# akanazawa/human_dynamics

Measured on AMD Instinct MI355X. Metric: frames/sec/GPU (ResNet+temporal+SMPL, 224x224); SMPL verts max-abs-err, higher is better.
Workload: dtype f16x3

## Files before the change

### human_dynamics_amd/_lib.py

```python
from __future__ import annotations

import ctypes as C
import os

from . import devflags

HERE = os.path.dirname(os.path.abspath(__file__))
LIB_PATH = devflags.get("LIB_PATH") or os.path.join(HERE, "libhmmr_hip.so")

HMMR_F32, HMMR_BF16, HMMR_F16X3 = 0, 1, 2
FLAG_SATURATED = 1
FLAG_NAN = 2
ABI_VERSION = 19
RESNET_UNITS = 16
RESNET_PROF_SLOTS = 64
MAX_TEMPORAL_BLOCKS = 8
MAX_REGRESSORS = 8

_vp, _fp, _ip = C.c_void_p, C.c_void_p, C.c_void_p


class ConvDesc(C.Structure):
    _fields_ = [
        ("in_", _vp), ("w", _vp), ("scale", _fp), ("shift", _fp), ("res", _vp), ("out", _vp),
        ("out2", _vp), ("scale2", _fp), ("shift2", _fp),
        ("in_dtype", C.c_int), ("out_dtype", C.c_int),
        ("n_img", C.c_int), ("hin", C.c_int), ("win", C.c_int), ("cin", C.c_int),
        ("in_img_stride", C.c_int64), ("in_row_stride", C.c_int), ("in_px_stride", C.c_int),
        ("kh", C.c_int), ("kw", C.c_int), ("sy", C.c_int), ("sx", C.c_int), ("py", C.c_int), ("px", C.c_int),
        ("ho", C.c_int), ("wo", C.c_int), ("cout", C.c_int), ("ldo", C.c_int),
        ("ldr", C.c_int), ("res_strided", C.c_int), ("res_img_stride", C.c_int64),
        ("res_row_stride", C.c_int), ("res_px_stride", C.c_int),
        ("relu", C.c_int), ("tile", C.c_int),
        ("split_k", C.c_int), ("ws", _vp), ("ws_bytes", C.c_size_t),
        ("pro_scale", _fp), ("pro_shift", _fp),
        ("out_b", _vp), ("ldo_b", C.c_int), ("n_split", C.c_int), ("relu_b", C.c_int),
        ("in2", _vp), ("cin2", C.c_int), ("k_order", C.c_int),
        ("batch", C.c_int), ("batch_in_bytes", C.c_int64), ("batch_w_bytes", C.c_int64), ("batch_out_bytes", C.c_int64),
        ("batch_res_bytes", C.c_int64), ("batch_scale_bytes", C.c_int64), ("batch_shift_bytes", C.c_int64),
    ]


class TailDesc(C.Structure):
    _fields_ = [
        ("dtype", C.c_int), ("h2", _vp), ("m", C.c_int), ("c_mid", C.c_int), ("depth", C.c_int),
        ("w3", _vp), ("scale3", _fp), ("shift3", _fp),
        ("res", _vp), ("ldr", C.c_int), ("res_strided", C.c_int), ("res_img_stride", C.c_int64),
        ("res_row_stride", C.c_int), ("res_px_stride", C.c_int), ("ho", C.c_int), ("wo", C.c_int),
        ("out", _vp), ("pre_scale", _fp), ("pre_shift", _fp),
        ("w1", _vp), ("scale1", _fp), ("shift1", _fp), ("relu1", C.c_int), ("n2", C.c_int),
        ("out_h1", _vp),
        ("h1", _vp), ("hin", C.c_int), ("win", C.c_int), ("w2", _vp), ("scale2", _fp), ("shift2", _fp),
        ("xp", _vp), ("wsc", _vp), ("shift_sc", _fp),
        ("conv2_stride", C.c_int), ("out_pre", _vp),
        ("pair_stream", _vp), ("c_xp", C.c_int), ("unit_stream", _vp),
    ]


class Debug(C.Structure):
    _fields_ = [("stem_route", C.c_int), ("stem_no_conv1", C.c_int), ("gemm_probe", C.c_int), ("smpl_blend_mfma", C.c_int), ("ief_no_group", C.c_int), ("reserved", C.c_int * 3),
                ("pair_min_pixels", C.c_int), ("pair_two_tile_min", C.c_int), ("pair_form", C.c_int)]


class LaunchCounts(C.Structure):
    _fields_ = [("unit_pair", C.c_ulonglong), ("b1_unit", C.c_ulonglong), ("tail_split", C.c_ulonglong), ("conv3x3_stream", C.c_ulonglong),
                ("conv1x1_stream", C.c_ulonglong)]


class StemCounts(C.Structure):
    _fields_ = [(k, C.c_ulonglong) for k in ("fused", "fused_conv1", "repack", "gemm", "pool")]


TILE_GENERIC, TILE_PATCH, TILE_STREAM_3X3, TILE_STREAM_1X1 = range(4)
CONV_TILE_MAX = 63


class ConvTileInfo(C.Structure):
    _fields_ = [(k, C.c_int) for k in ("tile", "family", "fm", "fn", "wgm", "wgn", "pixels", "channels", "row_blocks", "depth", "occupancy", "wmax",
                                       "split_only", "conv3_form", "cols", "tune_cols", "narrow", "rank", "candidate")] + [("text", C.c_char_p)]


class Layer(C.Structure):
    _fields_ = [("w", _vp), ("scale", _fp), ("shift", _fp), ("tile", C.c_int), ("k_order", C.c_int)]


class ResnetUnit(C.Structure):
    _fields_ = [("conv1", Layer), ("conv2", Layer), ("conv3", Layer), ("shortcut", Layer), ("c3sc", Layer), ("sc_c1", Layer),
                ("w3_frag", _vp), ("w1n_frag", _vp), ("pair_stream", _vp), ("conv1_frag", _vp), ("unit_stream", _vp), ("pre_scale", _fp), ("pre_shift", _fp),
                ("c_in", C.c_int), ("base", C.c_int), ("depth", C.c_int), ("stride", C.c_int),
                ("fuse_preact", C.c_int), ("fuse_tail", C.c_int)]


class ResnetWeights(C.Structure):
    _fields_ = [("dtype", C.c_int), ("stem", Layer),
                ("unit", ResnetUnit * RESNET_UNITS), ("post_scale", _fp), ("post_shift", _fp)]


SC_NONE, SC_LAUNCH, SC_LAUNCH_WITH_CONV1, SC_IN_CONV3, SC_IN_TAIL = range(5)
CONV1_LAUNCH, CONV1_READY = range(2)
CONV2_LAUNCH, CONV2_IN_TAIL = range(2)
END_CONV3_LAUNCH, END_TAIL_BF16, END_TAIL_BF16_STRIDE2, END_TAIL_SPLIT, END_B1_UNIT, END_UNIT_PAIR = range(6)


class UnitPlan(C.Structure):
    _fields_ = [(k, C.c_int) for k in ("shortcut", "conv1", "conv2", "end", "reads_fused_preact", "writes_raw", "writes_pre",
                                       "pair_demoted", "swaps_t1_t2", "leaves_h1")]


def resnet_plan(rw, n_total):
    plan = (UnitPlan * RESNET_UNITS)()
    check(load().hmmr_resnet50_plan(C.byref(rw), int(n_total), plan), "hmmr_resnet50_plan")
    return list(plan)


class TemporalBlock(C.Structure):
    _fields_ = [("gn1_gamma", _fp), ("gn1_beta", _fp), ("conv1", Layer),
                ("gn2_gamma", _fp), ("gn2_beta", _fp), ("conv2", Layer)]


class TemporalWeights(C.Structure):
    _fields_ = [("dtype", C.c_int), ("num_blocks", C.c_int), ("block", TemporalBlock * MAX_TEMPORAL_BLOCKS)]


class HallucinatorWeights(C.Structure):
    _fields_ = [("dtype", C.c_int), ("fc1", Layer), ("fc2", Layer), ("fc3", Layer)]


class IefRegressor(C.Structure):
    _fields_ = [("nd", C.c_int), ("fc1_phi", Layer), ("fc1_theta", Layer), ("fc2", Layer), ("fc3", Layer)]


class IefWeights(C.Structure):
    _fields_ = [("dtype", C.c_int), ("num_regressors", C.c_int), ("num_stages", C.c_int),
                ("reg", IefRegressor * MAX_REGRESSORS), ("mean_theta", _fp),
                ("no_optcam", C.c_int), ("delta_from_start", C.c_int)]


class IefRegGrads(C.Structure):
    _fields_ = [(k, _fp) for k in ("d_fc1_phi", "d_fc1_theta", "d_fc2", "d_fc3", "d_b1", "d_b2", "d_b3")]


class IefBwdDesc(C.Structure):
    _fields_ = [("strips", _fp), ("omega_start", _fp), ("keep", _vp), ("keep_scale", C.c_float), ("m", C.c_int), ("d_omegas", _fp),
                ("d_strips", _fp), ("d_omega_start", _fp), ("reg", IefRegGrads * MAX_REGRESSORS)]


TEMPORAL_GRAD_NAMES = ("gn1_gamma", "gn1_beta", "conv1", "b1", "gn2_gamma", "gn2_beta", "conv2", "b2")
HALLUCINATOR_GRAD_NAMES = ("fc1", "fc2", "fc3", "b1", "b2", "b3")


class TemporalBlockGrads(C.Structure):
    _fields_ = [("d_" + k, _fp) for k in TEMPORAL_GRAD_NAMES]


class TemporalBwdDesc(C.Structure):
    _fields_ = [("phi", _fp), ("b", C.c_int), ("t", C.c_int), ("d_strips", _fp), ("d_phi", _fp),
                ("block", TemporalBlockGrads * MAX_TEMPORAL_BLOCKS)]


class HallucinatorBwdDesc(C.Structure):
    _fields_ = [("phi", _fp), ("m", C.c_int), ("d_out", _fp), ("d_phi", _fp)] + [("d_" + k, _fp) for k in HALLUCINATOR_GRAD_NAMES]


class SmplConsts(C.Structure):
    _fields_ = [("num_verts", C.c_int), ("num_kps", C.c_int), ("lbs_nnz", C.c_int), ("vpad", C.c_int),
                ("dirs", _fp), ("j_template", _fp), ("j_shapedirs", _fp), ("parents", _ip),
                ("lbs_idx", _ip), ("lbs_w", _fp), ("kreg_ptr", _ip), ("kreg_idx", _ip), ("kreg_val", _fp),
                ("dirs_split", _vp)]


class SmplGradConsts(C.Structure):
    _fields_ = [("num_verts", C.c_int), ("num_kps", C.c_int), ("vk_ptr", _ip), ("vk_idx", _ip), ("vk_val", _fp)]


LOSS_KP, LOSS_KP_OPTCAM, LOSS_JOINTS, LOSS_SMPL, LOSS_CONST, LOSS_SHAPE_PRIOR = 1, 2, 4, 8, 16, 32
LOSS_NAMES = ("e_kp", "e_joints", "e_smpl_pose", "e_smpl_shape", "e_const", "e_shape", "total")
LOSS_NO_VISIBLE, LOSS_NOT_FINITE = 1, 2


class SeqLossDesc(C.Structure):
    _fields_ = [("B", C.c_int), ("T", C.c_int), ("K", C.c_int), ("delta_t", C.c_int), ("flags", C.c_uint), ("weights", C.c_float * 6),
                ("kps_pred", _fp), ("joints_pred", _fp), ("rs_pred", _fp), ("beta_pred", _fp), ("ld_beta", C.c_int),
                ("kps_gt", _fp), ("joints_gt", _fp), ("rs_gt", _fp), ("shapes_gt", _fp), ("has_gt3d_smpl", _fp), ("has_gt3d_joints", _fp),
                ("losses", _fp), ("d_kps", _fp), ("d_joints", _fp), ("d_rs", _fp), ("d_beta", _fp), ("best_cam", _fp), ("status", _vp),
                ("ws", _vp), ("ws_bytes", C.c_size_t)]


class Var(C.Structure):
    _fields_ = [("name", C.c_char_p), ("data", _fp), ("numel", C.c_int64)]


class SmplSource(C.Structure):
    _fields_ = [("num_verts", C.c_int), ("num_kps", C.c_int), ("v_template", _fp), ("shapedirs", _fp), ("posedirs", _fp),
                ("J_regressor", _fp), ("lbs_weights", _fp), ("kp_regressor", _fp), ("parents", _ip)]


class VideoPlan(C.Structure):
    _fields_ = [(k, C.c_int) for k in ("n", "T", "fov", "margin", "g", "n_windows", "max_frames", "max_windows", "resnet_passes", "tail_passes")]


class TracksPlan(C.Structure):
    _fields_ = [(k, C.c_int) for k in ("n_tracks", "T", "fov", "margin", "g", "n_frames", "n_windows", "max_frames", "max_windows",
                                       "resnet_passes", "tail_passes")]


class Model(C.Structure):
    _fields_ = [("resnet", C.POINTER(ResnetWeights)), ("temporal", C.POINTER(TemporalWeights)), ("hallucinator", C.POINTER(HallucinatorWeights)),
                ("ief", C.POINTER(IefWeights)), ("smpl", C.POINTER(SmplConsts)), ("sequence_length", C.c_int), ("fov", C.c_int)]


RENDER_MAX_FRAMES, RENDER_MIN_SIZE, RENDER_MAX_SIZE, RENDER_MAX_FACES = 4096, 16, 1024, 65536
RENDER_BG_COLOR, RENDER_BG_FLOAT, RENDER_BG_FRAME = 0, 1, 2
TRACK_MAX_KPS, TRACK_MAX_KERNEL, TRACK_MAX_RADIUS, TRACK_MAX_ROWS, TRACK_TILE = 64, 31, 64, 1 << 27, 256
TRACK_EMPTY, TRACK_BEFORE_ORIGIN, TRACK_CLIPPED, TRACK_NOT_FINITE = 1, 2, 4, 8
BBOX_EMPTY, BBOX_NOT_FINITE, BBOX_DEGENERATE, BBOX_BEYOND_START = 1, 2, 4, 8


class RenderDesc(C.Structure):
    _fields_ = [("verts", _fp), ("ld_verts", C.c_int64), ("cams", _fp), ("ld_cam", C.c_int64), ("geom", _fp),
                ("faces", _ip), ("face_colors", _fp), ("ld_face_colors", C.c_int64),
                ("n", C.c_int), ("nv", C.c_int), ("nf", C.c_int), ("size", C.c_int),
                ("rotate", C.c_int), ("rot", C.c_float * 9), ("color", C.c_float * 3), ("bg_color", C.c_float * 3),
                ("light_dir", C.c_float * 3), ("light_int_ambient", C.c_float), ("light_int_directional", C.c_float),
                ("light_color_ambient", C.c_float * 3), ("light_color_directional", C.c_float * 3),
                ("bg_mode", C.c_int), ("bg_image", _vp), ("bg_add", C.c_float), ("bg_mul", C.c_float),
                ("frame_h", C.c_int), ("frame_w", C.c_int), ("out_h", C.c_int), ("out_w", C.c_int),
                ("rgb", _vp), ("alpha", _fp), ("face_index", _ip), ("ws", _vp), ("ws_bytes", C.c_size_t)]


SCENE_MAX_TRACKS = 16


class SceneTrack(C.Structure):
    _fields_ = [("verts", _fp), ("ld_verts", C.c_int64), ("cams", _fp), ("ld_cam", C.c_int64), ("geom", _fp),
                ("priority", _fp), ("start", C.c_int), ("end", C.c_int), ("color", C.c_float * 3)]


class SceneDesc(C.Structure):
    _fields_ = [("tracks", C.POINTER(SceneTrack)), ("n_tracks", C.c_int), ("faces", _ip),
                ("nv", C.c_int), ("nf", C.c_int), ("n_frames", C.c_int), ("size", C.c_int),
                ("out_h", C.c_int), ("out_w", C.c_int), ("bg_color", C.c_float * 3),
                ("light_dir", C.c_float * 3), ("light_int_ambient", C.c_float), ("light_int_directional", C.c_float),
                ("light_color_ambient", C.c_float * 3), ("light_color_directional", C.c_float * 3),
                ("bg_mode", C.c_int), ("bg_image", _vp), ("frame_h", C.c_int), ("frame_w", C.c_int),
                ("rgb", _vp), ("alpha", _fp), ("face_index", _ip), ("owner", _ip), ("ws", _vp), ("ws_bytes", C.c_size_t)]


SKELETON_MAX_RADIUS, COLLAGE_MAX_PANEL_WIDTH = 1024, 4096


class SkeletonDesc(C.Structure):
    _fields_ = [("kps", _fp), ("ld_kps", C.c_int64), ("vis", _vp), ("n", C.c_int), ("nk", C.c_int), ("h", C.c_int), ("w", C.c_int),
                ("kp_add", C.c_float), ("kp_mul", C.c_float), ("draw_edges", C.c_int), ("radius", C.c_int),
                ("bg_float", _fp), ("bg_add", C.c_float), ("bg_mul", C.c_float), ("bg_u8", _vp), ("out", _vp)]


class CollageDesc(C.Structure):
    _fields_ = [("rend_crop", _vp), ("skel_crop", _vp), ("render_og", _vp), ("rot_og", _vp),
                ("n", C.c_int), ("S", C.c_int), ("h", C.c_int), ("w", C.c_int), ("out", _vp)]


SIGNATURES = {
    "hmmr_abi_version": (C.c_int, []),
    "hmmr_pack_resnet_bytes": (C.c_size_t, [C.POINTER(Var), C.c_int, C.c_int]),
    "hmmr_pack_resnet": (C.c_int, [C.POINTER(Var), C.c_int, C.c_int, _vp, C.c_size_t, _vp, C.POINTER(ResnetWeights)]),
    "hmmr_pack_temporal_bytes": (C.c_size_t, [C.POINTER(Var), C.c_int, C.c_int, C.c_int]),
    "hmmr_pack_temporal": (C.c_int, [C.POINTER(Var), C.c_int, C.c_int, C.c_int, _vp, C.c_size_t, _vp, C.POINTER(TemporalWeights)]),
    "hmmr_pack_hallucinator_bytes": (C.c_size_t, [C.POINTER(Var), C.c_int, C.c_int]),
    "hmmr_pack_hallucinator": (C.c_int, [C.POINTER(Var), C.c_int, C.c_int, _vp, C.c_size_t, _vp, C.POINTER(HallucinatorWeights)]),
    "hmmr_pack_ief_bytes": (C.c_size_t, [C.POINTER(Var), C.c_int, C.c_int, C.POINTER(C.c_int), C.c_int]),
    "hmmr_pack_ief": (C.c_int, [C.POINTER(Var), C.c_int, C.c_int, C.POINTER(C.c_int), C.c_int, C.c_int, _vp, C.c_size_t, _vp, C.POINTER(IefWeights)]),
    "hmmr_pack_smpl_bytes": (C.c_size_t, [C.POINTER(SmplSource), C.c_int, C.c_int]),
    "hmmr_pack_smpl": (C.c_int, [C.POINTER(SmplSource), C.c_int, C.c_int, _vp, C.c_size_t, _vp, C.POINTER(SmplConsts)]),
    "hmmr_pack_smpl_grad_bytes": (C.c_size_t, [C.POINTER(SmplSource), C.c_int]),
    "hmmr_pack_smpl_grad": (C.c_int, [C.POINTER(SmplSource), C.c_int, _vp, C.c_size_t, _vp, C.POINTER(SmplGradConsts)]),
    "hmmr_last_error": (C.c_char_p, []),
    "hmmr_run_flags": (C.c_int, [C.POINTER(C.c_uint), C.c_int]),
    "hmmr_set_debug": (None, [C.POINTER(Debug)]),
    "hmmr_get_debug": (None, [C.POINTER(Debug)]),
    "hmmr_launch_counts": (None, [C.POINTER(LaunchCounts), C.c_int]),
    "hmmr_stem_launch_counts": (None, [C.POINTER(StemCounts), C.c_int]),
    "hmmr_conv_gemm": (C.c_int, [C.POINTER(ConvDesc), _vp]),
    "hmmr_conv_tile_info": (C.c_int, [C.c_int, C.POINTER(ConvTileInfo)]),
    "hmmr_conv_tile_for": (C.c_int, [C.c_int] * 6),
    "hmmr_conv_tile_fits": (C.c_int, [C.c_int] * 8),
    "hmmr_conv_tile_f_movie": (C.c_int, []),
    "hmmr_conv_splitk_workspace_bytes": (C.c_size_t, [C.c_int, C.c_int, C.c_int]),
    "hmmr_resnet50_workspace_bytes": (C.c_size_t, [C.c_int, C.c_int]),
    "hmmr_resnet50_fwd": (C.c_int, [C.POINTER(ResnetWeights), _fp, C.c_int, C.c_int, _fp, _vp, C.c_size_t, _vp,
                                    C.POINTER(C.c_float)]),
    "hmmr_resnet50_stem_workspace_bytes": (C.c_size_t, [C.POINTER(ResnetWeights), C.c_int]),
    "hmmr_resnet50_stem": (C.c_int, [C.POINTER(ResnetWeights), _fp, C.c_int, C.c_int, _vp, _vp, C.POINTER(C.c_int), _vp, C.c_size_t, _vp]),
    "hmmr_resnet50_plan": (C.c_int, [C.POINTER(ResnetWeights), C.c_int, C.POINTER(UnitPlan)]),
    "hmmr_temporal_workspace_bytes": (C.c_size_t, [C.c_int, C.c_int, C.c_int]),
    "hmmr_temporal_fwd": (C.c_int, [C.POINTER(TemporalWeights), _fp, C.c_int, C.c_int, _fp, _vp, C.c_size_t, _vp]),
    "hmmr_hallucinator_workspace_bytes": (C.c_size_t, [C.c_int, C.c_int]),
    "hmmr_hallucinator_fwd": (C.c_int, [C.POINTER(HallucinatorWeights), _fp, C.c_int, _fp, _vp, C.c_size_t, _vp]),
    "hmmr_groupnorm_relu": (C.c_int, [_fp, _fp, _fp, C.c_int, C.c_int, C.c_int, C.c_int, _vp, C.c_int, _vp]),
    "hmmr_ief_workspace_bytes": (C.c_size_t, [C.c_int, C.c_int, C.c_int]),
    "hmmr_ief_fwd": (C.c_int, [C.POINTER(IefWeights), _fp, C.c_int, _fp, _vp, C.c_size_t, _vp]),
    "hmmr_ief_fwd_from": (C.c_int, [C.POINTER(IefWeights), _fp, _fp, C.c_int, _fp, _vp, C.c_size_t, _vp]),
    "hmmr_ief_bwd_workspace_bytes": (C.c_size_t, [C.c_int, C.c_int, C.c_int]),
    "hmmr_ief_fwd_train": (C.c_int, [C.POINTER(IefWeights), _fp, _fp, _vp, C.c_float, C.c_int, _fp, _vp, C.c_size_t, _vp]),
    "hmmr_ief_bwd": (C.c_int, [C.POINTER(IefWeights), C.POINTER(IefBwdDesc), _vp, C.c_size_t, _vp]),
    "hmmr_temporal_bwd_workspace_bytes": (C.c_size_t, [C.c_int, C.c_int, C.c_int]),
    "hmmr_temporal_bwd": (C.c_int, [C.POINTER(TemporalWeights), C.POINTER(TemporalBwdDesc), _vp, C.c_size_t, _vp]),
    "hmmr_hallucinator_bwd_workspace_bytes": (C.c_size_t, [C.c_int]),
    "hmmr_hallucinator_bwd": (C.c_int, [C.POINTER(HallucinatorWeights), C.POINTER(HallucinatorBwdDesc), _vp, C.c_size_t, _vp]),
    "hmmr_smpl_workspace_bytes": (C.c_size_t, [C.c_int]),
    "hmmr_smpl_fwd": (C.c_int, [C.POINTER(SmplConsts), _fp, C.c_int, _fp, C.c_int, _fp, C.c_int, C.c_int,
                                _fp, _fp, _fp, _fp, _vp, C.c_size_t, _vp]),
    "hmmr_smpl_bwd_workspace_bytes": (C.c_size_t, [C.POINTER(SmplConsts), C.c_int]),
    "hmmr_smpl_bwd": (C.c_int, [C.POINTER(SmplConsts), C.POINTER(SmplGradConsts), _fp, C.c_int, _fp, C.c_int, _fp, C.c_int, _fp, C.c_int,
                                _fp, _fp, _fp, _fp, _fp, _fp, _fp, _vp, C.c_size_t, _vp]),
    "hmmr_seq_losses_workspace_bytes": (C.c_size_t, [C.c_int, C.c_int]),
    "hmmr_seq_losses": (C.c_int, [C.POINTER(SeqLossDesc), _vp]),
    "hmmr_omega_loss_grad_workspace_bytes": (C.c_size_t, [C.POINTER(SmplConsts), C.c_int, C.c_int]),
    "hmmr_omega_loss_grad": (C.c_int, [C.POINTER(SmplConsts), C.POINTER(SmplGradConsts), C.POINTER(SeqLossDesc), _fp, C.c_int, _fp, _fp,
                                       _vp, C.c_size_t, _vp]),
    "hmmr_crop_frames": (C.c_int, [_vp, _ip, C.c_int, C.c_int, C.c_int, _fp, _vp]),
    "hmmr_tube_augment": (C.c_int, [_vp, C.c_int, C.c_int, C.c_int, C.c_int, _ip, _vp, _fp, C.c_int, _fp, _vp]),
    "hmmr_track_workspace_bytes": (C.c_size_t, [C.c_int, C.c_int]),
    "hmmr_track_bbox": (C.c_int, [_fp, _vp, C.POINTER(C.c_int32), C.c_int, C.c_int, C.c_double, C.c_int, C.POINTER(C.c_double), C.c_int,
                                  _fp, _fp, _ip, _vp, C.c_size_t, _vp]),
    "hmmr_track_smooth": (C.c_int, [_fp, C.POINTER(C.c_int32), C.c_int, C.c_int, C.POINTER(C.c_double), C.c_int, _fp, _vp, C.c_size_t, _vp]),
    "hmmr_track_crop_geom": (C.c_int, [_fp, C.POINTER(C.c_int32), _ip, C.c_int, C.c_int, C.c_int, _ip, _fp, _ip, _vp]),
    "hmmr_bottleneck_tail": (C.c_int, [C.POINTER(TailDesc), _vp]),
    "hmmr_pair_stream_bytes": (C.c_size_t, [C.c_int, C.c_int, C.c_int]),
    "hmmr_b1_unit_stream_bytes": (C.c_size_t, [C.c_int]),
    "hmmr_conv3x3_stream_bytes": (C.c_size_t, [C.c_int, C.c_int]),
    "hmmr_conv1x1_stream_bytes": (C.c_size_t, [C.c_int, C.c_int]),
    "hmmr_mfma_rate_probe": (C.c_int, [C.c_int, C.c_int, _fp, _vp]),
    "hmmr_clock_probe": (C.c_int, [_vp, C.c_int, C.c_int, _vp, _vp]),
    "hmmr_render_handoff": (C.c_int, [_fp, C.c_int64, _fp, C.c_int64, _fp, C.c_int64, _fp, C.c_int, C.c_int, C.c_int,
                                      _fp, _fp, _fp, _vp]),
    "hmmr_render_workspace_bytes": (C.c_size_t, [C.c_int, C.c_int, C.c_int]),
    "hmmr_render_mesh": (C.c_int, [C.POINTER(RenderDesc), _vp]),
    "hmmr_render_scene_workspace_bytes": (C.c_size_t, [C.c_int, C.c_int, C.c_int, C.c_int]),
    "hmmr_render_scene": (C.c_int, [C.POINTER(SceneDesc), _vp]),
    "hmmr_video_bbox": (C.c_int, [_fp, C.c_longlong, _fp, C.c_longlong, C.c_int, _fp, C.c_double, C.POINTER(C.c_int32), C.c_int, C.c_int, C.c_int,
                                  C.c_double, _ip, _fp, _ip, _vp]),
    "hmmr_skeleton_radius": (C.c_int, [C.c_int, C.c_int]),
    "hmmr_draw_skeleton": (C.c_int, [C.POINTER(SkeletonDesc), _vp]),
    "hmmr_collage_width": (C.c_int, [C.c_int, C.c_int, C.c_int]),
    "hmmr_compose_collage": (C.c_int, [C.POINTER(CollageDesc), _vp]),
    "hmmr_eval_joints": (C.c_int, [_fp, _fp, C.c_int, C.c_int, C.c_int, C.c_int, _fp, _fp, _fp, _fp, _vp]),
    "hmmr_eval_verts": (C.c_int, [_fp, C.c_int64, _fp, C.c_int64, C.c_int, C.c_int, _fp, _vp]),
    "hmmr_eval_joints_ld": (C.c_int, [_fp, C.c_int64, _fp, C.c_int64, C.c_int, C.c_int, C.c_int, C.c_int, _fp, _fp, _fp, _fp, _vp]),
    "hmmr_eval_kps": (C.c_int, [_fp, C.c_int64, _fp, C.c_int64, C.c_int, C.c_int, C.c_double, C.c_int, C.c_float,
                                _fp, _fp, _fp, _fp, _vp]),
    "hmmr_rotmat_to_axis_angle": (C.c_int, [_fp, C.c_int64, C.c_int, C.c_int, _fp, C.c_int64, _vp]),
    "hmmr_axis_angle_to_rotmat": (C.c_int, [_fp, C.c_int64, C.c_int, C.c_int, _fp, C.c_int64, _vp]),
    "hmmr_global_rigid_transformation": (C.c_int, [_fp, _fp, _ip, C.c_int, _fp, _fp, C.c_int, _vp]),
    "hmmr_smpl_fwd_records": (C.c_int, [C.POINTER(SmplConsts), _fp, C.c_int, C.c_int, _fp, C.c_int64, C.POINTER(C.c_int32),
                                        _vp, C.c_size_t, _vp]),
    "hmmr_smpl_fwd_strided": (C.c_int, [C.POINTER(SmplConsts), _fp, C.c_int, _fp, C.c_int, _fp, C.c_int, C.c_int,
                                        _fp, _fp, _fp, _fp, C.c_int64, _vp, C.c_size_t, _vp]),
    "hmmr_video_plan": (C.c_int, [C.c_int, C.c_int, C.c_int, C.c_int, C.c_int, C.POINTER(VideoPlan)]),
    "hmmr_record_layout": (C.c_int, [C.c_int, C.c_int, C.c_int, C.POINTER(C.c_int32), C.POINTER(C.c_int64)]),
    "hmmr_gather_windows": (C.c_int, [_fp, C.c_int, _fp, C.c_int, C.c_int, C.c_int, C.c_int, C.c_int, C.c_int, _fp, _vp]),
    "hmmr_keep_rows": (C.c_int, [_fp, C.c_int, C.c_int, C.c_int, C.c_int, C.c_int, C.c_int, C.c_int, _fp, C.c_int64, _vp]),
    "hmmr_predict_video_workspace_bytes": (C.c_size_t, [C.POINTER(Model), C.c_int, C.c_int, C.c_int]),
    "hmmr_predict_video": (C.c_int, [C.POINTER(Model), _fp, C.c_int, _fp, C.c_int64, C.POINTER(C.c_int32), C.c_int, C.c_int,
                                     _vp, C.c_size_t, _vp]),
    "hmmr_tracks_plan": (C.c_int, [C.POINTER(C.c_int32), C.c_int, C.c_int, C.c_int, C.c_int, C.c_int, C.POINTER(TracksPlan)]),
    "hmmr_tracks_window_owner": (C.c_int, [C.POINTER(C.c_int32), C.c_int, C.c_int, C.c_int, C.POINTER(C.c_int), C.POINTER(C.c_int)]),
    "hmmr_tracks_window_rows": (C.c_int, [C.POINTER(C.c_int32), C.c_int, C.c_int, C.c_int, C.c_int, C.POINTER(C.c_int), C.POINTER(C.c_int)]),
    "hmmr_tracks_tail_pass": (C.c_int, [C.POINTER(C.c_int32), C.c_int, C.POINTER(TracksPlan), C.c_int, C.POINTER(C.c_int), C.POINTER(C.c_int),
                                        C.POINTER(C.c_int), C.POINTER(C.c_int)]),
    "hmmr_gather_windows_tracks": (C.c_int, [_fp, _fp, C.POINTER(C.c_int32), C.c_int, C.c_int, C.c_int, C.c_int, C.c_int, C.c_int, C.c_int, _fp, _vp]),
    "hmmr_keep_rows_tracks": (C.c_int, [_fp, C.POINTER(C.c_int32), C.c_int, C.c_int, C.c_int, C.c_int, C.c_int, C.c_int, C.c_int, _fp, C.c_int64,
                                        _vp]),
    "hmmr_predict_tracks_workspace_bytes": (C.c_size_t, [C.POINTER(Model), C.POINTER(C.c_int32), C.c_int, C.c_int, C.c_int]),
    "hmmr_predict_tracks": (C.c_int, [C.POINTER(Model), _fp, C.POINTER(C.c_int32), C.c_int, _fp, C.c_int64, C.POINTER(C.c_int32), C.c_int, C.c_int,
                                      _vp, C.c_size_t, _vp]),
}

_lib = None


class HmmrError(RuntimeError):
    pass


def load():
    global _lib
    if _lib is not None:
        return _lib
    if not os.path.exists(LIB_PATH):
        raise HmmrError("%s not found: build it with `python -m human_dynamics_amd.build` "
                        "(the HIP library is mandatory; there is no CPU fallback)" % LIB_PATH)
    import torch
    if torch.cuda.is_available():
        torch.cuda.init()
    lib = C.CDLL(LIB_PATH)
    for name, (res, args) in SIGNATURES.items():
        fn = getattr(lib, name)
        fn.restype, fn.argtypes = res, args
    if lib.hmmr_abi_version() != ABI_VERSION:
        raise HmmrError("libhmmr_hip.so ABI version mismatch")
    _lib = lib
    return lib


def launch_counts(clear=False):
    c = LaunchCounts()
    load().hmmr_launch_counts(C.byref(c), int(bool(clear)))
    return {k: int(getattr(c, k)) for k, _ in LaunchCounts._fields_}


def conv_tiles(family=None):
    lib, rows = load(), []
    for t in range(1, CONV_TILE_MAX + 1):
        r = ConvTileInfo()
        if lib.hmmr_conv_tile_info(t, C.byref(r)) == 0 and family in (None, r.family):
            rows.append(r)
    return rows


def stem_launch_counts(clear=False):
    c = StemCounts()
    load().hmmr_stem_launch_counts(C.byref(c), int(bool(clear)))
    return {k: int(getattr(c, k)) for k, _ in StemCounts._fields_}


def check(rc, what=""):
    if rc != 0:
        msg = load().hmmr_last_error()
        raise HmmrError("%s failed (%d): %s" % (what or "hmmr call", rc, msg.decode() if msg else "?"))


def ptr(t):
    return None if t is None else t.data_ptr()
```

### human_dynamics_amd/csrc/gemm_conv.hip

```cpp
#include <stdlib.h>
#include <string.h>
#include <type_traits>

#include "conv_tiles.h"
#include "stream_kit.h"

struct ConvArgs {
    const void* in; const void* w; const float* scale; const float* shift;
    const void* res; void* out; void* out2; const float* scale2; const float* shift2;
    const float* pro_scale; const float* pro_shift;
    void* out_b; int ldo_b, n_split, relu_b;
    int M, K, cout, ldo, ldr;
    int Wo, HoWo, Hin, Win;
    long long in_img_stride; int in_row_stride, in_px_stride;
    int cin_log2, KH, KW, SY, SX, PY, PX;
    int res_strided; long long res_img_stride; int res_row_stride, res_px_stride;
    int relu, tiles_n, n_tiles;
    int kt_per_slice;
    long long out_slice_stride;
    int probe;
    const void* in2; int cin2, kt_split;
    int batch; long long bz_in, bz_w, bz_out, bz_res, bz_scale, bz_shift;
};

__device__ __forceinline__ ConvArgs batch_problem(const ConvArgs& a0, int z) {
    ConvArgs a = a0;
    if (a0.batch > 1) {
        const long long zz = z;
        a.in = (const char*)a0.in + zz * a0.bz_in;
        a.w = (const char*)a0.w + zz * a0.bz_w;
        if (a0.out) a.out = (char*)a0.out + zz * a0.bz_out;
        if (a0.out2) a.out2 = (char*)a0.out2 + zz * a0.bz_out;
        if (a0.res) a.res = (const char*)a0.res + zz * a0.bz_res;
        if (a0.scale) a.scale = (const float*)((const char*)a0.scale + zz * a0.bz_scale);
        if (a0.shift) a.shift = (const float*)((const char*)a0.shift + zz * a0.bz_shift);
        if (a0.scale2) a.scale2 = (const float*)((const char*)a0.scale2 + zz * a0.bz_scale);
        if (a0.shift2) a.shift2 = (const float*)((const char*)a0.shift2 + zz * a0.bz_shift);
    }
    return a;
}

#ifdef HMMR_GEMM_PROBE
#define HMMR_PROBE(a, bit) (((a).probe & (bit)) != 0)
#else
#define HMMR_PROBE(a, bit) false
#endif

template <typename TA> struct Frag;
template <> struct Frag<float>  { typedef f32x4 type; };
template <> struct Frag<bf16_t> { typedef bf16x8 type; };
struct split_frag { shalf8 hi, lo; };
template <> struct Frag<bsplit_t> { typedef split_frag type; };

__device__ __forceinline__ f32x16 mma(const f32x4& a, const f32x4& b, f32x16 c) {
#pragma unroll
    for (int j = 0; j < 4; ++j) c = __builtin_amdgcn_mfma_f32_32x32x2f32(a[j], b[j], c, 0, 0, 0);
    return c;
}
__device__ __forceinline__ f32x16 mma(const bf16x8& a, const bf16x8& b, f32x16 c) {
    return __builtin_amdgcn_mfma_f32_32x32x16_bf16(a, b, c, 0, 0, 0);
}
__device__ __forceinline__ f32x16 mma(const split_frag& a, const split_frag& b, f32x16 c) {
    c = mfma_split(a.lo, b.hi, c);
    c = mfma_split(a.hi, b.lo, c);
    return mfma_split(a.hi, b.hi, c);
}
template <typename TA> struct FragIO {
    static constexpr int CHUNKS = 4;
    __device__ static __forceinline__ typename Frag<TA>::type read(const char* row, int c, int lh, int fsw) {
        return *(const typename Frag<TA>::type*)(row + (((2 * c + lh) ^ fsw) << 4));
    }
};
template <> struct FragIO<bsplit_t> {
    static constexpr int CHUNKS = 2;
    __device__ static __forceinline__ split_frag read(const char* row, int c, int lh, int fsw) {
        const int g = 2 * (2 * c + lh);
        split_frag f;
        f.hi = *(const shalf8*)(row + ((g ^ fsw) << 4));
        f.lo = *(const shalf8*)(row + (((g + 1) ^ fsw) << 4));
        return f;
    }
};
template <typename TO> __device__ __forceinline__ void store_tail(TO* p, const float (&v)[8], int cnt) {
    if constexpr (!std::is_same<TO, bsplit_t>::value)
        for (int j = 0; j < cnt; ++j) p[j] = elem_traits<TO>::from_f32(v[j]);
}

__device__ const u32x4 g_zero_page[4] = {};

template <typename TA> __device__ __forceinline__ u32x4 preact_slot(const u32x4& v, const f32x4* sc, const f32x4* sh);
template <> __device__ __forceinline__ u32x4 preact_slot<float>(const u32x4& v, const f32x4* sc, const f32x4* sh) {
    u32x4 o;
#pragma unroll
    for (int i = 0; i < 4; ++i) o[i] = __float_as_uint(fmaxf(fmaf(__uint_as_float(v[i]), sc[0][i], sh[0][i]), 0.f));
    return o;
}
template <> __device__ __forceinline__ u32x4 preact_slot<bf16_t>(const u32x4& v, const f32x4* sc, const f32x4* sh) {
    u32x4 o;
#pragma unroll
    for (int i = 0; i < 4; ++i) {
        const float lo = __uint_as_float(v[i] << 16), hi = __uint_as_float(v[i] & 0xffff0000u);
        const int e = 2 * i;
        const float a = fmaxf(fmaf(lo, sc[e >> 2][e & 3], sh[e >> 2][e & 3]), 0.f);
        const float b = fmaxf(fmaf(hi, sc[(e + 1) >> 2][(e + 1) & 3], sh[(e + 1) >> 2][(e + 1) & 3]), 0.f);
        typedef __attribute__((ext_vector_type(2))) __bf16 bf16x2;
        bf16x2 pk = {(bf16_t)a, (bf16_t)b};
        o[i] = __builtin_bit_cast(unsigned, pk);
    }
    return o;
}


template <typename TA, typename TO, int BM, int BN, int WGM, int WGN, bool PRO, bool UTAP, int NSTAGE>
__global__ __launch_bounds__(WGM * WGN * 64, NSTAGE >= 3 ? (WGM * WGN) / 4 : ((WGM * WGN == 8) ? 4 : 1))
void conv_gemm_kernel(const ConvArgs a0) {
    const ConvArgs a = batch_problem(a0, blockIdx.z);
    static_assert(NSTAGE >= 2 && NSTAGE <= 4, "2 stages (two workgroups per CU) or a 3/4-stage ring (one workgroup per CU)");
    static_assert(NSTAGE == 2 || WGM * WGN == 8, "the deep ring is written for 8-wave workgroups");
    static_assert(!PRO || UTAP, "the fused pre-activation needs one tap per K step");
    constexpr int NT = WGM * WGN * 64;
    constexpr int RPP = NT / 8;
    constexpr int EPS = elem_traits<TA>::EPS;
    constexpr int BKE = 8 * EPS;
    constexpr int TM = BM / WGM, TN = BN / WGN;
    constexpr int FM = TM / 32, FN = TN / 32;
    constexpr int PA = BM / RPP, PB = BN / RPP;
    static_assert(PA >= 1 && PB >= 1, "tile smaller than one staging pass");
    constexpr int A_BYTES = BM * 128, B_BYTES = BN * 128, STAGE = A_BYTES + B_BYTES;
    typedef typename Frag<TA>::type frag_t;

    extern __shared__ __attribute__((aligned(16))) char smem[];

    const int tid = threadIdx.x;
    const int lane = tid & 63;
    const int wave = __builtin_amdgcn_readfirstlane(tid >> 6);
    const int L = xcd_remap(blockIdx.x, a.n_tiles);
    const int m0 = (L / a.tiles_n) * BM;
    const int n0 = (L % a.tiles_n) * BN;

    const int pslot = tid & 7, r0 = tid >> 3;
    const int lslot = pslot ^ ((r0 >> 1) & 7);
    const TA* __restrict__ in = (const TA*)a.in;
    const TA* __restrict__ wt = (const TA*)a.w;

    const TA* aptr[PA]; unsigned amask[PA];
#pragma unroll
    for (int p = 0; p < PA; ++p) {
        const int m = m0 + r0 + RPP * p;
        aptr[p] = in; amask[p] = 0u;
        if (m < a.M) {
            const int img = m / a.HoWo, rem = m - img * a.HoWo;
            const int oy = rem / a.Wo, ox = rem - oy * a.Wo;
            const int iy0 = oy * a.SY - a.PY, ix0 = ox * a.SX - a.PX;
            aptr[p] = in + (long long)img * a.in_img_stride + (long long)iy0 * a.in_row_stride +
                      (long long)ix0 * a.in_px_stride + lslot * EPS;
            unsigned mk = 0u;
            for (int t = 0; t < a.KH * a.KW; ++t) {
                const int ky = t / a.KW, kx = t - ky * a.KW;
                if ((unsigned)(iy0 + ky) < (unsigned)a.Hin && (unsigned)(ix0 + kx) < (unsigned)a.Win) mk |= 1u << t;
            }
            amask[p] = mk;
        }
    }
    const TA* wptr = wt + (long long)(n0 + r0) * a.K + lslot * EPS;
    const int cin_mask = (1 << a.cin_log2) - 1;

    auto tap_of = [&](int k, int& tap) -> int {
        tap = k >> a.cin_log2;
        const int ci = k & cin_mask;
        int ky, kx;
        if (a.KW == 1) { ky = tap; kx = 0; }
        else if (a.KW == 3) { ky = (int)(((unsigned)tap * 43691u) >> 17); kx = tap - 3 * ky; }
        else { ky = tap / a.KW; kx = tap - ky * a.KW; }
        return ky * a.in_row_stride + kx * a.in_px_stride + ci;
    };

    constexpr bool SPLIT = std::is_same<TA, bsplit_t>::value;
    constexpr int PCH = EPS;
    u32x4 ra[PRO ? PA : 1];
    f32x4 psc[PRO ? PCH / 4 : 1], psh[PRO ? PCH / 4 : 1];
    auto glds_a = [&](int kt, int buf) {
        int tap;
        const int koff = UTAP ? tap_of(kt * BKE, tap) : tap_of(kt * BKE + lslot * EPS, tap) - lslot * EPS;
        char* sa = smem + buf * STAGE + wave * 1024;
        if (a.in2 && kt >= a.kt_split) {
            const TA* in2 = (const TA*)a.in2 + (kt - a.kt_split) * BKE + lslot * EPS;
#pragma unroll
            for (int p = 0; p < PA; ++p) {
                const void* src = (amask[p] & 1u) ? (const void*)(in2 + (long long)(m0 + r0 + RPP * p) * a.cin2)
                                                  : (const void*)g_zero_page;
                __builtin_amdgcn_global_load_lds((gptr_t)src, (lptr_t)(sa + p * (RPP * 128)), 16, 0, 0);
            }
            return;
        }
#pragma unroll
        for (int p = 0; p < PA; ++p) {
            const bool ok = (amask[p] >> tap) & 1u;
            const void* src = ok ? (const void*)(aptr[p] + koff) : (const void*)g_zero_page;
            __builtin_amdgcn_global_load_lds((gptr_t)src, (lptr_t)(sa + p * (RPP * 128)), 16, 0, 0);
        }
    };
    auto glds_b = [&](int kt, int buf) {
        char* sb = smem + buf * STAGE + A_BYTES + wave * 1024;
#pragma unroll
        for (int p = 0; p < PB; ++p)
            __builtin_amdgcn_global_load_lds((gptr_t)(wptr + (long long)(RPP * p) * a.K + kt * BKE),
                                             (lptr_t)(sb + p * (RPP * 128)), 16, 0, 0);
    };
    u32x4 rb[PRO ? PB : 1];
    auto load_regs = [&](int kt) {
        if constexpr (PRO) {
            int tap;
            const int koff = tap_of(kt * BKE, tap);
            const int ci = ((kt * BKE) & cin_mask) + lslot * EPS;
#pragma unroll
            for (int q = 0; q < PCH / 4; ++q) {
                psc[q] = *(const f32x4*)(a.pro_scale + ci + 4 * q);
                psh[q] = *(const f32x4*)(a.pro_shift + ci + 4 * q);
            }
#pragma unroll
            for (int p = 0; p < PA; ++p) ra[p] = *(const u32x4*)(aptr[p] + koff);
#pragma unroll
            for (int p = 0; p < PB; ++p) rb[p] = *(const u32x4*)(wptr + (long long)(RPP * p) * a.K + kt * BKE);
        }
    };
    auto store_regs = [&](int buf) {
        if constexpr (PRO) {
            char* sa = smem + buf * STAGE + r0 * 128 + pslot * 16;
#pragma unroll
            for (int p = 0; p < PA; ++p) {
                if constexpr (SPLIT) *(u32x4*)(sa + p * (RPP * 128)) = preact_slot_split(ra[p], psc[0], psh[0], lslot & 1);
                else *(u32x4*)(sa + p * (RPP * 128)) = preact_slot<TA>(ra[p], psc, psh);
            }
#pragma unroll
            for (int p = 0; p < PB; ++p) *(u32x4*)(sa + A_BYTES + p * (RPP * 128)) = rb[p];
        }
    };

    const int wm = wave / WGN, wn = wave % WGN;
    const int lr = lane & 31, lh = lane >> 5;
    const int fsw = (lr >> 1) & 7;
    const int a_row_off = (wm * TM + lr) * 128;
    const int b_row_off = A_BYTES + (wn * TN + lr) * 128;

    f32x16 acc[FM][FN];
#pragma unroll
    for (int i = 0; i < FM; ++i)
#pragma unroll
        for (int j = 0; j < FN; ++j)
#pragma unroll
            for (int r = 0; r < 16; ++r) acc[i][j][r] = 0.f;

    constexpr int VPR = BN / 8;
    constexpr int NIT = (BM * VPR) / NT;
    constexpr int RV = (int)(8 * sizeof(TO) / 16);
    const TO* __restrict__ res = PRO ? nullptr : (const TO*)a.res;
    u32x4 rres[PRO ? 1 : NIT][RV];
    if (!PRO && res) {
#pragma unroll
        for (int it = 0; it < NIT; ++it) {
            const int idx = it * NT + tid;
            const int m = m0 + idx / VPR, n = n0 + (idx % VPR) * 8;
#pragma unroll
            for (int q = 0; q < RV; ++q) rres[it][q] = u32x4{0u, 0u, 0u, 0u};
            if (m < a.M && n < a.cout) {
                long long ro;
                if (a.res_strided) {
                    const int img = m / a.HoWo, rem = m - img * a.HoWo;
                    const int oy = rem / a.Wo, ox = rem - oy * a.Wo;
                    ro = (long long)img * a.res_img_stride + (long long)oy * a.res_row_stride +
                         (long long)ox * a.res_px_stride + n;
                } else {
                    ro = (long long)m * a.ldr + n;
                }
#pragma unroll
                for (int q = 0; q < RV; ++q) rres[it][q] = *((const u32x4*)(res + ro) + q);
            }
        }
    }

    const int nk = a.K / BKE;
    auto compute_stage = [&](const char* sbuf) {
        constexpr int NCHK = FragIO<TA>::CHUNKS;
        constexpr bool DBUF = NSTAGE >= 3 || !(std::is_same<TA, bsplit_t>::value && WGM * WGN == 8 && FM * FN >= 2);
        frag_t fa[DBUF ? 2 : 1][FM], fb[DBUF ? 2 : 1][FN];
        auto read_frags = [&](int c, int slot_) {
#pragma unroll
            for (int i = 0; i < FM; ++i) fa[slot_][i] = FragIO<TA>::read(sbuf + a_row_off + i * 32 * 128, c, lh, fsw);
#pragma unroll
            for (int j = 0; j < FN; ++j) fb[slot_][j] = FragIO<TA>::read(sbuf + b_row_off + j * 32 * 128, c, lh, fsw);
        };
        if constexpr (DBUF) {
            read_frags(0, 0);
#pragma unroll
            for (int c = 0; c < NCHK; ++c) {
                if (c + 1 < NCHK) read_frags(c + 1, (c + 1) & 1);
                __builtin_amdgcn_sched_barrier(0);
#pragma unroll
                for (int i = 0; i < FM; ++i)
#pragma unroll
                    for (int j = 0; j < FN; ++j) acc[i][j] = mma(fa[c & 1][i], fb[c & 1][j], acc[i][j]);
            }
        } else {
#pragma unroll
            for (int c = 0; c < NCHK; ++c) {
                read_frags(c, 0);
#pragma unroll
                for (int i = 0; i < FM; ++i)
#pragma unroll
                    for (int j = 0; j < FN; ++j) acc[i][j] = mma(fa[0][i], fb[0][j], acc[i][j]);
            }
        }
    };
    const int kt0 = blockIdx.y * a.kt_per_slice;
    const int kt1 = min(nk, kt0 + a.kt_per_slice);
    if constexpr (NSTAGE >= 3) {
        constexpr int LPW = PA + PB;
        static_assert(LPW * (NSTAGE - 2) < 64, "vmcnt range");
        [[maybe_unused]] float* s_pro = (float*)(smem + NSTAGE * STAGE);
        if constexpr (PRO) {
            for (int i = tid; i < a.K; i += NT) { s_pro[i] = a.pro_scale[i]; s_pro[a.K + i] = a.pro_shift[i]; }
        }
        auto transform = [&](int kt, int buf) {
            if constexpr (PRO) {
                const int ci = ((kt * BKE) & cin_mask) + lslot * EPS;
                f32x4 sc_[PCH / 4], sh_[PCH / 4];
#pragma unroll
                for (int q = 0; q < PCH / 4; ++q) {
                    sc_[q] = *(const f32x4*)(s_pro + ci + 4 * q);
                    sh_[q] = *(const f32x4*)(s_pro + a.K + ci + 4 * q);
                }
                char* sa = smem + buf * STAGE + r0 * 128 + pslot * 16;
#pragma unroll
                for (int p = 0; p < PA; ++p) {
                    u32x4* q = (u32x4*)(sa + p * (RPP * 128));
                    if constexpr (SPLIT) *q = preact_slot_split(*q, sc_[0], sh_[0], lslot & 1);
                    else *q = preact_slot<TA>(*q, sc_, sh_);
                }
            }
        };
        auto wait_ahead = [&](int ahead) {
            __builtin_amdgcn_sched_barrier(0);
            if (ahead >= 2) { if constexpr (NSTAGE >= 4) wait_vm_lgkm0<2 * LPW>(); }
            else if (ahead == 1) wait_vm_lgkm0<LPW>();
            else wait_vm_lgkm0<0>();
        };
        const int nloc = kt1 - kt0;
#pragma unroll
        for (int s_ = 0; s_ < NSTAGE - 1; ++s_)
            if (s_ < nloc && !HMMR_PROBE(a, 8)) { glds_a(kt0 + s_, s_); glds_b(kt0 + s_, s_); }
        if constexpr (PRO) {
            wait_vm_lgkm0<63>();
            __builtin_amdgcn_s_barrier();
        }
        wait_ahead(min(NSTAGE - 2, nloc - 1));
        transform(kt0, 0);
        wait_vm_lgkm0<63>();
        __builtin_amdgcn_s_barrier();
        constexpr int NCHK = FragIO<TA>::CHUNKS;
        const int grp = wave >> 2;
        int cur = 0, nxt = NSTAGE - 1;
        if (grp == 1) __builtin_amdgcn_s_barrier();
        for (int kt = kt0; kt < kt1; ++kt) {
            const char* sbuf = smem + cur * STAGE;
            const int c1 = (cur + 1 == NSTAGE) ? 0 : cur + 1;
            const bool fill = kt + NSTAGE - 1 < kt1 && !HMMR_PROBE(a, 2);
            frag_t fa[NCHK][FM], fb[NCHK][FN];
#pragma unroll
            for (int c = 0; c < NCHK; ++c) {
                if (c > 0 && HMMR_PROBE(a, 16)) {
#pragma unroll
                    for (int i = 0; i < FM; ++i) fa[c][i] = fa[0][i];
#pragma unroll
                    for (int j = 0; j < FN; ++j) fb[c][j] = fb[0][j];
                    continue;
                }
#pragma unroll
                for (int i = 0; i < FM; ++i) fa[c][i] = FragIO<TA>::read(sbuf + a_row_off + i * 32 * 128, c, lh, fsw);
#pragma unroll
                for (int j = 0; j < FN; ++j) fb[c][j] = FragIO<TA>::read(sbuf + b_row_off + j * 32 * 128, c, lh, fsw);
            }
            if (fill) {
                if (!HMMR_PROBE(a, 64)) glds_a(kt + NSTAGE - 1, nxt);
                if (!HMMR_PROBE(a, 32)) glds_b(kt + NSTAGE - 1, nxt);
            }
            if (grp == 1 && kt + 1 < kt1) {
                wait_ahead(min(NSTAGE - 2, kt1 - 2 - kt));
                transform(kt + 1, c1);
            }
            wait_vm_lgkm0<63>();
            __builtin_amdgcn_sched_barrier(0);
            __builtin_amdgcn_s_barrier();
            __builtin_amdgcn_sched_barrier(0);
            if (!HMMR_PROBE(a, 1)) {
                __builtin_amdgcn_s_setprio(1);
#pragma unroll
                for (int c = 0; c < NCHK; ++c)
#pragma unroll
                    for (int i = 0; i < FM; ++i)
#pragma unroll
                        for (int j = 0; j < FN; ++j) acc[i][j] = mma(fa[c][i], fb[c][j], acc[i][j]);
                __builtin_amdgcn_s_setprio(0);
            }
            if (grp == 0 && kt + 1 < kt1) {
                wait_ahead(min(NSTAGE - 2, kt1 - 2 - kt));
                transform(kt + 1, c1);
                wait_vm_lgkm0<63>();
            }
            __builtin_amdgcn_sched_barrier(0);
            __builtin_amdgcn_s_barrier();
            __builtin_amdgcn_sched_barrier(0);
            nxt = cur; cur = c1;
        }
        if (grp == 0) __builtin_amdgcn_s_barrier();
    } else if constexpr (PRO) {
        load_regs(kt0);
        store_regs(0);
        if (kt0 + 1 < kt1) load_regs(kt0 + 1);
        __syncthreads();
        for (int kt = kt0; kt < kt1; ++kt) {
            const int cur = (kt - kt0) & 1;
            if (kt + 1 < kt1 && !HMMR_PROBE(a, 2)) store_regs(cur ^ 1);
            if (kt + 2 < kt1 && !HMMR_PROBE(a, 2)) load_regs(kt + 2);
            if (!HMMR_PROBE(a, 1)) compute_stage(smem + cur * STAGE);
            if (!HMMR_PROBE(a, 4)) __syncthreads();
        }
    } else {
        glds_a(kt0, 0);
        glds_b(kt0, 0);
        __syncthreads();
        for (int kt = kt0; kt < kt1; ++kt) {
            const int cur = (kt - kt0) & 1;
            if (kt + 1 < kt1 && !HMMR_PROBE(a, 2)) { glds_a(kt + 1, cur ^ 1); glds_b(kt + 1, cur ^ 1); }
            if (!HMMR_PROBE(a, 1)) compute_stage(smem + cur * STAGE);
            if (!HMMR_PROBE(a, 4)) __syncthreads();
        }
    }

    float* sc = (float*)smem;
#pragma unroll
    for (int i = 0; i < FM; ++i)
#pragma unroll
        for (int j = 0; j < FN; ++j)
#pragma unroll
            for (int r = 0; r < 16; ++r) {
                const int row = wm * TM + i * 32 + (r & 3) + 8 * (r >> 2) + 4 * lh;
                const int col = wn * TN + j * 32 + lr;
                sc[row * BN + col] = acc[i][j][r];
            }
    __syncthreads();

    TO* __restrict__ out = a.out ? (TO*)a.out + (long long)blockIdx.y * a.out_slice_stride : nullptr;
    TO* __restrict__ out2 = (TO*)a.out2;
    float satmax = 0.f;
#pragma unroll
    for (int it = 0; it < NIT; ++it) {
        const int idx = it * NT + tid;
        const int row = idx / VPR, col = (idx % VPR) * 8;
        const int m = m0 + row, n = n0 + col;
        if (m >= a.M || n >= a.cout) continue;
        float v[8];
        load8(sc + row * BN + col, v);
        if (a.scale && a.shift) {
            float s[8], b[8]; load8(a.scale + n, s); load8(a.shift + n, b);
#pragma unroll
            for (int j = 0; j < 8; ++j) v[j] = fmaf(v[j], s[j], b[j]);
        } else if (a.scale) {
            float s[8]; load8(a.scale + n, s);
#pragma unroll
            for (int j = 0; j < 8; ++j) v[j] *= s[j];
        } else if (a.shift) {
            float b[8]; load8(a.shift + n, b);
#pragma unroll
            for (int j = 0; j < 8; ++j) v[j] += b[j];
        }
        const bool full = (n + 8 <= a.cout);
        if (!PRO && res) {
            float rr[8];
            unpack8<TO>(rres[PRO ? 0 : it], rr);
#pragma unroll
            for (int j = 0; j < 8; ++j) v[j] += rr[j];
        }
        const bool second = a.out_b && n >= a.n_split;
        if (second ? a.relu_b : a.relu) {
#pragma unroll
            for (int j = 0; j < 8; ++j) v[j] = fmaxf(v[j], 0.f);
        }
        if (second) {
            TO* ob = (TO*)a.out_b + (long long)m * a.ldo_b + (n - a.n_split);
            if (full) store8<TO>(ob, v, satmax);
            else store_tail(ob, v, a.cout - n);
            continue;
        }
        const long long oo = (long long)m * a.ldo + n;
        if (out) {
            if (full) store8<TO>(out + oo, v, satmax);
            else store_tail(out + oo, v, a.cout - n);
        }
        if (out2) {
            float s2[8], b2[8], u[8];
            load8(a.scale2 + n, s2); load8(a.shift2 + n, b2);
#pragma unroll
            for (int j = 0; j < 8; ++j) {
                const float vr = stored_value<TO>(v[j]);
                u[j] = fmaxf(fmaf(vr, s2[j], b2[j]), 0.f);
            }
            if (full) store8<TO>(out2 + oo, u, satmax);
            else store_tail(out2 + oo, u, a.cout - n);
        }
    }
    if constexpr (std::is_same<TO, bsplit_t>::value) split_flag_max(satmax);
}

__device__ __forceinline__ unsigned patch_tap_mask(int m, const ConvArgs& a) {
    if (m >= a.M) return 0u;
    const int rem = m % a.HoWo, y = rem / a.Wo, x = rem - y * a.Wo;
    unsigned mk = 0u;
#pragma unroll
    for (int t = 0; t < 9; ++t) {
        const int yy = y + t / 3 - 1, xx = x + t % 3 - 1;
        if ((unsigned)yy < (unsigned)a.Hin && (unsigned)xx < (unsigned)a.Win) mk |= 1u << t;
    }
    return mk;
}
template <typename TO, int BM, int BN, int WGM, int WGN>
__device__ __forceinline__ void patch_epilogue(const ConvArgs& a, char* smem, const f32x16 (&acc)[2][2], int m0, int n0,
                                               int tid, int wm, int wn, int lr, int lh) {
    constexpr int NT = 512, TM = BM / WGM, TN = BN / WGN;
    static_assert(TM == 64 && TN == 64, "64x64 wave tiles");
    float* sc = (float*)smem;
#pragma unroll
    for (int i = 0; i < 2; ++i)
#pragma unroll
        for (int j = 0; j < 2; ++j)
#pragma unroll
            for (int r = 0; r < 16; ++r) {
                const int row = wm * TM + i * 32 + (r & 3) + 8 * (r >> 2) + 4 * lh;
                const int col = wn * TN + j * 32 + lr;
                sc[row * BN + col] = acc[i][j][r];
            }
    __syncthreads();
    constexpr int VPR = BN / 8, NIT = (BM * VPR) / NT;
    TO* __restrict__ out = (TO*)a.out;
    float satmax = 0.f;
#pragma unroll
    for (int it = 0; it < NIT; ++it) {
        const int idx = it * NT + tid;
        const int row = idx / VPR, col = (idx % VPR) * 8;
        const int m = m0 + row, n = n0 + col;
        if (m >= a.M || n >= a.cout) continue;
        float v[8];
        load8(sc + row * BN + col, v);
        if (a.scale && a.shift) {
            float s[8], b[8]; load8(a.scale + n, s); load8(a.shift + n, b);
#pragma unroll
            for (int j = 0; j < 8; ++j) v[j] = fmaf(v[j], s[j], b[j]);
        } else if (a.scale) {
            float s[8]; load8(a.scale + n, s);
#pragma unroll
            for (int j = 0; j < 8; ++j) v[j] *= s[j];
        } else if (a.shift) {
            float b[8]; load8(a.shift + n, b);
#pragma unroll
            for (int j = 0; j < 8; ++j) v[j] += b[j];
        }
        if (a.relu) {
#pragma unroll
            for (int j = 0; j < 8; ++j) v[j] = fmaxf(v[j], 0.f);
        }
        store8<TO>(out + (long long)m * a.ldo + n, v, satmax);
    }
    if constexpr (std::is_same<TO, bsplit_t>::value) split_flag_max(satmax);
}

template <typename TA, typename TO, int BM, int BN, int WGM, int WGN, int NPP>
__global__ __launch_bounds__(512, 1) void conv3x3_patch_kernel(const ConvArgs a) {
    static_assert(WGM * WGN == 8, "8-wave workgroups");
    constexpr int RPP = 64, NSB = 3;
    constexpr int EPS = elem_traits<TA>::EPS, BKE = 8 * EPS;
    constexpr int TM = BM / WGM, TN = BN / WGN, FM = TM / 32, FN = TN / 32;
    constexpr int PB = BN / RPP;
    constexpr int B_BYTES = BN * 128, P_BYTES = NPP * RPP * 128, OFF_P = NSB * B_BYTES;
    constexpr int NCHK = FragIO<TA>::CHUNKS;
    typedef typename Frag<TA>::type frag_t;

    extern __shared__ __attribute__((aligned(16))) char smem[];
    const int tid = threadIdx.x;
    const int lane = tid & 63;
    const int wave = __builtin_amdgcn_readfirstlane(tid >> 6);
    const int L = xcd_remap(blockIdx.x, a.n_tiles);
    const int m0 = (L / a.tiles_n) * BM;
    const int n0 = (L % a.tiles_n) * BN;
    const int W = a.Win, C = 1 << a.cin_log2;
    const int need = BM + 2 * W + 2;
    constexpr int ZROW = NPP * RPP - 2;
    const int base = m0 - W - 1;

    const int pslot = tid & 7, r0 = tid >> 3;
    const int lslot = pslot ^ ((r0 >> 1) & 7);
    const TA* __restrict__ in = (const TA*)a.in;
    const TA* pptr[NPP];
#pragma unroll
    for (int p = 0; p < NPP; ++p) {
        const int r = RPP * p + r0, px = base + r;
        pptr[p] = (r < need && px >= 0 && px < a.M) ? in + (long long)px * C + lslot * EPS : nullptr;
    }
    const TA* wptr = (const TA*)a.w + (long long)(n0 + r0) * a.K + lslot * EPS;
    auto glds_patch = [&](int c, int buf) {
        char* sp = smem + OFF_P + buf * P_BYTES + wave * 1024;
#pragma unroll
        for (int p = 0; p < NPP; ++p) {
            const void* src = pptr[p] ? (const void*)(pptr[p] + c * BKE) : (const void*)g_zero_page;
            __builtin_amdgcn_global_load_lds((gptr_t)src, (lptr_t)(sp + p * (RPP * 128)), 16, 0, 0);
        }
    };
    auto glds_b = [&](int kt, int buf) {
        char* sb = smem + buf * B_BYTES + wave * 1024;
#pragma unroll
        for (int p = 0; p < PB; ++p)
            __builtin_amdgcn_global_load_lds((gptr_t)(wptr + (long long)(RPP * p) * a.K + kt * BKE),
                                             (lptr_t)(sb + p * (RPP * 128)), 16, 0, 0);
    };

    const int wm = wave / WGN, wn = wave % WGN;
    const int lr = lane & 31, lh = lane >> 5;
    const int fswb = (lr >> 1) & 7;
    const int b_row_off = (wn * TN + lr) * 128;
    int prow[FM];
    unsigned pmask[FM];
#pragma unroll
    for (int i = 0; i < FM; ++i) {
        prow[i] = wm * TM + i * 32 + lr;
        pmask[i] = patch_tap_mask(m0 + prow[i], a);
    }

    f32x16 acc[FM][FN];
#pragma unroll
    for (int i = 0; i < FM; ++i)
#pragma unroll
        for (int j = 0; j < FN; ++j)
#pragma unroll
            for (int r = 0; r < 16; ++r) acc[i][j][r] = 0.f;

    const int nc = C / BKE, nk = 9 * nc;
    auto wait_stage = [&](int kt, int t, int c) {
        __builtin_amdgcn_sched_barrier(0);
        if (kt + 2 < nk) {
            if (t <= 1 && c + 1 < nc) wait_vm_lgkm0<PB + NPP>();
            else wait_vm_lgkm0<PB>();
        } else wait_vm_lgkm0<0>();
    };
    glds_patch(0, 0);
    glds_b(0, 0);
    glds_b(1, 1);
    __builtin_amdgcn_sched_barrier(0);
    wait_vm_lgkm0<PB>();
    __builtin_amdgcn_s_barrier();
    const int grp = wave >> 2;
    int cur = 0, nxt = NSB - 1, t = 0, c = 0;
    if (grp == 1) __builtin_amdgcn_s_barrier();
    for (int kt = 0; kt < nk; ++kt) {
        const char* sb = smem + cur * B_BYTES;
        const char* sp = smem + OFF_P + (c & 1) * P_BYTES;
        const int c1 = (cur + 1 == NSB) ? 0 : cur + 1;
        const int ky = (t * 11) >> 5;
        int ts = ky * W + (t - 3 * ky);
        if (HMMR_PROBE(a, 128)) ts = 0;
        if (HMMR_PROBE(a, 256)) ts &= ~1;
        if (HMMR_PROBE(a, 512)) ts &= ~15;
        frag_t fa[NCHK][FM], fb[NCHK][FN];
#pragma unroll
        for (int i = 0; i < FM; ++i) {
            const int tap_row = prow[i] + ts;
            const int row = ((pmask[i] >> t) & 1u) ? tap_row : ZROW + (tap_row & 1);
            const char* rp = sp + row * 128;
            const int fsw = (tap_row >> 1) & 7;
#pragma unroll
            for (int ch = 0; ch < NCHK; ++ch) {
                if (ch > 0 && HMMR_PROBE(a, 16)) { fa[ch][i] = fa[0][i]; continue; }
                fa[ch][i] = FragIO<TA>::read(rp, ch, lh, fsw);
            }
        }
#pragma unroll
        for (int j = 0; j < FN; ++j)
#pragma unroll
            for (int ch = 0; ch < NCHK; ++ch) {
                if (ch > 0 && HMMR_PROBE(a, 16)) { fb[ch][j] = fb[0][j]; continue; }
                fb[ch][j] = FragIO<TA>::read(sb + b_row_off + j * 32 * 128, ch, lh, fswb);
            }
        if (kt + 2 < nk && !HMMR_PROBE(a, 32)) glds_b(kt + 2, nxt);
        if (t == 0 && c + 1 < nc && !HMMR_PROBE(a, 64)) glds_patch(c + 1, (c + 1) & 1);
        if (grp == 1 && kt + 1 < nk) wait_stage(kt, t, c);
        wait_vm_lgkm0<63>();
        __builtin_amdgcn_sched_barrier(0);
        __builtin_amdgcn_s_barrier();
        __builtin_amdgcn_sched_barrier(0);
        if (!HMMR_PROBE(a, 1)) {
            __builtin_amdgcn_s_setprio(1);
#pragma unroll
            for (int ch = 0; ch < NCHK; ++ch)
#pragma unroll
                for (int i = 0; i < FM; ++i)
#pragma unroll
                    for (int j = 0; j < FN; ++j) acc[i][j] = mma(fa[ch][i], fb[ch][j], acc[i][j]);
            __builtin_amdgcn_s_setprio(0);
        }
        if (grp == 0 && kt + 1 < nk) wait_stage(kt, t, c);
        __builtin_amdgcn_sched_barrier(0);
        __builtin_amdgcn_s_barrier();
        __builtin_amdgcn_sched_barrier(0);
        nxt = cur; cur = c1;
        if (++t == 9) { t = 0; ++c; }
    }
    if (grp == 0) __builtin_amdgcn_s_barrier();

    patch_epilogue<TO, BM, BN, WGM, WGN>(a, smem, acc, m0, n0, tid, wm, wn, lr, lh);
}

template <typename TA, typename TO, int NPP>
__global__ __launch_bounds__(512, 1) void conv3x3_pipe_kernel(const ConvArgs a) {
    constexpr int BM = 256, BN = 128, WGM = 4, WGN = 2;
    constexpr int RPP = 64, NSB = 4;
    constexpr int EPS = elem_traits<TA>::EPS, BKE = 8 * EPS;
    constexpr int TM = BM / WGM, TN = BN / WGN, FM = TM / 32, FN = TN / 32;
    constexpr int PB = BN / RPP;
    constexpr int B_BYTES = BN * 128, P_BYTES = NPP * RPP * 128, OFF_P = NSB * B_BYTES;
    constexpr int NCHK = FragIO<TA>::CHUNKS;
    static_assert(FM == 2 && FN == 2 && NCHK == 2, "written for 64x64 wave tiles of split operands");
    typedef typename Frag<TA>::type frag_t;

    extern __shared__ __attribute__((aligned(16))) char smem[];
    const int tid = threadIdx.x;
    const int lane = tid & 63;
    const int wave = __builtin_amdgcn_readfirstlane(tid >> 6);
    const int L = xcd_remap(blockIdx.x, a.n_tiles);
    const int m0 = (L / a.tiles_n) * BM;
    const int n0 = (L % a.tiles_n) * BN;
    const int W = a.Win, C = 1 << a.cin_log2;
    const int need = BM + 2 * W + 2;
    constexpr int ZROW = NPP * RPP - 2;
    const int base = m0 - W - 1;

    const int pslot = tid & 7, r0 = tid >> 3;
    const int lslot = pslot ^ ((r0 >> 1) & 7);
    const TA* __restrict__ in = (const TA*)a.in;
    const TA* pptr[NPP];
#pragma unroll
    for (int p = 0; p < NPP; ++p) {
        const int r = RPP * p + r0, px = base + r;
        pptr[p] = (r < need && px >= 0 && px < a.M) ? in + (long long)px * C + lslot * EPS : nullptr;
    }
    const TA* wptr = (const TA*)a.w + (long long)(n0 + r0) * a.K + lslot * EPS;
    auto glds_patch = [&](int c, int buf) {
        char* sp = smem + OFF_P + buf * P_BYTES + wave * 1024;
#pragma unroll
        for (int p = 0; p < NPP; ++p) {
            const void* src = pptr[p] ? (const void*)(pptr[p] + c * BKE) : (const void*)g_zero_page;
            __builtin_amdgcn_global_load_lds((gptr_t)src, (lptr_t)(sp + p * (RPP * 128)), 16, 0, 0);
        }
    };
    auto glds_b = [&](int kt, int buf) {
        char* sb = smem + buf * B_BYTES + wave * 1024;
#pragma unroll
        for (int p = 0; p < PB; ++p)
            __builtin_amdgcn_global_load_lds((gptr_t)(wptr + (long long)(RPP * p) * a.K + kt * BKE),
                                             (lptr_t)(sb + p * (RPP * 128)), 16, 0, 0);
    };

    const int wm = wave / WGN, wn = wave % WGN;
    const int lr = lane & 31, lh = lane >> 5;
    const int fswb = (lr >> 1) & 7;
    const int b_row_off = (wn * TN + lr) * 128;
    int prow[FM];
    unsigned pmask[FM];
#pragma unroll
    for (int i = 0; i < FM; ++i) {
        prow[i] = wm * TM + i * 32 + lr;
        pmask[i] = patch_tap_mask(m0 + prow[i], a);
    }

    f32x16 acc[FM][FN];
#pragma unroll
    for (int i = 0; i < FM; ++i)
#pragma unroll
        for (int j = 0; j < FN; ++j)
#pragma unroll
            for (int r = 0; r < 16; ++r) acc[i][j][r] = 0.f;

    const int nc = C / BKE, nk = 9 * nc;
    frag_t fa[2][NCHK][FM], fb[2][NCHK][FN];
    auto read_piece = [&](frag_t (&da)[NCHK][FM], frag_t (&db)[NCHK][FN], int q, int t_, const char* sp_, const char* sb_) {
        const int ch = q >> 2, w_ = q & 3;
        if (w_ == 0 || w_ == 3) {
            const int i = w_ == 0 ? 0 : 1;
            const int ky = (t_ * 11) >> 5;
            const int tap_row = prow[i] + ky * W + (t_ - 3 * ky);
            const int row = ((pmask[i] >> t_) & 1u) ? tap_row : ZROW + (tap_row & 1);
            da[ch][i] = FragIO<TA>::read(sp_ + row * 128, ch, lh, (tap_row >> 1) & 7);
        } else {
            const int j = w_ - 1;
            db[ch][j] = FragIO<TA>::read(sb_ + b_row_off + j * 32 * 128, ch, lh, fswb);
        }
    };
    glds_patch(0, 0);
#pragma unroll
    for (int s_ = 0; s_ < NSB - 1; ++s_) glds_b(s_, s_);
    __builtin_amdgcn_sched_barrier(0);
    wait_vm_lgkm0<PB>();
    __builtin_amdgcn_s_barrier();
#pragma unroll
    for (int q = 0; q < 8; ++q) read_piece(fa[0], fb[0], q, 0, smem + OFF_P, smem);
    int t = 0, c = 0;
    auto step = [&](auto cur_c, int kt) {
        constexpr int CUR = decltype(cur_c)::value, NXT = CUR ^ 1;
        if (kt + 3 < nk) glds_b(kt + 3, (kt + 3) & 3);
        if (t == 0 && c + 1 < nc) glds_patch(c + 1, (c + 1) & 1);
        const int t1 = (t == 8) ? 0 : t + 1, cn = (t == 8) ? c + 1 : c;
        const char* sp1 = smem + OFF_P + (cn & 1) * P_BYTES;
        const char* sb1 = smem + ((kt + 1) & 3) * B_BYTES;
#pragma unroll
        for (int q = 0; q < 8; ++q) {
            read_piece(fa[NXT], fb[NXT], q, t1, sp1, sb1);
            const int ch = q >> 2, i = (q >> 1) & 1, j = q & 1;
            acc[i][j] = mma(fa[CUR][ch][i], fb[CUR][ch][j], acc[i][j]);
        }
        __builtin_amdgcn_sched_barrier(0);
        if (kt + 2 < nk) {
            const bool pend = t <= 1 && c + 1 < nc;
            if (kt + 3 < nk) { if (pend) wait_vm_lgkm0<PB + NPP>(); else wait_vm_lgkm0<PB>(); }
            else wait_vm_lgkm0<0>();
        } else wait_vm_lgkm0<63>();
        __builtin_amdgcn_sched_barrier(0);
        __builtin_amdgcn_s_barrier();
        __builtin_amdgcn_sched_barrier(0);
        t = t1; c = cn;
    };
    for (int kt = 0; kt < nk; kt += 2) {
        step(ic<0>{}, kt);
        if (kt + 1 < nk) step(ic<1>{}, kt + 1);
    }

    patch_epilogue<TO, BM, BN, WGM, WGN>(a, smem, acc, m0, n0, tid, wm, wn, lr, lh);
}

template <typename TA, typename TO, int NPP>
static int launch_pipe(const ConvArgs& base, hipStream_t stream) {
    ConvArgs a = base;
    const int tiles_m = (a.M + 255) / 256;
    a.tiles_n = (a.cout + 127) / 128;
    a.n_tiles = tiles_m * a.tiles_n;
    constexpr int kloop = 4 * 128 * 128 + 2 * NPP * 64 * 128, epi = 256 * 128 * 4;
    constexpr int lds = kloop > epi ? kloop : epi;
    static_assert(lds <= 160 * 1024, "LDS");
    auto kern = conv3x3_pipe_kernel<TA, TO, NPP>;
    static DeviceOnce once;
    return launch_with_lds(kern, once, dim3(a.n_tiles), dim3(512), 160 * 1024, lds, stream, a);
}

static int patch_rows_bound(int bm, int h, int w) { (void)h; return bm + 2 * w + 2 + 2; }

template <typename TA, typename TO, int BM, int BN, int WGM, int WGN, int NPP>
static int launch_patch(const ConvArgs& base, hipStream_t stream) {
    ConvArgs a = base;
    const int tiles_m = (a.M + BM - 1) / BM;
    a.tiles_n = (a.cout + BN - 1) / BN;
    a.n_tiles = tiles_m * a.tiles_n;
    constexpr int kloop = 3 * BN * 128 + 2 * NPP * 64 * 128, epi = BM * BN * 4;
    constexpr int lds = kloop > epi ? kloop : epi;
    static_assert(lds <= 160 * 1024, "LDS");
    auto kern = conv3x3_patch_kernel<TA, TO, BM, BN, WGM, WGN, NPP>;
    static DeviceOnce once;
    return launch_with_lds(kern, once, dim3(a.n_tiles), dim3(512), 160 * 1024, lds, stream, a);
}

template <typename TA, typename TO, int BM, int BN, int WGM, int WGN, bool PIPE>
static int launch_patch_npp(const ConvArgs& a, int tile, hipStream_t stream) {
    const int npp = (patch_rows_bound(BM, a.Hin, a.Win) + 63) / 64;
    if constexpr (PIPE) {
        if constexpr (std::is_same<TA, bsplit_t>::value) {
            if (npp <= 5) return launch_pipe<TA, TO, 5>(a, stream);
            if (npp <= 6) return launch_pipe<TA, TO, 6>(a, stream);
        }
    } else if constexpr (BM == 256) {
        if (npp <= 5) return launch_patch<TA, TO, BM, BN, WGM, WGN, 5>(a, stream);
        if (npp <= 7) return launch_patch<TA, TO, BM, BN, WGM, WGN, 7>(a, stream);
    } else {
        if (npp <= 3) return launch_patch<TA, TO, BM, BN, WGM, WGN, 3>(a, stream);
        if (npp <= 4) return launch_patch<TA, TO, BM, BN, WGM, WGN, 4>(a, stream);
    }
    hmmr_set_error("hmmr_conv_gemm: k_order 1, tile %d: a %d x %d image needs a patch of %d x 64 rows, more than LDS holds",
                   tile, a.Hin, a.Win, npp);
    return -1;
}

template <typename TA, typename TO>
static int launch_patch_tiled(const ConvArgs& a, int tile, hipStream_t stream) {
    switch (tile) {
#define X(ID, BM, BN, WGM, WGN, PIPE, ...) case ID: return launch_patch_npp<TA, TO, BM, BN, WGM, WGN, PIPE>(a, tile, stream);
        HMMR_PATCH_TILES(X)
#undef X
        default: hmmr_set_error("hmmr_conv_gemm: k_order 1: no tile %d", tile); return -1;
    }
}

template <typename TA, typename TO, int BM, int BN, int WGM, int WGN, bool PRO, bool UTAP, int NSTAGE>
static int launch_cfg(const ConvArgs& base, int slices, hipStream_t stream) {
    ConvArgs a = base;
    const int tiles_m = (a.M + BM - 1) / BM;
    a.tiles_n = (a.cout + BN - 1) / BN;
    a.n_tiles = tiles_m * a.tiles_n;
    constexpr int kring = NSTAGE * (BM + BN) * 128, epi = BM * BN * 4;
    const int kloop = kring + ((PRO && NSTAGE >= 3) ? 8 * a.K : 0);
    const int lds = kloop > epi ? kloop : epi;
    if (lds > 160 * 1024) { hmmr_set_error("hmmr_conv_gemm: tile needs %d B of LDS (K = %d)", lds, a.K); return -1; }
    auto kern = conv_gemm_kernel<TA, TO, BM, BN, WGM, WGN, PRO, UTAP, NSTAGE>;
    static DeviceOnce once;
    constexpr int BKE_ = 8 * elem_traits<TA>::EPS;
    const int nk = a.K / BKE_;
    a.kt_per_slice = (nk + slices - 1) / slices;
    return launch_with_lds(kern, once, dim3(a.n_tiles, slices, a.batch), dim3(WGM * WGN * 64), NSTAGE >= 3 ? 160 * 1024 : lds, lds, stream, a);
}

template <typename TA, typename TO, bool PRO, bool UTAP>
static int launch_tiled(const ConvArgs& a, int tile, int slices, hipStream_t stream) {
    switch (tile) {
#define X(ID, BM, BN, WGM, WGN, NSTAGE, ...) case ID: return launch_cfg<TA, TO, BM, BN, WGM, WGN, PRO, UTAP, NSTAGE>(a, slices, stream);
        HMMR_GENERIC_TILES(X)
#undef X
        default: hmmr_set_error("hmmr_conv_gemm: k_order 0: no tile %d", tile); return -1;
    }
}

template <typename TA, typename TO>
static int launch_typed(const ConvArgs& a, int tile, int slices, hipStream_t stream) {
    if (tile == 0) tile = conv_tiles::choose_generic(a.M, a.cout, slices);
    char why[256];
    HMMR_REQUIRE(!conv_tiles::fit(tile, conv_tiles::Problem{0, 0, 0, a.cout, -1, 0, 0}, why, sizeof why), "hmmr_conv_gemm: %s", why);
    const bool utap = ((size_t)1 << a.cin_log2) * sizeof(TA) >= 128;
    if (a.pro_scale) {
        if (!utap) { hmmr_set_error("hmmr_conv_gemm: fused pre-activation needs cin*sizeof >= 128"); return -1; }
        return launch_tiled<TA, TO, true, true>(a, tile, slices, stream);
    }
    return utap ? launch_tiled<TA, TO, false, true>(a, tile, slices, stream)
                : launch_tiled<TA, TO, false, false>(a, tile, slices, stream);
}

template <typename TO>
__global__ __launch_bounds__(256) void splitk_reduce_kernel(const ConvArgs a0, const float* __restrict__ part,
                                                            int slices, int ldw, long long plane) {
    const ConvArgs a = batch_problem(a0, blockIdx.y);
    part += (long long)blockIdx.y * slices * plane;
    const int vpr = (a.cout + 7) / 8;
    const long long i = (long long)blockIdx.x * 256 + threadIdx.x;
    if (i >= (long long)a.M * vpr) return;
    const int m = (int)(i / vpr), n = (int)(i % vpr) * 8;
    float v[8];
    load8(part + (long long)m * ldw + n, v);
    for (int s = 1; s < slices; ++s) {
        float p[8];
        load8(part + s * plane + (long long)m * ldw + n, p);
#pragma unroll
        for (int j = 0; j < 8; ++j) v[j] += p[j];
    }
    if (a.scale && a.shift) {
        float s[8], b[8]; load8(a.scale + n, s); load8(a.shift + n, b);
#pragma unroll
        for (int j = 0; j < 8; ++j) v[j] = fmaf(v[j], s[j], b[j]);
    } else if (a.scale) {
        float s[8]; load8(a.scale + n, s);
#pragma unroll
        for (int j = 0; j < 8; ++j) v[j] *= s[j];
    } else if (a.shift) {
        float b[8]; load8(a.shift + n, b);
#pragma unroll
        for (int j = 0; j < 8; ++j) v[j] += b[j];
    }
    const bool full = (n + 8 <= a.cout);
    const TO* __restrict__ res = (const TO*)a.res;
    if (res) {
        long long ro;
        if (a.res_strided) {
            const int img = m / a.HoWo, rem = m - img * a.HoWo;
            const int oy = rem / a.Wo, ox = rem - oy * a.Wo;
            ro = (long long)img * a.res_img_stride + (long long)oy * a.res_row_stride + (long long)ox * a.res_px_stride + n;
        } else {
            ro = (long long)m * a.ldr + n;
        }
        float rr[8];
        load8(res + ro, rr);
#pragma unroll
        for (int j = 0; j < 8; ++j) v[j] += rr[j];
    }
    if (a.relu) {
#pragma unroll
        for (int j = 0; j < 8; ++j) v[j] = fmaxf(v[j], 0.f);
    }
    TO* __restrict__ out = (TO*)a.out;
    TO* __restrict__ out2 = (TO*)a.out2;
    const long long oo = (long long)m * a.ldo + n;
    if (out) {
        if (full) store8(out + oo, v);
        else store_tail(out + oo, v, a.cout - n);
    }
    if (out2) {
        float s2[8], b2[8], u[8];
        load8(a.scale2 + n, s2); load8(a.shift2 + n, b2);
#pragma unroll
        for (int j = 0; j < 8; ++j) {
            const float vr = stored_value<TO>(v[j]);
            u[j] = fmaxf(fmaf(vr, s2[j], b2[j]), 0.f);
        }
        if (full) store8(out2 + oo, u);
        else store_tail(out2 + oo, u, a.cout - n);
    }
}

extern "C" size_t hmmr_conv_splitk_workspace_bytes(int m, int cout, int split_k) {
    if (split_k <= 1 || m <= 0) return 0;
    return (size_t)split_k * (size_t)m * (size_t)((cout + 127) / 128 * 128) * sizeof(float);
}

static int ilog2_exact(int v) {
    int l = 0;
    while ((1 << l) < v) ++l;
    return ((1 << l) == v) ? l : -1;
}

int hmmr_conv3x3_stream(const hmmr_conv_desc_t* d, hipStream_t stream);
int hmmr_conv1x1_stream(const hmmr_conv_desc_t* d, hipStream_t stream);

extern "C" int hmmr_conv_gemm(const hmmr_conv_desc_t* d, void* stream) {
    HMMR_REQUIRE(d && d->in && d->w && (d->out || d->out2), "hmmr_conv_gemm: null operand");
    const int esz = d->in_dtype == HMMR_BF16 ? 2 : 4;
    const int eps = d->in_dtype == HMMR_F16X3 ? 8 : 16 / esz;
    const int cl2 = ilog2_exact(d->cin);
    HMMR_REQUIRE(cl2 >= 0 && d->cin % eps == 0, "hmmr_conv_gemm: cin=%d must be a power of two >= %d", d->cin, eps);
    const int K = d->kh * d->kw * d->cin + (d->in2 ? d->cin2 : 0);
    HMMR_REQUIRE(d->kh * d->kw <= 32, "hmmr_conv_gemm: at most 32 filter taps");
    const int bke = 128 / esz;
    HMMR_REQUIRE(K % bke == 0, "hmmr_conv_gemm: K=%d must be a multiple of %d", K, bke);
    HMMR_REQUIRE(d->out_dtype != HMMR_F16X3 || d->cout % 8 == 0,
                 "hmmr_conv_gemm: a split (f16x3) output needs cout %% 8 == 0 (rows are whole hi/lo groups)");
    HMMR_REQUIRE(d->ldo % 8 == 0, "hmmr_conv_gemm: ldo=%d must be a multiple of 8", d->ldo);
    const bool px_ok = d->in_px_stride % eps == 0 ||
                       (d->kw == 1 && d->px == 0 && (d->in_px_stride * d->sx) % eps == 0);
    HMMR_REQUIRE(px_ok && d->in_row_stride % eps == 0 && d->in_img_stride % eps == 0,
                 "hmmr_conv_gemm: input strides must keep 16-byte alignment");
    HMMR_REQUIRE(!d->res || d->res_strided || d->ldr % 8 == 0, "hmmr_conv_gemm: ldr must be a multiple of 8");
    HMMR_REQUIRE(!d->res || d->cout % 8 == 0 || (!d->res_strided && d->ldr >= (d->cout + 7) / 8 * 8),
                 "hmmr_conv_gemm: residual rows must be readable up to cout rounded up to 8");
    HMMR_REQUIRE(!d->out2 || (d->scale2 && d->shift2), "hmmr_conv_gemm: out2 needs scale2/shift2");
    HMMR_REQUIRE(!d->pro_scale == !d->pro_shift, "hmmr_conv_gemm: pro_scale and pro_shift go together");
    HMMR_REQUIRE(!d->out_b || (d->out && !d->out2 && !d->res && d->split_k <= 1 && d->n_split > 0 && d->n_split < d->cout &&
                               d->n_split % 8 == 0 && d->ldo_b % 8 == 0 && d->ldo_b >= d->cout - d->n_split),
                 "hmmr_conv_gemm: bad column split (out_b needs out, n_split %% 8 == 0, no out2 / res / split_k)");
    HMMR_REQUIRE(!d->pro_scale || !d->res, "hmmr_conv_gemm: a fused pre-activation (pro_*) cannot be combined with a residual");
    HMMR_REQUIRE(!d->pro_scale || (d->py == 0 && d->px == 0 && d->kh == 1 && d->kw == 1),
                 "hmmr_conv_gemm: the fused pre-activation is for un-padded 1x1 gathers (padding must stay zero)");
    char why[256];
    if (const hmmr_conv_tile_info_t* t = conv_tiles::row(d->tile); t && t->family == HMMR_TILE_GENERIC)
        HMMR_REQUIRE(!conv_tiles::fit(d->tile, conv_tiles::Problem{0, 0, 0, d->cout, -1, 0, 0}, why, sizeof why), "hmmr_conv_gemm: %s", why);
    HMMR_REQUIRE(!d->in2 || (d->kh == 1 && d->kw == 1 && d->py == 0 && d->px == 0 && d->sy == 1 && d->sx == 1 && !d->pro_scale &&
                             d->split_k <= 1 && d->cin2 > 0 && d->cin % bke == 0 && d->cin2 % bke == 0 &&
                             d->in_px_stride == d->cin && d->in_row_stride == d->win * d->cin &&
                             d->in_img_stride == (int64_t)d->hin * d->win * d->cin && d->ho == d->hin && d->wo == d->win),
                 "hmmr_conv_gemm: a second operand source (in2) needs a dense 1x1 stride-1 un-padded GEMM, cin and cin2 "
                 "multiples of the 128-byte K step, no pro_scale, no split_k");
    ConvArgs a;
    a.in = d->in; a.w = d->w; a.scale = d->scale; a.shift = d->shift; a.res = d->res;
    a.out = d->out; a.out2 = d->out2; a.scale2 = d->scale2; a.shift2 = d->shift2;
    a.pro_scale = d->pro_scale; a.pro_shift = d->pro_shift;
    a.out_b = d->out_b; a.ldo_b = d->ldo_b; a.n_split = d->n_split; a.relu_b = d->relu_b;
    a.M = d->n_img * d->ho * d->wo; a.K = K; a.cout = d->cout; a.ldo = d->ldo; a.ldr = d->ldr;
    a.Wo = d->wo; a.HoWo = d->ho * d->wo; a.Hin = d->hin; a.Win = d->win;
    a.in_img_stride = d->in_img_stride; a.in_row_stride = d->in_row_stride; a.in_px_stride = d->in_px_stride;
    a.cin_log2 = cl2; a.KH = d->kh; a.KW = d->kw; a.SY = d->sy; a.SX = d->sx; a.PY = d->py; a.PX = d->px;
    a.res_strided = d->res_strided; a.res_img_stride = d->res_img_stride;
    a.res_row_stride = d->res_row_stride; a.res_px_stride = d->res_px_stride;
    a.relu = d->relu; a.tiles_n = 0; a.n_tiles = 0;
    a.kt_per_slice = 0; a.out_slice_stride = 0; a.probe = 0;
    a.in2 = d->in2; a.cin2 = d->in2 ? d->cin2 : 0; a.kt_split = d->cin / bke;
    a.batch = d->batch > 1 ? d->batch : 1;
    a.bz_in = d->batch_in_bytes; a.bz_w = d->batch_w_bytes; a.bz_out = d->batch_out_bytes;
    a.bz_res = d->batch_res_bytes; a.bz_scale = d->batch_scale_bytes; a.bz_shift = d->batch_shift_bytes;
    HMMR_REQUIRE(a.batch == 1 || (a.batch <= 64 && !d->k_order && !d->out_b && !d->in2 && !d->pro_scale &&
                                  ((d->batch_in_bytes | d->batch_w_bytes | d->batch_out_bytes | d->batch_res_bytes | d->batch_scale_bytes | d->batch_shift_bytes) & 15) == 0),
                 "hmmr_conv_gemm: a grouped launch (batch > 1) takes up to 64 problems, strides that are multiples of 16 bytes, "
                 "and no k_order / out_b / in2 / pro_scale");
#ifdef HMMR_GEMM_PROBE
    a.probe = hmmr_debug_state()->gemm_probe;
#endif
    if (a.M <= 0) return 0;
    hipStream_t s = (hipStream_t)stream;
    if (d->k_order == 2 && d->kh == 1 && d->kw == 1) return hmmr_conv1x1_stream(d, s);
    if (d->k_order) {
        HMMR_REQUIRE((d->k_order == 1 || d->k_order == 2) && d->kh == 3 && d->kw == 3 && d->sy == 1 && d->sx == 1 && d->py == 1 && d->px == 1 &&
                     d->ho == d->hin && d->wo == d->win && d->in_px_stride == d->cin && d->in_row_stride == d->win * d->cin &&
                     d->in_img_stride == (int64_t)d->hin * d->win * d->cin && (d->cin * esz) % 128 == 0 &&
                     !d->res && !d->out2 && !d->out_b && !d->pro_scale && !d->in2 && d->split_k <= 1 && d->out && d->cout % 8 == 0,
                     "hmmr_conv_gemm: k_order 1 is for 3x3 / stride 1 / pad 1 convolutions over a dense NHWC tensor with "
                     "cin a multiple of the 128-byte K step and a scale/shift/relu epilogue (no res, out2, out_b, pro_scale, in2, split_k)");
        if (d->k_order == 2) return hmmr_conv3x3_stream(d, s);
        const bool px3 = d->in_dtype == HMMR_F16X3 && d->out_dtype == HMMR_F16X3, pbf = d->in_dtype == HMMR_BF16 && d->out_dtype == HMMR_BF16;
        HMMR_REQUIRE(px3 || pbf, "hmmr_conv_gemm: k_order 1 is built for split (f16x3) and bf16 tensors");
        const int ptile = d->tile ? d->tile : conv_tiles::choose_patch();
        HMMR_REQUIRE(!conv_tiles::fit(ptile, conv_tiles::Problem{1, 0, 0, d->cout, d->in_dtype, 0, 0}, why, sizeof why), "hmmr_conv_gemm: %s", why);
        if (pbf) return launch_patch_tiled<bf16_t, bf16_t>(a, ptile, s);
        return launch_patch_tiled<bsplit_t, bsplit_t>(a, ptile, s);
    }
    const bool in16 = d->in_dtype == HMMR_BF16, in32 = d->in_dtype == HMMR_F32, inx3 = d->in_dtype == HMMR_F16X3;
    const bool out16 = d->out_dtype == HMMR_BF16, out32 = d->out_dtype == HMMR_F32, outx3 = d->out_dtype == HMMR_F16X3;
    HMMR_REQUIRE((in16 || in32 || inx3) && (out16 || out32 || outx3), "hmmr_conv_gemm: unsupported dtypes %d -> %d", d->in_dtype, d->out_dtype);
    const int nk = K / bke;
    int slices = d->split_k > 1 ? d->split_k : 1;
    if (slices > nk) slices = nk;
    slices = (nk + ((nk + slices - 1) / slices) - 1) / ((nk + slices - 1) / slices);
    if (slices > 1) {
        const int ldw = (d->cout + 127) / 128 * 128;
        const long long plane = (long long)a.M * ldw;
        HMMR_REQUIRE(d->ws && d->ws_bytes >= a.batch * hmmr_conv_splitk_workspace_bytes(a.M, d->cout, slices),
                     "hmmr_conv_gemm: split-K workspace missing or too small (a grouped launch needs batch x the planes)");
        ConvArgs p = a;
        p.bz_out = (long long)slices * plane * (long long)sizeof(float);
        p.scale = p.shift = nullptr; p.res = nullptr; p.out2 = nullptr; p.scale2 = p.shift2 = nullptr;
        p.relu = 0; p.out = d->ws; p.ldo = ldw; p.out_slice_stride = plane;
        const int rc = in16 ? launch_typed<bf16_t, float>(p, d->tile, slices, s)
                     : inx3 ? launch_typed<bsplit_t, float>(p, d->tile, slices, s)
                            : launch_typed<float, float>(p, d->tile, slices, s);
        if (rc) return rc;
        const long long nvec = (long long)a.M * ((a.cout + 7) / 8);
        const unsigned grid = (unsigned)((nvec + 255) / 256);
        const dim3 rgrid(grid, a.batch);
        if (out16) hipLaunchKernelGGL(splitk_reduce_kernel<bf16_t>, rgrid, dim3(256), 0, s, a, (const float*)d->ws, slices, ldw, plane);
        else if (outx3) hipLaunchKernelGGL(splitk_reduce_kernel<bsplit_t>, rgrid, dim3(256), 0, s, a, (const float*)d->ws, slices, ldw, plane);
        else hipLaunchKernelGGL(splitk_reduce_kernel<float>, rgrid, dim3(256), 0, s, a, (const float*)d->ws, slices, ldw, plane);
        HMMR_CHECK_HIP(hipGetLastError());
        return 0;
    }
    if (in16 && out16) return launch_typed<bf16_t, bf16_t>(a, d->tile, 1, s);
    if (in16 && out32) return launch_typed<bf16_t, float>(a, d->tile, 1, s);
    if (in32 && out32) return launch_typed<float, float>(a, d->tile, 1, s);
    if (in32 && out16) return launch_typed<float, bf16_t>(a, d->tile, 1, s);
    if (inx3 && outx3) return launch_typed<bsplit_t, bsplit_t>(a, d->tile, 1, s);
    if (inx3 && out32) return launch_typed<bsplit_t, float>(a, d->tile, 1, s);
    if (in32 && outx3) return launch_typed<float, bsplit_t>(a, d->tile, 1, s);
    hmmr_set_error("hmmr_conv_gemm: unsupported dtypes %d -> %d", d->in_dtype, d->out_dtype);
    return -1;
}
```

### human_dynamics_amd/csrc/tail_sched.h

```cpp
#pragma once
#include "common.h"
#include "hmmr_hip.h"

static constexpr int TAIL_C = 2048;
static constexpr float GN_EPS = 1e-6f;
static constexpr int GN_GROUPS = 32;
static constexpr int TEMPORAL_SPLIT_K_MAX = 5;
static inline int temporal_split_k(int dtype) { return dtype == HMMR_F16X3 ? 5 : 4; }
static constexpr int HAL_SPLIT_K = 4;

__device__ __forceinline__ float block_sum_256(float v, float* red) {
#pragma unroll
    for (int o = 32; o > 0; o >>= 1) v += __shfl_xor(v, o);
    __syncthreads();
    if ((threadIdx.x & 63) == 0) red[threadIdx.x >> 6] = v;
    __syncthreads();
    return red[0] + red[1] + red[2] + red[3];
}

static inline hmmr_conv_desc_t temporal_conv_desc(const void* in, int in_dtype, const hmmr_layer_t& l, const float* res, float* out, int b, int t,
                                                  void* sk, size_t skbytes) {
    constexpr int C = TAIL_C;
    hmmr_conv_desc_t d = {};
    d.in = in; d.w = l.w; d.scale = l.scale; d.shift = l.shift; d.tile = l.tile;
    d.out = out; d.in_dtype = in_dtype; d.out_dtype = HMMR_F32;
    d.n_img = b; d.hin = t; d.win = 1; d.cin = C;
    d.in_img_stride = (int64_t)t * C; d.in_row_stride = C; d.in_px_stride = C;
    d.kh = 3; d.kw = 1; d.sy = d.sx = 1; d.py = 1; d.px = 0; d.ho = t; d.wo = 1; d.cout = C; d.ldo = C;
    d.split_k = temporal_split_k(in_dtype); d.ws = sk; d.ws_bytes = skbytes;
    if (res) { d.res = res; d.ldr = C; }
    return d;
}

static inline hmmr_conv_desc_t fc_desc(const void* in, int in_dtype, int m, int k, const hmmr_layer_t& l, void* out, int out_dtype, int cout,
                                       int ldo, int split_k = 0, void* sk = nullptr, size_t skbytes = 0) {
    hmmr_conv_desc_t d = {};
    d.in = in; d.w = l.w; d.scale = l.scale; d.shift = l.shift; d.out = out;
    d.in_dtype = in_dtype; d.out_dtype = out_dtype;
    d.n_img = m; d.hin = d.win = 1; d.cin = k;
    d.in_img_stride = k; d.in_row_stride = k; d.in_px_stride = k;
    d.kh = d.kw = 1; d.sy = d.sx = 1; d.ho = d.wo = 1; d.cout = cout; d.ldo = ldo;
    if (split_k) { d.split_k = split_k; d.ws = sk; d.ws_bytes = skbytes; }
    return d;
}
static inline hmmr_conv_desc_t hal_fc_desc(const void* in, int in_dtype, const hmmr_layer_t& l, void* out, int out_dtype, int m, int relu,
                                           const float* res, void* sk, size_t skbytes) {
    hmmr_conv_desc_t d = fc_desc(in, in_dtype, m, TAIL_C, l, out, out_dtype, TAIL_C, TAIL_C, HAL_SPLIT_K, sk, skbytes);
    d.relu = relu; d.res = res; d.ldr = TAIL_C;
    return d;
}

static constexpr int LDT = 128;
static constexpr int IEF_SPLIT_K = 4;

__global__ void ief_finalize_kernel(const float* __restrict__ theta, const float* __restrict__ bsrc, int ld_b, int mode,
                                    float* __restrict__ out, int m, long long th_stride);
```

### human_dynamics_amd/csrc/temporal.hip

```cpp
#include "common.h"
#include "hmmr_hip.h"
#include "tail_sched.h"
#include "workspace.h"

template <typename TO>
__global__ __launch_bounds__(256) void groupnorm_relu_kernel(const float* __restrict__ x,
                                                             const float* __restrict__ gamma,
                                                             const float* __restrict__ beta,
                                                             TO* __restrict__ out, int t, int c, int groups) {
    __shared__ float red[4];
    const int cpg = c / groups;
    const int b = blockIdx.x / groups, g = blockIdx.x % groups;
    const int cnt = t * cpg;
    const float* xb = x + (long long)b * t * c + g * cpg;
    float s = 0.f;
    for (int i = threadIdx.x; i < cnt; i += 256) s += xb[(i / cpg) * c + (i % cpg)];
    const float mean = block_sum_256(s, red) / (float)cnt;
    float q = 0.f;
    for (int i = threadIdx.x; i < cnt; i += 256) {
        const float d = xb[(i / cpg) * c + (i % cpg)] - mean;
        q += d * d;
    }
    const float var = block_sum_256(q, red) / (float)cnt;
    const float rstd = rsqrtf(var + GN_EPS);
    TO* ob = out + (long long)b * t * c + g * cpg;
    const int v8 = cpg / 8;
    for (int i = threadIdx.x; i < t * v8; i += 256) {
        const int tt = i / v8, j = (i % v8) * 8;
        float xv[8], gm[8], bt[8], o[8];
        load8(xb + tt * c + j, xv); load8(gamma + g * cpg + j, gm); load8(beta + g * cpg + j, bt);
#pragma unroll
        for (int e = 0; e < 8; ++e) {
            const float gain = rstd * gm[e];
            o[e] = fmaxf((xv[e] - mean) * gain + bt[e], 0.f);
        }
        store8(ob + tt * c + j, o);
    }
}

extern "C" int hmmr_groupnorm_relu(const float* x, const float* gamma, const float* beta, int b, int t,
                                   int c, int groups, void* out, int out_dtype, void* stream) {
    HMMR_REQUIRE(x && gamma && beta && out, "hmmr_groupnorm_relu: null argument");
    HMMR_REQUIRE(b > 0 && t > 0 && groups > 0 && c % groups == 0 && (c / groups) % 8 == 0,
                 "hmmr_groupnorm_relu: bad shape (channels per group must be a multiple of 8)");
    hipStream_t s = (hipStream_t)stream;
    if (out_dtype == HMMR_BF16)
        hipLaunchKernelGGL(groupnorm_relu_kernel<bf16_t>, dim3(b * groups), dim3(256), 0, s, x, gamma, beta,
                           (bf16_t*)out, t, c, groups);
    else if (out_dtype == HMMR_F32)
        hipLaunchKernelGGL(groupnorm_relu_kernel<float>, dim3(b * groups), dim3(256), 0, s, x, gamma, beta,
                           (float*)out, t, c, groups);
    else if (out_dtype == HMMR_F16X3)
        hipLaunchKernelGGL(groupnorm_relu_kernel<bsplit_t>, dim3(b * groups), dim3(256), 0, s, x, gamma, beta,
                           (bsplit_t*)out, t, c, groups);
    else { hmmr_set_error("hmmr_groupnorm_relu: bad dtype %d", out_dtype); return -1; }
    HMMR_CHECK_HIP(hipGetLastError());
    return 0;
}

struct MovieBufs { size_t buf[4], sk, skbytes, total; };
static MovieBufs movie_layout(size_t m, int dtype, int nop, int nf32) {
    MovieBufs l = {}; WsCarver c;
    for (int i = 0; i < nop + nf32; ++i) l.buf[i] = c.take(m * 2048 * (i < nop && dtype == HMMR_BF16 ? 2 : 4));
    l.skbytes = hmmr_conv_splitk_workspace_bytes((int)m, 2048, TEMPORAL_SPLIT_K_MAX);
    l.sk = c.take(l.skbytes);
    l.total = c.total();
    return l;
}
static MovieBufs temporal_layout(int b, int t, int dtype) { return movie_layout((size_t)b * t, dtype, 1, 3); }
static MovieBufs hallucinator_layout(int m, int dtype) { return movie_layout((size_t)m, dtype, 3, 0); }

extern "C" size_t hmmr_temporal_workspace_bytes(int b, int t, int dtype) {
    return b > 0 && t > 0 ? temporal_layout(b, t, dtype).total : 0;
}

extern "C" int hmmr_temporal_fwd(const hmmr_temporal_weights_t* w, const float* phi, int b, int t,
                                 float* strips, void* ws, size_t ws_bytes, void* stream) {
    HMMR_REQUIRE(w && phi && strips && ws, "hmmr_temporal_fwd: null argument");
    HMMR_REQUIRE(b > 0 && t > 0, "hmmr_temporal_fwd: bad shape");
    HMMR_REQUIRE(w->num_blocks >= 1 && w->num_blocks <= HMMR_MAX_TEMPORAL_BLOCKS, "hmmr_temporal_fwd: bad num_blocks");
    const MovieBufs L = temporal_layout(b, t, w->dtype);
    HMMR_REQUIRE(ws_bytes >= L.total, "hmmr_temporal_fwd: workspace too small");
    constexpr int C = TAIL_C;
    char* base = (char*)ws;
    void* h = base + L.buf[0];
    float *h1 = (float*)(base + L.buf[1]), *net[2] = {(float*)(base + L.buf[2]), (float*)(base + L.buf[3])};
    const float* cur = phi;
    for (int i = 0; i < w->num_blocks; ++i) {
        const hmmr_temporal_block_t& B = w->block[i];
        float* dst = (i == w->num_blocks - 1) ? strips : net[i & 1];
        if (hmmr_groupnorm_relu(cur, B.gn1_gamma, B.gn1_beta, b, t, C, GN_GROUPS, h, w->dtype, stream)) return -2;
        hmmr_conv_desc_t d = temporal_conv_desc(h, w->dtype, B.conv1, nullptr, h1, b, t, base + L.sk, L.skbytes);
        if (hmmr_conv_gemm(&d, stream)) return -2;
        if (hmmr_groupnorm_relu(h1, B.gn2_gamma, B.gn2_beta, b, t, C, GN_GROUPS, h, w->dtype, stream)) return -2;
        d = temporal_conv_desc(h, w->dtype, B.conv2, cur, dst, b, t, base + L.sk, L.skbytes);
        if (hmmr_conv_gemm(&d, stream)) return -2;
        cur = dst;
    }
    return 0;
}

extern "C" size_t hmmr_hallucinator_workspace_bytes(int m, int dtype) {
    return m > 0 ? hallucinator_layout(m, dtype).total : 0;
}

template <typename TO>
__global__ void hal_cast_kernel(const float* __restrict__ in, TO* __restrict__ out, long long n8) {
    const long long i = (long long)blockIdx.x * blockDim.x + threadIdx.x;
    if (i >= n8) return;
    float v[8];
    load8(in + i * 8, v);
    store8(out + i * 8, v);
}

extern "C" int hmmr_hallucinator_fwd(const hmmr_hallucinator_weights_t* w, const float* phi, int m,
                                     float* out, void* ws, size_t ws_bytes, void* stream) {
    HMMR_REQUIRE(w && phi && out && ws, "hmmr_hallucinator_fwd: null argument");
    HMMR_REQUIRE(m > 0, "hmmr_hallucinator_fwd: m must be positive");
    const MovieBufs L = hallucinator_layout(m, w->dtype);
    HMMR_REQUIRE(ws_bytes >= L.total, "hmmr_hallucinator_fwd: workspace too small");
    constexpr int C = TAIL_C;
    char* base = (char*)ws;
    void *x = base + L.buf[0], *h1 = base + L.buf[1], *h2 = base + L.buf[2];
    hipStream_t s = (hipStream_t)stream;
    const void* xin = phi;
    if (w->dtype != HMMR_F32) {
        const long long n8 = (long long)m * C / 8;
        if (w->dtype == HMMR_BF16)
            hipLaunchKernelGGL(hal_cast_kernel<bf16_t>, dim3((unsigned)((n8 + 255) / 256)), dim3(256), 0, s, phi, (bf16_t*)x, n8);
        else
            hipLaunchKernelGGL(hal_cast_kernel<bsplit_t>, dim3((unsigned)((n8 + 255) / 256)), dim3(256), 0, s, phi, (bsplit_t*)x, n8);
        HMMR_CHECK_HIP(hipGetLastError());
        xin = x;
    }
    auto fc = [&](const void* in, const hmmr_layer_t& l, void* o, int odt, int relu, const float* res) {
        hmmr_conv_desc_t d = hal_fc_desc(in, w->dtype, l, o, odt, m, relu, res, base + L.sk, L.skbytes);
        return hmmr_conv_gemm(&d, s);
    };
    if (fc(xin, w->fc1, h1, w->dtype, 1, nullptr)) return -2;
    if (fc(h1, w->fc2, h2, w->dtype, 1, nullptr)) return -2;
    if (fc(h2, w->fc3, out, HMMR_F32, 0, phi)) return -2;
    return 0;
}
```

### human_dynamics_amd/engine.py

```python
from __future__ import annotations

import ctypes as C
import os
import threading
import time

import numpy as np
import torch

from . import _lib as L
from . import assets, devflags, packing

DTYPES = {"f32": L.HMMR_F32, "fp32": L.HMMR_F32, "float32": L.HMMR_F32,
          "bf16": L.HMMR_BF16, "bfloat16": L.HMMR_BF16,
          "f16x3": L.HMMR_F16X3, "split": L.HMMR_F16X3}
DTYPE_NAMES = {L.HMMR_F32: "f32", L.HMMR_BF16: "bf16", L.HMMR_F16X3: "f16x3"}
DEFAULT_DTYPE = "f16x3"
TILE_TABLES = os.path.join(os.path.dirname(os.path.abspath(__file__)), "tile_tables.json")


def set_debug(stem_route=0, stem_no_conv1=0, gemm_probe=0, smpl_blend_mfma=0, ief_no_group=0, pair_min_pixels=0, pair_two_tile_min=0, pair_form=0):
    d = L.Debug()
    d.stem_route, d.stem_no_conv1, d.gemm_probe = int(stem_route), int(stem_no_conv1), int(gemm_probe)
    d.smpl_blend_mfma, d.ief_no_group, d.pair_min_pixels = int(smpl_blend_mfma), int(ief_no_group), int(pair_min_pixels)
    d.pair_two_tile_min, d.pair_form = int(pair_two_tile_min), int(pair_form)
    L.load().hmmr_set_debug(C.byref(d))


def _debug_from_env():
    e = devflags.get("STEM")
    c1 = devflags.get("STEM_C1")
    probe = int(devflags.get("GEMM_PROBE") or 0)
    if e or c1 == "0" or probe or _debug_from_env.was_set:
        set_debug(stem_route={"u": 1, "f": 2}.get(e[:1], 0), stem_no_conv1=int(c1 == "0"), gemm_probe=probe)
        _debug_from_env.was_set = bool(e or c1 == "0" or probe)


_debug_from_env.was_set = False


def _dt(d):
    if isinstance(d, str):
        if d == "bf16x3":
            import warnings
            warnings.warn("dtype 'bf16x3' is now 'f16x3' (split operands with fp16 halves since round 3)", DeprecationWarning, stacklevel=3)
            d = "f16x3"
        if d not in DTYPES:
            raise ValueError("unknown operand mode %r: use one of %s" % (d, ", ".join(sorted(set(DTYPES)))))
        return DTYPES[d]
    return int(d)


def _packer_choices(fold_sc=None, fuse_tail=None, patch_3x3=None, unit_pair=None, b1_stream=None, b1_unit=None, stem_conv1=True,
                    stream_1x1=None):
    def _flag_choice(name):
        v = devflags.get(name)
        return {"0": False, "1": True}.get(v, v)

    def pick(arg, flag):
        return flag if arg is None else arg
    fsc, fold = _flag_choice("FUSE_SC"), _flag_choice("FOLD_SC")
    return dict(fuse_preact_blocks=tuple(b for b in devflags.get("FUSE_PREACT").split(",") if b),
                fuse_tail=pick(fuse_tail, _flag_choice("FUSE_TAIL")),
                fuse_sc=fsc if isinstance(fsc, bool) else "all",
                fuse_preact_first=_flag_choice("PREACT_FIRST") is not False,
                fold_sc=pick(fold_sc, fold if isinstance(fold, bool) else None),
                patch_3x3=pick(patch_3x3, int(devflags.get("PATCH_3X3"))),
                unit_pair=pick(unit_pair, _flag_choice("UNIT_PAIR")),
                b1_stream=pick(b1_stream, _flag_choice("B1_STREAM") is True),
                b1_unit=pick(b1_unit, _flag_choice("B1_UNIT") is True),
                stem_conv1=stem_conv1,
                stream_1x1=pick(stream_1x1, _flag_choice("STREAM_1X1") is True))


class _Workspace(object):

    def __init__(self, device):
        self.device, self.buf = device, None

    def get(self, nbytes):
        if self.buf is None or self.buf.numel() < nbytes:
            self.buf = torch.empty(int(nbytes), dtype=torch.uint8, device=self.device)
        return self.buf


class HmmrEngine(object):

    def __init__(self, weights, smpl, dtype=DEFAULT_DTYPE, device="cuda:0", num_conv_layers=3,
                 delta_t_values=(-5, 5), joint_type="cocoplus", resnet_chunk=0,
                 temporal_dtype=None, ief_dtype=None, autotune=True, fold_sc=None, fuse_tail=None, patch_3x3=None,
                 unit_pair=None, b1_stream=None, b1_unit=None, stem_conv1=True, stream_1x1=None):
        self.lib = L.load()
        _debug_from_env()
        if not torch.cuda.is_available():
            raise L.HmmrError("HmmrEngine needs a HIP device (torch.cuda.is_available() is False)")
        self.device = torch.device(device)
        torch.cuda.set_device(self.device)
        self.dtype = _dt(dtype)
        self.temporal_dtype = self.dtype if temporal_dtype is None else _dt(temporal_dtype)
        self.ief_dtype = self.dtype if ief_dtype is None else _dt(ief_dtype)
        self.resnet_chunk = int(devflags.get("RESNET_CHUNK") or resnet_chunk)
        self.store = packing.DeviceStore(self.device)
        self.num_conv_layers = num_conv_layers
        self.delta_keys = sorted(int(d) for d in delta_t_values)
        w = weights if weights is not None else {}
        for name, v in w.items():
            a_ = np.asarray(v)
            if a_.dtype.kind == "f" and not np.isfinite(a_).all():
                raise ValueError("variable %r holds %d non-finite value(s)" % (name, int((~np.isfinite(a_)).sum())))
        choices = _packer_choices(fold_sc=fold_sc, fuse_tail=fuse_tail, patch_3x3=patch_3x3, unit_pair=unit_pair, b1_stream=b1_stream,
                                  b1_unit=b1_unit, stem_conv1=stem_conv1, stream_1x1=stream_1x1)
        self.rw = packing.pack_resnet(w, self.dtype, self.store, **choices) if "resnet_v2_50/conv1/weights" in w else None
        self.tw = (packing.pack_temporal(w, self.temporal_dtype, self.store, num_conv_layers)
                   if assets.temporal_scopes(0)[1] + "/weights" in w else None)
        self.hw = packing.pack_hallucinator(w, self.temporal_dtype, self.store)
        if "single_view_ief/3D_module/fc1/weights" in w and "mean_param" in w:
            self.iw, self.reg_keys = packing.pack_ief(w, self.ief_dtype, self.store, self.delta_keys)
        else:
            self.iw, self.reg_keys = None, [0]
        self._ief_source = {k: v for k, v in w.items() if k.startswith("single_view_ief") or k == "mean_param"} if self.iw is not None else None
        self._ief_bank = None
        self._movie_source = {k: v for k, v in w.items() if k.startswith(("AZ_FC_block", "fc2_res/"))} if self.tw is not None else None
        self._movie_bank = None
        all_f32 = (self.dtype, self.temporal_dtype, self.ief_dtype) == (L.HMMR_F32,) * 3
        self.sc = packing.pack_smpl(smpl, self.store, joint_type, split=not all_f32) if smpl is not None else None
        self._smpl_source, self.joint_type, self._gc = smpl, joint_type, None
        self.num_kps = self.sc.num_kps if self.sc is not None else assets.NUM_KPS
        self.num_verts = self.sc.num_verts if self.sc is not None else assets.NUM_VERTS
        self._ws = {k: _Workspace(self.device) for k in ("resnet", "temporal", "ief", "smpl", "hal")}
        at = devflags.get("AUTOTUNE")
        self.autotune = False if (not autotune or at == "0") else ("force" if (autotune == "force" or at == "force") else True)
        self._tiles, self._shipped = {}, set()
        self.tune_log = []
        self._tile_cache = devflags.get("TILE_CACHE")
        sources = []
        if self.autotune != "force" and devflags.get("TILE_TABLE") != "0" and os.path.exists(TILE_TABLES):
            sources.append((TILE_TABLES, True))
        if self._tile_cache and os.path.exists(self._tile_cache):
            sources.append((self._tile_cache, False))
        for path, shipped in sources:
            import json
            for key, tab in json.load(open(path)).items():
                if key.startswith("_"):
                    continue
                dt, nt = key.split(":")
                if int(dt) == self.dtype:
                    self._tiles[int(nt)] = {(int(k.split(":")[0]), k.split(":")[1]): int(v) for k, v in tab.items()}
                    if shipped:
                        self._shipped.add(int(nt))
        self.resnet_streams = int(devflags.get("RESNET_STREAMS"))
        self._side_streams = []

    @staticmethod
    def _need(packed, names):
        if packed is None:
            raise L.HmmrError("the loaded weights have no %s variables: this stage was not packed" % names)

    def _stream(self):
        return torch.cuda.current_stream(self.device).cuda_stream

    _carried_flags = {}

    def run_flags(self, clear=False):
        key = (self.device.type, self.device.index)
        v = self._device_flags(clear) | HmmrEngine._carried_flags.get(key, 0)
        if clear:
            HmmrEngine._carried_flags.pop(key, None)
        return v

    def _device_flags(self, clear):
        torch.cuda.synchronize(self.device)
        with torch.cuda.device(self.device):
            v = C.c_uint(0)
            L.check(self.lib.hmmr_run_flags(C.byref(v), int(bool(clear))), "hmmr_run_flags")
        return int(v.value)

    def flag_scope(self):
        return _FlagScope(self)

    def to_device(self, a, dtype=torch.float32):
        if isinstance(a, torch.Tensor):
            return a.to(self.device, dtype).contiguous()
        return torch.from_numpy(np.ascontiguousarray(a)).to(self.device).to(dtype).contiguous()

    _TUNE_TILES = tuple(int(t) for t in devflags.get("TUNE_TILES").split(","))
    _TUNE_MIN_FRAMES = 32
    _SPLIT_MIN_FRAMES = 176

    def _resnet_layers(self):
        out, slot = [], 3
        for u in range(L.RESNET_UNITS):
            names = (["shortcut"] if self.rw.unit[u].shortcut.w else []) + ["conv1", "conv2", "conv3"]
            for nm in names:
                out.append((slot, u, nm))
                slot += 1
        return out

    def _layer_of(self, u, nm):
        U = self.rw.unit[u]
        if nm == "conv3" and U.c3sc.w:
            return U.c3sc
        return getattr(U, nm)

    @staticmethod
    def _tile_for(lay, cand, cout, dtype=None, nm="conv2"):
        return L.load().hmmr_conv_tile_for(lay.k_order, int(nm != "conv2"), int(nm == "conv3"), cout, -1 if dtype is None else dtype, cand)

    def _layer_cout(self, u, nm):
        U = self.rw.unit[u]
        if nm == "shortcut" and U.sc_c1.w:
            return U.depth + U.base
        return U.base if nm in ("conv1", "conv2") else U.depth

    def _set_tiles(self, table):
        for (u, nm), t in table.items():
            self._layer_of(u, nm).tile = self._tile_for(self._layer_of(u, nm), int(t), self._layer_cout(u, nm), self.dtype, nm)

    def _needs_tuning(self, nt):
        if not self.autotune or nt < self._TUNE_MIN_FRAMES or nt in self._tiles or torch.cuda.is_current_stream_capturing():
            return False
        if len(self.tune_log) >= 8:
            return False
        if self.autotune == "force":
            return True
        return not any(max(k, nt) <= 1.3 * min(k, nt) for k in self._tiles)

    def _tune_resnet(self, images, n, n_zero, ws_key="resnet", reps=3):
        layers = self._resnet_layers()
        t_start = time.perf_counter()
        nt = n + n_zero
        nbytes = self.lib.hmmr_resnet50_workspace_bytes(nt, self.dtype)
        ws = self._ws.setdefault(ws_key, _Workspace(self.device)).get(nbytes)
        phi = torch.empty((nt, 2048), dtype=torch.float32, device=self.device)
        src = images.data_ptr() if n else None
        best = {}
        for cand in (0,) + self._TUNE_TILES:
            for slot, u, nm in layers:
                lay = self._layer_of(u, nm)
                lay.tile = self._tile_for(lay, cand, self._layer_cout(u, nm), self.dtype, nm)
            t = None
            for rep in range(reps):
                pm = (C.c_float * L.RESNET_PROF_SLOTS)()
                L.check(self.lib.hmmr_resnet50_fwd(C.byref(self.rw), src, n, n_zero, phi.data_ptr(), ws.data_ptr(),
                                                   nbytes, self._stream(), pm), "hmmr_resnet50_fwd")
                cur = np.frombuffer(pm, dtype=np.float32).copy()
                t = cur if (t is None or rep == 0) else np.minimum(t, cur)
            for slot, u, nm in layers:
                tile = self._layer_of(u, nm).tile
                if (u, nm) not in best or t[slot] < best[(u, nm)][0] * 0.98:
                    best[(u, nm)] = (float(t[slot]), tile)
        table = {k: v[1] for k, v in best.items()}
        self.tune_log.append((nt, round((time.perf_counter() - t_start) * 1e3, 1)))
        if self._tile_cache:
            import json
            old = json.load(open(self._tile_cache)) if os.path.exists(self._tile_cache) else {}
            old["%d:%d" % (self.dtype, nt)] = {"%d:%s" % k: v for k, v in table.items()}
            json.dump(old, open(self._tile_cache, "w"))
        return table

    def _resnet_pass(self, images, n, n_zero, phi, ws_key, prof=False, tune=True):
        nt = n + n_zero
        table = None
        if tune and nt >= self._TUNE_MIN_FRAMES:
            if self._needs_tuning(nt):
                self._tiles[nt] = self._tune_resnet(images, n, n_zero, ws_key)
            if self._tiles:
                table = self._tiles[min(self._tiles, key=lambda k: abs(k - nt))]
        if table is not None:
            self._set_tiles(table)
        elif self._tiles:
            self._set_tiles({k: 0 for k in next(iter(self._tiles.values()))})
        nbytes = self.lib.hmmr_resnet50_workspace_bytes(nt, self.dtype)
        ws = self._ws.setdefault(ws_key, _Workspace(self.device)).get(nbytes)
        pm = (C.c_float * L.RESNET_PROF_SLOTS)() if prof else None
        L.check(self.lib.hmmr_resnet50_fwd(C.byref(self.rw), images.data_ptr() if n else None, n, n_zero,
                                           phi.data_ptr(), ws.data_ptr(), nbytes, self._stream(), pm),
                "hmmr_resnet50_fwd")
        return np.frombuffer(pm, dtype=np.float32).astype(np.float64) if prof else None

    def resnet_cuts(self, n, parts=None):
        parts = self.resnet_streams if parts is None else int(parts)
        if parts < 2 or n < self._SPLIT_MIN_FRAMES or self.resnet_chunk > 0:
            return [0, n]
        return [(i * n) // parts for i in range(parts + 1)]

    def resnet(self, images, prof=False, n_zero=0, out=None, ws_key="resnet", parts=None):
        self._need(self.rw, "resnet_v2_50/*")
        images = self.to_device(images)
        n = images.shape[0]
        assert n == 0 or tuple(images.shape[1:]) == (224, 224, 3), images.shape
        nt = n + n_zero
        if out is not None:
            assert out.is_cuda and out.dtype == torch.float32 and out.shape == (nt, 2048) and out.is_contiguous()
        phi = out if out is not None else torch.empty((nt, 2048), dtype=torch.float32, device=self.device)
        if self.resnet_chunk > 0:
            chunk, i = self.resnet_chunk, 0
            prof_tot = np.zeros(L.RESNET_PROF_SLOTS, np.float64) if prof else None
            while i < nt:
                c_real = max(0, min(chunk, n - i))
                c_zero = min(chunk - c_real, nt - i - c_real) if i + c_real >= n else 0
                pm = self._resnet_pass(images[i:i + c_real], c_real, c_zero, phi[i:i + c_real + c_zero], "resnet",
                                       prof, tune=False)
                if prof:
                    prof_tot += pm
                i += c_real + c_zero
            return (phi, prof_tot) if prof else phi
        parts = self.resnet_streams if parts is None else int(parts)
        if prof or parts < 2 or n < self._SPLIT_MIN_FRAMES or torch.cuda.is_current_stream_capturing():
            pm = self._resnet_pass(images, n, n_zero, phi, ws_key, prof)
            return (phi, pm) if prof else phi
        cur = torch.cuda.current_stream(self.device)
        self.side_stream(parts - 1)
        cuts = [(i * n) // parts for i in range(parts + 1)]
        if self.autotune:
            for i in range(parts):
                ni, nz = cuts[i + 1] - cuts[i], (n_zero if i == parts - 1 else 0)
                if self._needs_tuning(ni + nz):
                    self._tiles[ni + nz] = self._tune_resnet(images[cuts[i]:cuts[i + 1]], ni, nz, "resnet%d" % i)
        for i in range(parts):
            side = self._side_streams[i]
            side.wait_stream(cur)
            with torch.cuda.stream(side):
                nz = n_zero if i == parts - 1 else 0
                self._resnet_pass(images[cuts[i]:cuts[i + 1]], cuts[i + 1] - cuts[i], nz,
                                  phi[cuts[i]:cuts[i + 1] + nz], "resnet%d" % i)
        for i in range(parts):
            cur.wait_stream(self._side_streams[i])
        return phi

    def side_stream(self, i):
        while len(self._side_streams) <= i:
            self._side_streams.append(torch.cuda.Stream(device=self.device, priority=int(devflags.get("RESNET_PRIORITY"))))
        return self._side_streams[i]

    def _out(self, out, shape, dtype=torch.float32):
        if out is None:
            return torch.empty(shape, dtype=dtype, device=self.device)
        assert out.is_cuda and out.device == self.device and out.dtype == dtype and out.is_contiguous(), "out: a contiguous device tensor"
        assert out.dim() == len(shape) and out.shape[0] >= shape[0] and tuple(out.shape[1:]) == tuple(shape[1:]), (tuple(out.shape), shape)
        return out[:shape[0]]

    def temporal(self, phi, out=None):
        self._need(self.tw, "AZ_FC_block*")
        phi = self.to_device(phi)
        b, t, c = phi.shape
        assert c == 2048
        out = self._out(out, (b, t, c))
        nbytes = self.lib.hmmr_temporal_workspace_bytes(b, t, self.temporal_dtype)
        ws = self._ws["temporal"].get(nbytes)
        L.check(self.lib.hmmr_temporal_fwd(C.byref(self.tw), phi.data_ptr(), b, t, out.data_ptr(),
                                           ws.data_ptr(), nbytes, self._stream()), "hmmr_temporal_fwd")
        return out

    def hallucinate(self, phi, out=None):
        if self.hw is None:
            raise L.HmmrError("the loaded weights have no fc2_res/* variables (pred_mode 'hal')")
        phi = self.to_device(phi)
        flat = phi.reshape(-1, 2048)
        m = flat.shape[0]
        out = self._out(out, (m, 2048))
        nbytes = self.lib.hmmr_hallucinator_workspace_bytes(m, self.temporal_dtype)
        ws = self._ws["hal"].get(nbytes)
        L.check(self.lib.hmmr_hallucinator_fwd(C.byref(self.hw), flat.data_ptr(), m, out.data_ptr(),
                                               ws.data_ptr(), nbytes, self._stream()), "hmmr_hallucinator_fwd")
        return out.reshape(phi.shape)

    def ief(self, strips, omega_start=None, use_delta_from_pred=True, out=None):
        self._need(self.iw, "single_view_ief*/3D_module/* and mean_param")
        strips = self.to_device(strips)
        m = strips.shape[0]
        R = self.iw.num_regressors
        out = self._out(out, (R * m * 85,)).view(R, m, 85)
        nbytes = self.lib.hmmr_ief_workspace_bytes(m, R, self.ief_dtype)
        ws = self._ws["ief"].get(nbytes)
        start = None
        if omega_start is not None:
            start = self.to_device(omega_start).reshape(-1, 85)
            if start.shape[0] == 1:
                start = start.expand(m, 85).contiguous()
            assert start.shape == (m, 85), start.shape
        iw = L.IefWeights.from_buffer_copy(self.iw)
        iw.delta_from_start = int(not use_delta_from_pred)
        L.check(self.lib.hmmr_ief_fwd_from(C.byref(iw), strips.data_ptr(), L.ptr(start), m, out.data_ptr(),
                                           ws.data_ptr(), nbytes, self._stream()), "hmmr_ief_fwd_from")
        return out

    @property
    def use_optcam(self):
        return self.iw is None or not self.iw.no_optcam

    def ief_bank(self):
        self._need(self.iw, "single_view_ief*/3D_module/* and mean_param")
        if self._ief_bank is None:
            from .ief_bank import IefBank
            self._ief_bank = IefBank(self._ief_source, [k for k in self.reg_keys if k != 0], self.device, num_stages=self.iw.num_stages)
        return self._ief_bank

    def _ief_train_args(self, strips, omega_start, keep, keep_prob, use_delta_from_pred):
        bank = self.ief_bank()
        strips = self.to_device(strips).reshape(-1, 2048)
        m, R, S = strips.shape[0], bank.iw.num_regressors, bank.iw.num_stages
        start = None
        if omega_start is not None:
            start = self.to_device(omega_start).reshape(-1, 85)
            if start.shape[0] == 1:
                start = start.expand(m, 85).contiguous()
            if start.shape != (m, 85):
                raise ValueError("omega_start: expected [%d, 85], got %s" % (m, tuple(start.shape)))
        scale = 1.0
        if keep is not None:
            keep = (keep if isinstance(keep, torch.Tensor) else torch.tensor(np.asarray(keep))).to(self.device, torch.uint8).contiguous()
            if tuple(keep.shape) != (R, S, 2, m, 1024):
                raise ValueError("keep: expected a uint8 mask of shape %s, got %s" % ((R, S, 2, m, 1024), tuple(keep.shape)))
            if keep_prob is None or not (0.0 < float(keep_prob) <= 1.0):
                raise ValueError("keep is given: keep_prob must lie in (0, 1], got %r" % (keep_prob,))
            scale = 1.0 / float(keep_prob)
        iw = L.IefWeights.from_buffer_copy(bank.iw)
        iw.delta_from_start = int(not use_delta_from_pred)
        nbytes = self.lib.hmmr_ief_bwd_workspace_bytes(m, R, S)
        ws = self._ws.setdefault("ief_grad", _Workspace(self.device)).get(nbytes)
        return bank, iw, strips, start, keep, scale, m, R, ws, nbytes

    def ief_train(self, strips, omega_start=None, keep=None, keep_prob=None, use_delta_from_pred=True):
        bank, iw, strips, start, keep, scale, m, R, ws, nbytes = self._ief_train_args(strips, omega_start, keep, keep_prob, use_delta_from_pred)
        out = torch.empty((R, m, 85), dtype=torch.float32, device=self.device)
        L.check(self.lib.hmmr_ief_fwd_train(C.byref(iw), strips.data_ptr(), L.ptr(start), L.ptr(keep), scale, m, out.data_ptr(),
                                            ws.data_ptr(), nbytes, self._stream()), "hmmr_ief_fwd_train")
        return out

    def ief_backward(self, strips, d_omegas, omega_start=None, keep=None, keep_prob=None, use_delta_from_pred=True,
                     want_strips=True, want_start=None, want_weights=True):
        from .ief_bank import NAMES
        bank, iw, strips, start, keep, scale, m, R, ws, nbytes = self._ief_train_args(strips, omega_start, keep, keep_prob, use_delta_from_pred)
        d_omegas = self.to_device(d_omegas).reshape(R, m, 85).contiguous()
        want_start = (start is not None) if want_start is None else bool(want_start)
        d = L.IefBwdDesc()
        d.strips, d.omega_start, d.keep, d.keep_scale, d.m, d.d_omegas = strips.data_ptr(), L.ptr(start), L.ptr(keep), scale, m, d_omegas.data_ptr()
        d_strips = torch.empty((m, 2048), dtype=torch.float32, device=self.device) if want_strips else None
        d_start = torch.empty((m, 85), dtype=torch.float32, device=self.device) if want_start else None
        d.d_strips, d.d_omega_start = L.ptr(d_strips), L.ptr(d_start)
        grads = []
        for r in range(R):
            names = NAMES if want_weights is True else (() if not want_weights else tuple(want_weights[r] or ()))
            g = {n: (torch.empty(bank.params[r][n].shape, dtype=torch.float32, device=self.device) if n in names else None) for n in NAMES}
            for n in NAMES:
                setattr(d.reg[r], "d_" + n, L.ptr(g[n]))
            grads.append(g)
        L.check(self.lib.hmmr_ief_bwd(C.byref(iw), C.byref(d), ws.data_ptr(), nbytes, self._stream()), "hmmr_ief_bwd")
        return d_strips, d_start, grads

    def movie_bank(self):
        self._need(self.tw, "AZ_FC_block*")
        if self._movie_bank is None:
            from .movie_bank import MovieBank
            self._movie_bank = MovieBank(self._movie_source, self.device, num_conv_layers=self.num_conv_layers)
        return self._movie_bank

    def _hal_bank(self):
        bank = self.movie_bank()
        if bank.hw is None:
            raise L.HmmrError("the loaded weights have no fc2_res/* variables (pred_mode 'hal')")
        return bank

    def _movie_ws(self, nbytes):
        return self._ws.setdefault("movie_grad", _Workspace(self.device)).get(nbytes)

    def temporal_train(self, phi):
        bank = self.movie_bank()
        phi = self.to_device(phi)
        b, t, c = phi.shape
        assert c == 2048
        out = torch.empty((b, t, c), dtype=torch.float32, device=self.device)
        nbytes = self.lib.hmmr_temporal_workspace_bytes(b, t, L.HMMR_F32)
        ws = self._movie_ws(nbytes)
        L.check(self.lib.hmmr_temporal_fwd(C.byref(bank.tw), phi.data_ptr(), b, t, out.data_ptr(), ws.data_ptr(), nbytes, self._stream()),
                "hmmr_temporal_fwd")
        return out

    def hallucinate_train(self, phi):
        bank = self._hal_bank()
        phi = self.to_device(phi)
        flat = phi.reshape(-1, 2048)
        m = flat.shape[0]
        out = torch.empty((m, 2048), dtype=torch.float32, device=self.device)
        nbytes = self.lib.hmmr_hallucinator_workspace_bytes(m, L.HMMR_F32)
        ws = self._movie_ws(nbytes)
        L.check(self.lib.hmmr_hallucinator_fwd(C.byref(bank.hw), flat.data_ptr(), m, out.data_ptr(), ws.data_ptr(), nbytes, self._stream()),
                "hmmr_hallucinator_fwd")
        return out.reshape(phi.shape)

    def temporal_backward(self, phi, d_strips, want_phi=True, want_weights=True):
        from .movie_bank import BLOCK_NAMES
        bank = self.movie_bank()
        phi = self.to_device(phi)
        b, t, c = phi.shape
        assert c == 2048
        d_strips = self.to_device(d_strips).reshape(b, t, c)
        d = L.TemporalBwdDesc()
        d.phi, d.b, d.t, d.d_strips = phi.data_ptr(), b, t, d_strips.data_ptr()
        d_phi = torch.empty((b, t, c), dtype=torch.float32, device=self.device) if want_phi else None
        d.d_phi = L.ptr(d_phi)
        grads = []
        for i in range(bank.num_blocks):
            names = BLOCK_NAMES if want_weights is True else (() if not want_weights else tuple(want_weights[i] or ()))
            g = {n: (torch.empty(bank.blocks[i][n].shape, dtype=torch.float32, device=self.device) if n in names else None) for n in BLOCK_NAMES}
            for n in BLOCK_NAMES:
                setattr(d.block[i], "d_" + n, L.ptr(g[n]))
            grads.append(g)
        nbytes = self.lib.hmmr_temporal_bwd_workspace_bytes(b, t, bank.num_blocks)
        ws = self._movie_ws(nbytes)
        L.check(self.lib.hmmr_temporal_bwd(C.byref(bank.tw), C.byref(d), ws.data_ptr(), nbytes, self._stream()), "hmmr_temporal_bwd")
        return d_phi, grads

    def hallucinate_backward(self, phi, d_out, want_phi=True, want_weights=True):
        from .movie_bank import HAL_NAMES
        bank = self._hal_bank()
        phi = self.to_device(phi)
        flat = phi.reshape(-1, 2048)
        m = flat.shape[0]
        d_out = self.to_device(d_out).reshape(m, 2048)
        names = HAL_NAMES if want_weights is True else (() if not want_weights else tuple(want_weights))
        d = L.HallucinatorBwdDesc()
        d.phi, d.m, d.d_out = flat.data_ptr(), m, d_out.data_ptr()
        d_phi = torch.empty((m, 2048), dtype=torch.float32, device=self.device) if want_phi else None
        d.d_phi = L.ptr(d_phi)
        g = {n: (torch.empty(bank.hal[n].shape, dtype=torch.float32, device=self.device) if n in names else None) for n in HAL_NAMES}
        for n in HAL_NAMES:
            setattr(d, "d_" + n, L.ptr(g[n]))
        nbytes = self.lib.hmmr_hallucinator_bwd_workspace_bytes(m)
        ws = self._movie_ws(nbytes)
        L.check(self.lib.hmmr_hallucinator_bwd(C.byref(bank.hw), C.byref(d), ws.data_ptr(), nbytes, self._stream()), "hmmr_hallucinator_bwd")
        return (d_phi.reshape(phi.shape) if d_phi is not None else None), g

    def smpl(self, theta, beta, cams=None, want_rs=True):
        def prep(x, width):
            if not (isinstance(x, torch.Tensor) and x.is_cuda and x.dtype == torch.float32
                    and x.dim() == 2 and x.stride(1) == 1 and x.shape[1] == width):
                x = self.to_device(x).reshape(-1, width)
            return x
        theta, beta = prep(theta, 72), prep(beta, 10)
        m = theta.shape[0]
        cams = prep(cams, 3) if cams is not None else None
        V, K = self.num_verts, self.num_kps
        verts = torch.empty((m, V, 3), dtype=torch.float32, device=self.device)
        joints = torch.empty((m, K, 3), dtype=torch.float32, device=self.device)
        kps = torch.empty((m, K, 2), dtype=torch.float32, device=self.device) if cams is not None else None
        rs = torch.empty((m, 24, 3, 3), dtype=torch.float32, device=self.device) if want_rs else None
        nbytes = self.lib.hmmr_smpl_workspace_bytes(m)
        ws = self._ws["smpl"].get(nbytes)
        L.check(self.lib.hmmr_smpl_fwd(C.byref(self.sc), theta.data_ptr(), theta.stride(0),
                                       beta.data_ptr(), beta.stride(0),
                                       L.ptr(cams), cams.stride(0) if cams is not None else 0, m,
                                       verts.data_ptr(), joints.data_ptr(), L.ptr(kps), L.ptr(rs),
                                       ws.data_ptr(), nbytes, self._stream()), "hmmr_smpl_fwd")
        return verts, joints, kps, rs

    def smpl_backward(self, theta, beta, cams=None, joints=None, d_verts=None, d_joints=None, d_kps=None, d_rs=None, want_cams=None):
        def prep(x, width):
            if not (isinstance(x, torch.Tensor) and x.is_cuda and x.dtype == torch.float32
                    and x.dim() == 2 and x.stride(1) == 1 and x.shape[1] == width):
                x = self.to_device(x).reshape(-1, width)
            return x
        theta, beta = prep(theta, 72), prep(beta, 10)
        m = theta.shape[0]
        cams = prep(cams, 3) if cams is not None else None
        V, K = self.num_verts, self.num_kps

        def dense(x, shape):
            if x is None:
                return None
            x = self.to_device(x)
            if tuple(x.shape) != (m,) + shape:
                raise ValueError("expected a gradient of shape %s, got %s" % ((m,) + shape, tuple(x.shape)))
            return x
        joints, d_verts, d_joints = dense(joints, (K, 3)), dense(d_verts, (V, 3)), dense(d_joints, (K, 3))
        d_kps, d_rs = dense(d_kps, (K, 2)), dense(d_rs, (24, 3, 3))
        if self._gc is None:
            self._gc = packing.pack_smpl_grad(self._smpl_source, self.store, self.joint_type)
        want_cams = (cams is not None) if want_cams is None else (bool(want_cams) and cams is not None)
        d_theta = torch.empty((m, 72), dtype=torch.float32, device=self.device)
        d_beta = torch.empty((m, 10), dtype=torch.float32, device=self.device)
        d_cams = torch.empty((m, 3), dtype=torch.float32, device=self.device) if want_cams else None
        nbytes = self.lib.hmmr_smpl_bwd_workspace_bytes(C.byref(self.sc), m)
        ws = self._ws.setdefault("smpl_bwd", _Workspace(self.device)).get(nbytes)
        L.check(self.lib.hmmr_smpl_bwd(C.byref(self.sc), C.byref(self._gc), theta.data_ptr(), theta.stride(0), beta.data_ptr(), beta.stride(0),
                                       L.ptr(cams), cams.stride(0) if cams is not None else 0, L.ptr(joints), m,
                                       L.ptr(d_verts), L.ptr(d_joints), L.ptr(d_kps), L.ptr(d_rs),
                                       d_theta.data_ptr(), d_beta.data_ptr(), L.ptr(d_cams),
                                       ws.data_ptr(), nbytes, self._stream()), "hmmr_smpl_bwd")
        return d_theta, d_beta, d_cams

    def _loss_desc(self, B, T, K, flags, weights, delta_t, gt):
        d = L.SeqLossDesc()
        d.B, d.T, d.K, d.delta_t, d.flags = int(B), int(T), int(K), int(delta_t), int(flags)
        w = list(weights) if weights is not None else [1.0] * 5
        if len(w) not in (5, 6):
            raise ValueError("weights: (e_kp, e_joints, e_smpl, e_const, e_shape), got %d values" % len(w))
        d.weights = (C.c_float * 6)(*([float(v) for v in w] + [0.0] * (6 - len(w))))
        N = d.B * d.T
        shapes = {"kps": (N, d.K, 3), "joints": (N, 14, 3), "rs": (N, 24, 3, 3), "shapes": (d.B, 10), "has_gt3d_smpl": (d.B,),
                  "has_gt3d_joints": (d.B,)}
        keep = {}
        for k, shp in shapes.items():
            x = (gt or {}).get(k)
            if x is None:
                continue
            x = self.to_device(x).reshape(shp)
            keep[k] = x
            setattr(d, {"kps": "kps_gt", "joints": "joints_gt", "rs": "rs_gt", "shapes": "shapes_gt"}.get(k, k), x.data_ptr())
        return d, keep

    def seq_losses(self, B, T, flags, gt, kps_pred=None, joints_pred=None, rs_pred=None, beta_pred=None, weights=None, delta_t=0,
                   want_grads=True, want_best_cam=False, check=False, K=None):
        N, K = int(B) * int(T), int(self.num_kps if K is None else K)
        d, keep = self._loss_desc(B, T, K, flags, weights, delta_t, gt)

        def dense(x, shape):
            if x is None:
                return None
            x = self.to_device(x)
            if tuple(x.shape) != shape:
                raise ValueError("expected a prediction of shape %s, got %s" % (shape, tuple(x.shape)))
            return x
        kps_pred, joints_pred, rs_pred = dense(kps_pred, (N, K, 2)), dense(joints_pred, (N, K, 3)), dense(rs_pred, (N, 24, 3, 3))
        if beta_pred is not None:
            if not (isinstance(beta_pred, torch.Tensor) and beta_pred.is_cuda and beta_pred.dtype == torch.float32 and beta_pred.dim() == 2
                    and beta_pred.stride(1) == 1 and beta_pred.shape[1] == 10):
                beta_pred = self.to_device(beta_pred).reshape(-1, 10)
            if beta_pred.shape[0] != N:
                raise ValueError("expected %d rows of beta, got %d" % (N, beta_pred.shape[0]))
            d.beta_pred, d.ld_beta = beta_pred.data_ptr(), beta_pred.stride(0)
        d.kps_pred, d.joints_pred, d.rs_pred = L.ptr(kps_pred), L.ptr(joints_pred), L.ptr(rs_pred)
        names = ("d_kps", "d_joints", "d_rs", "d_beta")
        wanted = set(names if want_grads is True else (() if not want_grads else want_grads))
        out = {"losses": torch.empty(8, dtype=torch.float32, device=self.device),
               "status": torch.zeros(1, dtype=torch.int32, device=self.device)}
        for k, shp in zip(names, ((N, K, 2), (N, K, 3), (N, 24, 3, 3), (N, 10))):
            out[k] = torch.empty(shp, dtype=torch.float32, device=self.device) if k in wanted else None
            setattr(d, k, L.ptr(out[k]))
        out["best_cam"] = torch.full((N, 3), float("nan"), dtype=torch.float32, device=self.device) if want_best_cam else None
        d.losses, d.status, d.best_cam = out["losses"].data_ptr(), out["status"].data_ptr(), L.ptr(out["best_cam"])
        nbytes = self.lib.hmmr_seq_losses_workspace_bytes(d.B, d.T)
        ws = self._ws.setdefault("losses", _Workspace(self.device)).get(nbytes)
        d.ws, d.ws_bytes = ws.data_ptr(), nbytes
        L.check(self.lib.hmmr_seq_losses(C.byref(d), self._stream()), "hmmr_seq_losses")
        if check and int(out["status"].item()) & L.LOSS_NO_VISIBLE:
            raise L.HmmrError("hmmr_seq_losses: a frame of the slice has no visible keypoint under KP_OPTCAM (the loss is not finite)")
        return out

    def omega_loss_grad(self, omega, B, T, flags, gt, weights=None, delta_t=0, use_optcam=False, want_best_cam=False):
        shape = tuple(omega.shape) if isinstance(omega, torch.Tensor) else None
        om = self.to_device(omega).reshape(-1, 85)
        N = int(B) * int(T)
        if om.shape[0] != N:
# ... 546 lines not shown
```

### human_dynamics_amd/evaluation/tester.py

```python
from __future__ import annotations

import os

import numpy as np
import torch

from .. import _lib as L
from .. import assets
from ..engine import DEFAULT_DTYPE, HmmrEngine
from ..models import (batch_pred_omega, get_hallucinator_model, get_image_encoder,
                      get_temporal_encoder)
from ..omega import OmegasPred
from ..tf_smpl.batch_smpl import SMPL, load_smpl_constants

OUTPUT_KEYS = ("cams", "joints", "kps", "poses", "shapes", "verts", "omegas")


def mean_theta_from_file(path):
    if not os.path.exists(path):
        raise FileNotFoundError("{} doesnt exist..".format(path))
    if str(path).endswith((".h5", ".hdf5")):
        from .. import hdf5_lite
        v = hdf5_lite.load(path)
        if "pose" not in v or "shape" not in v:
            raise ValueError("%s has no 'pose' / 'shape' datasets (found %s)" % (path, sorted(v)))
    else:
        v = np.load(path)
    if isinstance(v, np.ndarray):
        if v.size != 85:
            raise ValueError("%s holds %d values, the mean theta has 85" % (path, v.size))
        return np.asarray(v, np.float32).reshape(1, 85)
    pose = np.array(v["pose"], np.float64).reshape(72)
    pose[:3] = 0.0
    pose[0] = np.pi
    shape = np.asarray(v["shape"], np.float64).reshape(10)
    return np.hstack(([0.9, 0.0, 0.0], pose, shape))[None].astype(np.float32)


def load_weights(load_path, resnet_path="", mean_param_path=""):
    from .. import tf_checkpoint

    def one(path):
        if str(path).startswith("synthetic"):
            seed = int(str(path).split(":")[1]) if ":" in str(path) else 0
            return assets.make_synthetic_weights(seed)
        if os.path.exists(path) and str(path).endswith(".npz"):
            return {k: v for k, v in np.load(path).items()}
        if tf_checkpoint.is_checkpoint(path):
            return tf_checkpoint.read_checkpoint(path)
        raise FileNotFoundError("{} doesnt exist..".format(path))
    w = dict(one(load_path))
    if resnet_path:
        for k, v in one(resnet_path).items():
            if "resnet" in k:
                w[k] = v
    if mean_param_path:
        mean = mean_theta_from_file(mean_param_path)
        w.setdefault("mean_param", mean)
    return w


def window_plan(n_frames, batch_size, sequence_length, fov):
    margin = (fov - 1) // 2
    g = sequence_length - 2 * margin
    count = int(np.ceil(n_frames / float(g * batch_size)))
    num_fill = count * batch_size * g + sequence_length - n_frames
    return margin, g, count, num_fill


class Tester(object):
    MAX_DEVICE_FRAMES = 1024
    MAX_TAIL_WINDOWS = 128

    def __init__(self, config, pretrained_resnet_path="", sequence_length=None,
                 weights=None, smpl=None, dtype=None, device=None, dedup=True, use_containers=False):
        self.config = config
        self.load_path = config.load_path
        if not config.load_path and weights is None:
            raise Exception("[!] You need to specify `load_path` to load a pretrained model")
        self.batch_size = config.batch_size
        self.sequence_length = sequence_length if sequence_length else config.sequence_length
        self.pred_mode = config.pred_mode
        self.num_conv_layers = config.num_conv_layers
        self.fov = self.num_conv_layers * 4 + 1
        self.delta_t_values = [int(dt) for dt in config.delta_t_values]
        self.img_size = 224
        self.num_output = 85
        self.smpl_model_path = config.smpl_model_path
        self.dedup = dedup
        self.use_containers = use_containers
        if self.pred_mode not in ("pred", "hal"):
            raise Exception("Pred mode {} not recognized".format(self.pred_mode))

        if weights is None:
            weights = load_weights(config.load_path, pretrained_resnet_path,
                                   getattr(config, "mean_param_path", "") or self._default_mean_path(config))
        if smpl is None:
            smpl = load_smpl_constants(self.smpl_model_path, checkpoint_vars=weights)
        dtype = dtype or getattr(config, "dtype", None) or "auto"
        device = device or getattr(config, "device", "cuda:0")
        kw = dict(num_conv_layers=self.num_conv_layers, delta_t_values=self.delta_t_values,
                  resnet_chunk=getattr(config, "resnet_chunk", 0))
        self.precision = None
        if dtype == "auto":
            from .. import precision
            self.engine, self.precision = precision.choose_engine(weights, smpl, device, pred_mode=self.pred_mode, **kw)
        else:
            self.engine = HmmrEngine(weights, smpl, dtype=dtype, device=device, **kw)
        if self.precision is None:
            from .. import precision
            self.precision = {"operands": precision.describe(self.engine), "rungs": []}
        self.precision["saturated"] = False
        self._rebuild = (weights, smpl, device, kw)
        self.smpl = SMPL(smpl, engine=self.engine)
        if self.engine.num_kps != config.num_kps:
            raise ValueError("config.num_kps=%d but the SMPL regressor has %d keypoints"
                             % (config.num_kps, self.engine.num_kps))
        self.f_hal = get_hallucinator_model()
        self.f_image_enc = get_image_encoder()
        self.f_temporal_enc = get_temporal_encoder()
        if "mean_param" not in weights:
            raise KeyError("the loaded weights have no 'mean_param' variable (the 1 x 85 mean theta both published "
                           "checkpoints carry) and no neutral_smpl_meanwjoints.h5 sits next to the SMPL model; add the variable to "
                           "the .npz, load a checkpoint that was saved by the reference, or set config.mean_param_path to the .h5 "
                           "(or an .npy / .npz of its pose / shape fields)")
        self.theta_mean = np.asarray(weights["mean_param"], np.float32).reshape(1, 85)
        self._streamer = None

    @staticmethod
    def _default_mean_path(config):
        d = os.path.dirname(str(getattr(config, "smpl_model_path", "") or ""))
        for ext in (".h5", ".npz", ".npy"):
            p = os.path.join(d, "neutral_smpl_meanwjoints" + ext)
            if d and os.path.exists(p):
                return p
        return ""

    def make_omega_pred(self, registry, use_optcam=False, batch_size=None):
        return OmegasPred(config=self.config, smpl_engine=self.engine, use_optcam=use_optcam,
                          vis_max_batch=batch_size or self.batch_size, batch_size=batch_size,
                          is_training=False, registry=registry)

    def _regress(self, movie_strips, B, T):
        registry = []
        omegas_pred = {0: self.make_omega_pred(registry, use_optcam=False, batch_size=B)}
        for dt in self.delta_t_values:
            omegas_pred[dt] = self.make_omega_pred(registry, use_optcam=True, batch_size=B)
        omegas_raw, deltas_pred = batch_pred_omega(
            input_features=movie_strips, batch_size=B, sequence_length=T,
            num_output=self.num_output, is_training=False, omega_mean=None,
            scope="single_view_ief", engine=self.engine,
            predict_delta_keys=omegas_pred.keys(), use_optcam=True, use_delta_from_pred=True)
        omegas_pred[0].append_batched(omegas_raw)
        for k in deltas_pred.keys():
            omegas_pred[k].append_batched(deltas_pred[k])
            omegas_pred[k].set_cams(omegas_pred[0].get_cams())
        OmegasPred.compute_all_smpl(registry)
        return omegas_pred

    @staticmethod
    def make_fetch_dict(omegas, suffix=""):
        return {
            "cams" + suffix: omegas.get_cams(),
            "joints" + suffix: omegas.get_joints(),
            "kps" + suffix: omegas.get_kps(),
            "poses" + suffix: omegas.get_poses_rot(),
            "shapes" + suffix: omegas.get_shapes(),
            "verts" + suffix: omegas.get_verts(),
            "omegas" + suffix: omegas.get_raw(),
        }

    def _fetch(self, omegas_pred, to_numpy=True):
        fetch = self.make_fetch_dict(omegas_pred[0])
        deltas = {}
        for delta_t, omega_delta in sorted(omegas_pred.items()):
            if delta_t == 0:
                continue
            for k, v in self.make_fetch_dict(omega_delta, suffix="_delta").items():
                deltas.setdefault(k, []).append(v)
        for k, v in deltas.items():
            fetch[k] = torch.stack(v, dim=2)
        if not to_numpy:
            return fetch
        torch.cuda.synchronize(self.engine.device)
        return {k: v.float().cpu().numpy() for k, v in fetch.items()}

    def record_layout(self):
        from ..dist import record_layout
        K = self.engine.num_kps
        V = self.engine.num_verts
        fields = (("cams", (3,)), ("joints", (K, 3)), ("kps", (K, 2)), ("poses", (24, 3, 3)),
                  ("shapes", (10,)), ("verts", (V, 3)), ("omegas", (85,)))
        return record_layout(len(self.delta_t_values), fields)

    def predict_records(self, strips, out=None):
        return self.records_from_omegas(self.engine.ief(strips), out)

    def records_from_omegas(self, om, out=None):
        eng = self.engine
        n = om.shape[1]
        layout, rec_len = self.record_layout()
        off = {k: (o, sz) for k, shp, o, sz in layout}
        if out is None:
            out = torch.empty((n, rec_len), dtype=torch.float32, device=eng.device)
        if n == 0:
            return out
        rows = []
        for r, key in enumerate(eng.reg_keys):
            if key == 0:
                rows.append([off[k][0] for k in OUTPUT_KEYS])
            else:
                d = r - 1
                rows.append([off[k + "_delta"][0] + d * (off[k + "_delta"][1] // len(self.delta_t_values)) for k in OUTPUT_KEYS])
        eng.smpl_records(om.contiguous(), out, rows)
        return out

    def _movie_strips(self, img_feat_full):
        if self.pred_mode == "pred":
            return self.f_temporal_enc(is_training=False, net=img_feat_full,
                                       num_conv_layers=self.num_conv_layers, engine=self.engine)
        return self.f_hal(img_feat_full, engine=self.engine)

    def predict_device(self, images):
        from ..dist import unpack_outputs
        B, T = images.shape[0], images.shape[1]
        I_t = self.engine.to_device(images).reshape(B * T, self.img_size, self.img_size, 3)
        img_feat, _ = self.f_image_enc(I_t, engine=self.engine, is_training=False, reuse=False)
        img_feat_full = img_feat.reshape(B, T, -1)
        movie_strips = self._movie_strips(img_feat_full)
        if self.use_containers:
            return self._fetch(self._regress(movie_strips, B, T), to_numpy=False)
        rec = self.predict_records(movie_strips.reshape(B * T, -1))
        layout, _ = self.record_layout()
        return {k: v.reshape((B, T) + v.shape[1:]) for k, v in unpack_outputs(rec, layout).items()}

    def predict(self, images):
        def run():
            out = self.predict_device(images)
            torch.cuda.synchronize(self.engine.device)
            return {k: v.float().cpu().numpy() for k, v in out.items()}
        return self._guard_saturation(run)

    def _uses_split_operands(self):
        e = self.engine
        return L.HMMR_F16X3 in (e.dtype, e.temporal_dtype, e.ief_dtype) or bool(e.sc is not None and e.sc.dirs_split)

    def _guard_saturation(self, run):
        if not self._uses_split_operands():
            return run()
        with self.engine.flag_scope() as scope:
            out = run()
        if not (scope.flags & L.FLAG_SATURATED):
            return out
        import warnings
        e = self.engine
        stages = [n for n, d in (("ResNet", e.dtype), ("f_movie", e.temporal_dtype), ("IEF", e.ief_dtype)) if d == L.HMMR_F16X3]
        if e.sc is not None and e.sc.dirs_split:
            stages.append("SMPL blend product")
        what = "a NaN reached" if scope.flags & L.FLAG_NAN else "a value left the fp16 range (clamped to +-65504) in"
        warnings.warn("human_dynamics_amd: %s a split-fp16 store (stages with split operands: %s) -- repeating the call with "
                      "fp32 operands and keeping them for this Tester" % (what, ", ".join(stages)), RuntimeWarning, stacklevel=3)
        weights, smpl, device, kw = self._rebuild
        self.engine = HmmrEngine(weights, smpl, dtype="f32", device=device, **kw)
        self.smpl = SMPL(smpl, engine=self.engine)
        self._streamer = None
        self.precision.update(saturated=True, operands="f32", nan=bool(scope.flags & L.FLAG_NAN))
        return run()

    def features(self, frames, chunk=256, n_zero=0):
        if isinstance(frames, torch.Tensor) and frames.is_cuda:
            N, big = len(frames), self.MAX_DEVICE_FRAMES
            if N <= big:
                return self.engine.resnet(frames, n_zero=n_zero)
            phi = torch.empty((N + n_zero, 2048), dtype=torch.float32, device=self.engine.device)
            for i in range(0, N, big):
                last = i + big >= N
                self.engine.resnet(frames[i:i + big], n_zero=n_zero if last else 0,
                                   out=phi[i:min(i + big, N) + (n_zero if last else 0)])
            return phi
        outs = []
        for i in range(0, len(frames), chunk):
            last = i + chunk >= len(frames)
            outs.append(self.engine.resnet(np.asarray(frames[i:i + chunk], np.float32),
                                           n_zero=n_zero if last else 0))
        return torch.cat(outs, dim=0)

    def predict_strips_records(self, windows, n_keep, out=None):
        T = self.sequence_length
        margin = (self.fov - 1) // 2
        strips = self._movie_strips(windows)
        kept = strips[:, margin:T - margin].reshape(-1, strips.shape[-1])[:n_keep]
        return self.predict_records(kept, out)

    def predict_strips_omegas(self, windows, n_keep):
        T = self.sequence_length
        margin = (self.fov - 1) // 2
        strips = self._movie_strips(windows)
        kept = strips[:, margin:T - margin].reshape(-1, strips.shape[-1])[:n_keep]
        return self.engine.ief(kept)

    def predict_strips_device(self, windows, n_keep):
        from ..dist import unpack_outputs
        if n_keep == 0:
            return {}
        layout, _ = self.record_layout()
        return unpack_outputs(self.predict_strips_records(windows, n_keep), layout)

    def predict_windows_device(self, phi, phi_zero):
        B, T = self.batch_size, self.sequence_length
        N = phi.shape[0]
        margin, g, count, num_fill = window_plan(N, B, T, self.fov)
        padded = torch.cat([phi_zero.expand(margin, -1), phi, phi_zero.expand(num_fill, -1)], dim=0)
        idx = (torch.arange(count * B, device=phi.device)[:, None] * g +
               torch.arange(T, device=phi.device)[None, :])
        wmax = self.MAX_TAIL_WINDOWS
        if idx.shape[0] <= wmax or N == 0:
            return self.predict_strips_device(padded[idx], N)
        from ..dist import unpack_outputs
        layout, rec_len = self.record_layout()
        rec = torch.empty((N, rec_len), dtype=torch.float32, device=phi.device)
        for w0 in range(0, idx.shape[0], wmax):
            o0, o1 = w0 * g, min(N, (w0 + wmax) * g)
            if o0 >= N:
                break
            self.predict_strips_records(padded[idx[w0:w0 + wmax]], o1 - o0, out=rec[o0:o1])
        return unpack_outputs(rec, layout)

    def predict_all_images(self, all_images, want=None, stream=True):
        if self._uses_split_operands() and not getattr(self, "_in_guard", False):
            self._in_guard = True
            try:
                return self._guard_saturation(lambda: self.predict_all_images(all_images, want, stream))
            finally:
                self._in_guard = False
        N = len(all_images)
        if not self.dedup:
            return self._predict_all_images_literal(all_images)
        host_input = not (isinstance(all_images, torch.Tensor) and all_images.is_cuda)
        if host_input and stream:
            if self._streamer is None:
                from .streaming import HostStreamer
                self._streamer = HostStreamer(self)
            return self._streamer.run(all_images, want)
        if host_input and getattr(all_images, "dtype", None) == np.uint8:
            raise ValueError("uint8 input goes through the streamed path (stream=True)")
        phi = self.features(all_images, n_zero=1)
        out = self.predict_windows_device(phi[:N], phi[N:])
        torch.cuda.synchronize(self.engine.device)
        return {k: v.float().cpu().numpy() for k, v in out.items() if want is None or k in want}

    def native_model(self):
        import ctypes as C
        eng = self.engine
        eng._need(eng.rw, "resnet_v2_50/*")
        eng._need(eng.iw, "single_view_ief*/3D_module/* and mean_param")
        eng._need(eng.sc, "SMPL")
        model = L.Model()
        model.resnet, model.ief, model.smpl = C.pointer(eng.rw), C.pointer(eng.iw), C.pointer(eng.sc)
        if self.pred_mode == "pred":
            eng._need(eng.tw, "AZ_FC_block*")
            model.temporal = C.pointer(eng.tw)
        else:
            eng._need(eng.hw, "fc2_res/*")
            model.hallucinator = C.pointer(eng.hw)
        model.sequence_length, model.fov = self.sequence_length, self.fov
        return model

    def _native_records(self, frames, who, max_frames, max_windows):
        import ctypes as C
        from ..engine import _Workspace
        eng = self.engine
        model = self.native_model()
        if isinstance(who, np.ndarray):
            name, n, args = "hmmr_predict_tracks", int(who[-1]), (who.ctypes.data_as(C.POINTER(C.c_int32)), len(who) - 1)
        else:
            name, n, args = "hmmr_predict_video", int(who), (int(who),)
        R = eng.iw.num_regressors
        offs, ld_rec = (C.c_int32 * (R * 7))(), C.c_int64(0)
        L.check(eng.lib.hmmr_record_layout(eng.num_kps, eng.num_verts, R, offs, C.byref(ld_rec)), "hmmr_record_layout")
        layout, rec_len = self.record_layout()
        assert rec_len == ld_rec.value, (rec_len, ld_rec.value)
        rec = torch.empty((n, rec_len), dtype=torch.float32, device=eng.device)
        nbytes = getattr(eng.lib, name + "_workspace_bytes")(C.byref(model), *args, max_frames, max_windows)
        if not nbytes:
            L.check(-1, name + "_workspace_bytes")
        ws = eng._ws.setdefault("video", _Workspace(eng.device)).get(nbytes)
        L.check(getattr(eng.lib, name)(C.byref(model), frames.data_ptr() if n else None, *args, rec.data_ptr() if n else None, rec_len, offs,
                                       max_frames, max_windows, ws.data_ptr(), nbytes, eng._stream()), name)
        torch.cuda.synchronize(eng.device)
        return rec, layout

    def predict_all_images_native(self, all_images, want=None, max_frames=MAX_DEVICE_FRAMES, max_windows=MAX_TAIL_WINDOWS):
        from ..dist import unpack_outputs

        def run():
            frames = self.engine.to_device(all_images)
            n = frames.shape[0]
            assert n == 0 or tuple(frames.shape[1:]) == (224, 224, 3), frames.shape
            rec, layout = self._native_records(frames, n, int(max_frames), int(max_windows))
            return {k: v.float().cpu().numpy() for k, v in unpack_outputs(rec, layout).items() if want is None or k in want}
        return self._guard_saturation(run)

    def predict_tracks(self, tracks, want=None, records=False, max_frames=MAX_DEVICE_FRAMES, max_windows=MAX_TAIL_WINDOWS):
        from ..dist import unpack_outputs
        tracks = list(tracks)
        for k, trk in enumerate(tracks):
            if (trk.dtype == torch.uint8) if isinstance(trk, torch.Tensor) else (np.asarray(trk).dtype == np.uint8):
                raise ValueError("track %d: uint8 input goes through the streamed path (predict_videos / predict_all_images, stream=True)" % k)
            if len(trk) and tuple(trk.shape[1:]) != (224, 224, 3):
                raise ValueError("track %d: frames of shape %s, need [N,224,224,3]" % (k, tuple(trk.shape)))

        def run():
            parts = [self.engine.to_device(trk).reshape(-1, 224, 224, 3) for trk in tracks if len(trk)]
            offsets = np.zeros(len(tracks) + 1, np.int32)
            np.cumsum([len(trk) for trk in tracks], out=offsets[1:])
            frames = parts[0] if len(parts) == 1 else torch.cat(parts, dim=0) if parts else None
            rec, layout = self._native_records(frames, offsets, int(max_frames), int(max_windows))
            views = [rec[int(offsets[k]):int(offsets[k + 1])] for k in range(len(tracks))]
            if records:
                return views, layout
            return [{k: v.float().cpu().numpy() for k, v in unpack_outputs(view, layout).items() if want is None or k in want} for view in views]
        return self._guard_saturation(run)

    def predict_videos(self, videos, want=None, batched=False):
        videos = list(videos)
        if batched:
            return self.predict_tracks(videos, want)
        if self._uses_split_operands() and not getattr(self, "_in_guard", False):
            self._in_guard = True
            try:
                return self._guard_saturation(lambda: self.predict_videos(videos, want))
            finally:
                self._in_guard = False
        if not self.dedup or any(isinstance(v, torch.Tensor) and v.is_cuda for v in videos):
            return [self.predict_all_images(v, want) for v in videos]
        if self._streamer is None:
            from .streaming import HostStreamer
            self._streamer = HostStreamer(self)
        return self._streamer.run_many(videos, want)

    def _predict_all_images_literal(self, all_images):
        B, T = self.batch_size, self.sequence_length
        N = len(all_images)
        H = W = self.img_size
        margin, g, count, num_fill = window_plan(N, B, T, self.fov)
        images_padded = np.concatenate((np.zeros((margin, H, W, 3), np.float32),
                                        np.asarray(all_images, np.float32),
                                        np.zeros((num_fill, H, W, 3), np.float32)), axis=0)
        results = {}
        for c in range(count):
            batch = np.stack([images_padded[i * g:i * g + T] for i in range(c * B, (c + 1) * B)])
            for k, v in self.predict(batch).items():
                results.setdefault(k, []).append(v)
        new_results = {}
        for k, v in results.items():
            v = np.array(v)[:, :, margin:-margin]
            new_results[k] = v.reshape((-1,) + v.shape[3:])[:N]
        return new_results
```

### include/hmmr_hip.h

```cpp
#ifndef HMMR_HIP_H
#define HMMR_HIP_H

#include <stddef.h>
#include <stdint.h>

#ifdef __cplusplus
extern "C" {
#endif

#define HMMR_ABI_VERSION 19

enum { HMMR_F32 = 0, HMMR_BF16 = 1, HMMR_F16X3 = 2 };

int hmmr_abi_version(void);
const char* hmmr_last_error(void);

#define HMMR_FLAG_SATURATED 1u
#define HMMR_FLAG_NAN 2u
int hmmr_run_flags(unsigned* flags, int clear);

typedef struct hmmr_debug_s {
    int stem_route;
    int stem_no_conv1;
    int gemm_probe;
    int smpl_blend_mfma;
    int ief_no_group;
    int reserved[3];
    int pair_min_pixels;
    int pair_two_tile_min;
    int pair_form;
} hmmr_debug_t;
void hmmr_set_debug(const hmmr_debug_t* d);
void hmmr_get_debug(hmmr_debug_t* d);

typedef struct {
    unsigned long long unit_pair;
    unsigned long long b1_unit;
    unsigned long long tail_split;
    unsigned long long conv3x3_stream;
    unsigned long long conv1x1_stream;
} hmmr_launch_counts_t;
void hmmr_launch_counts(hmmr_launch_counts_t* out, int clear);
typedef struct {
    unsigned long long fused;
    unsigned long long fused_conv1;
    unsigned long long repack;
    unsigned long long gemm;
    unsigned long long pool;
} hmmr_stem_counts_t;
void hmmr_stem_launch_counts(hmmr_stem_counts_t* out, int clear);

typedef struct {
    const void* in;
    const void* w;
    const float* scale;
    const float* shift;
    const void* res;
    void* out;
    void* out2;
    const float* scale2;
    const float* shift2;
    int in_dtype;
    int out_dtype;
    int n_img, hin, win, cin;
    int64_t in_img_stride;
    int in_row_stride, in_px_stride;
    int kh, kw, sy, sx, py, px;
    int ho, wo;
    int cout;
    int ldo;
    int ldr;
    int res_strided;
    int64_t res_img_stride;
    int res_row_stride, res_px_stride;
    int relu;
    int tile;
    int split_k;
    void* ws;
    size_t ws_bytes;
    const float* pro_scale;
    const float* pro_shift;
    void* out_b;
    int ldo_b, n_split, relu_b;
    const void* in2;
    int cin2;
    int k_order;
    int batch;
    int64_t batch_in_bytes, batch_w_bytes, batch_out_bytes, batch_res_bytes, batch_scale_bytes, batch_shift_bytes;
} hmmr_conv_desc_t;

#define HMMR_CONV_TILE_MAX 63
enum { HMMR_TILE_GENERIC = 0, HMMR_TILE_PATCH = 1, HMMR_TILE_STREAM_3X3 = 2, HMMR_TILE_STREAM_1X1 = 3 };
typedef struct {
    int tile, family;
    int fm, fn, wgm, wgn;
    int pixels, channels;
    int row_blocks;
    int depth;
    int occupancy;
    int wmax;
    int split_only;
    int conv3_form;
    int cols;
    int tune_cols;
    int narrow;
    int rank;
    int candidate;
    const char* text;
} hmmr_conv_tile_info_t;
int hmmr_conv_tile_info(int tile, hmmr_conv_tile_info_t* out);
int hmmr_conv_tile_for(int k_order, int filter_1x1, int conv3_form, int cout, int dtype, int candidate);
int hmmr_conv_tile_fits(int tile, int k_order, int filter_1x1, int conv3_form, int cout, int dtype, int win, int ksteps);
int hmmr_conv_tile_f_movie(void);

int hmmr_conv_gemm(const hmmr_conv_desc_t* d, void* stream);
size_t hmmr_conv_splitk_workspace_bytes(int m, int cout, int split_k);

typedef struct {
    const void* w;
    const float* scale;
    const float* shift;
    int tile;
    int k_order;
} hmmr_layer_t;

typedef struct {
    hmmr_layer_t conv1, conv2, conv3, shortcut;
    hmmr_layer_t c3sc;
    hmmr_layer_t sc_c1;
    const void* w3_frag;
    const void* w1n_frag;
    const void* pair_stream;
    const void* conv1_frag;
    const void* unit_stream;
    const float* pre_scale;
    const float* pre_shift;
    int c_in, base, depth, stride;
    int fuse_preact;
    int fuse_tail;
} hmmr_resnet_unit_t;

#define HMMR_RESNET_UNITS 16

typedef struct {
    int dtype;
    hmmr_layer_t stem;
    hmmr_resnet_unit_t unit[HMMR_RESNET_UNITS];
    const float* post_scale;
    const float* post_shift;
} hmmr_resnet_weights_t;

typedef struct {
    int dtype;
    const void* h2; int m; int c_mid; int depth;
    const void* w3; const float* scale3; const float* shift3;
    const void* res; int ldr; int res_strided; int64_t res_img_stride; int res_row_stride, res_px_stride; int ho, wo;
    void* out;
    const float* pre_scale; const float* pre_shift;
    const void* w1; const float* scale1; const float* shift1; int relu1; int n2;
    void* out_h1;
    const void* h1; int hin, win;
    const void* w2; const float* scale2; const float* shift2;
    const void* xp;
    const void* wsc; const float* shift_sc;
    int conv2_stride;
    void* out_pre;
    const void* pair_stream;
    int c_xp;
    const void* unit_stream;
} hmmr_tail_desc_t;
size_t hmmr_pair_stream_bytes(int kc3, int depth, int n2);
size_t hmmr_b1_unit_stream_bytes(int c_xp);
int hmmr_mfma_rate_probe(int workgroups, int n8, float* out, void* stream);
int hmmr_clock_probe(unsigned long long* samples, int n, int sleep, const int* stop, void* stream);
size_t hmmr_conv3x3_stream_bytes(int cin, int cout);
size_t hmmr_conv1x1_stream_bytes(int cin, int cout);
int hmmr_bottleneck_tail(const hmmr_tail_desc_t* d, void* stream);

size_t hmmr_resnet50_workspace_bytes(int n, int dtype);
#define HMMR_RESNET_PROF_SLOTS 64
int hmmr_resnet50_fwd(const hmmr_resnet_weights_t* w, const float* images, int n, int n_zero,
                      float* phi, void* ws, size_t ws_bytes, void* stream, float* prof_ms);

size_t hmmr_resnet50_stem_workspace_bytes(const hmmr_resnet_weights_t* w, int n_total);
int hmmr_resnet50_stem(const hmmr_resnet_weights_t* w, const float* images, int n, int n_zero, void* pooled, void* h1,
                       int* h1_written, void* ws, size_t ws_bytes, void* stream);

enum { HMMR_SC_NONE = 0,
       HMMR_SC_LAUNCH,
       HMMR_SC_LAUNCH_WITH_CONV1,
       HMMR_SC_IN_CONV3,
       HMMR_SC_IN_TAIL };
enum { HMMR_CONV1_LAUNCH = 0,
       HMMR_CONV1_READY };
enum { HMMR_CONV2_LAUNCH = 0, HMMR_CONV2_IN_TAIL };
enum { HMMR_END_CONV3_LAUNCH = 0,
       HMMR_END_TAIL_BF16,
       HMMR_END_TAIL_BF16_STRIDE2,
       HMMR_END_TAIL_SPLIT,
       HMMR_END_B1_UNIT,
       HMMR_END_UNIT_PAIR };
typedef struct {
    int shortcut, conv1, conv2, end;
    int reads_fused_preact;
    int writes_raw, writes_pre;
    int pair_demoted;
    int swaps_t1_t2;
    int leaves_h1;
} hmmr_unit_plan_t;
int hmmr_resnet50_plan(const hmmr_resnet_weights_t* w, int n_total, hmmr_unit_plan_t out[HMMR_RESNET_UNITS]);

typedef struct {
    const float* gn1_gamma; const float* gn1_beta;
    hmmr_layer_t conv1;
    const float* gn2_gamma; const float* gn2_beta;
    hmmr_layer_t conv2;
} hmmr_temporal_block_t;

#define HMMR_MAX_TEMPORAL_BLOCKS 8

typedef struct {
    int dtype;
    int num_blocks;
    hmmr_temporal_block_t block[HMMR_MAX_TEMPORAL_BLOCKS];
} hmmr_temporal_weights_t;

size_t hmmr_temporal_workspace_bytes(int b, int t, int dtype);
int hmmr_temporal_fwd(const hmmr_temporal_weights_t* w, const float* phi, int b, int t,
                      float* strips, void* ws, size_t ws_bytes, void* stream);

typedef struct {
    int dtype;
    hmmr_layer_t fc1, fc2, fc3;
} hmmr_hallucinator_weights_t;

size_t hmmr_hallucinator_workspace_bytes(int m, int dtype);
int hmmr_hallucinator_fwd(const hmmr_hallucinator_weights_t* w, const float* phi, int m,
                          float* out, void* ws, size_t ws_bytes, void* stream);

int hmmr_groupnorm_relu(const float* x, const float* gamma, const float* beta, int b, int t,
                        int c, int groups, void* out, int out_dtype, void* stream);

typedef struct {
    int nd;
    hmmr_layer_t fc1_phi;
    hmmr_layer_t fc1_theta;
    hmmr_layer_t fc2;
    hmmr_layer_t fc3;
} hmmr_ief_regressor_t;

#define HMMR_MAX_REGRESSORS 8

typedef struct {
    int dtype;
    int num_regressors;
    int num_stages;
    hmmr_ief_regressor_t reg[HMMR_MAX_REGRESSORS];
    const float* mean_theta;
    int no_optcam;
    int delta_from_start;
} hmmr_ief_weights_t;

size_t hmmr_ief_workspace_bytes(int m, int num_regressors, int dtype);
int hmmr_ief_fwd(const hmmr_ief_weights_t* w, const float* strips, int m, float* omegas,
                 void* ws, size_t ws_bytes, void* stream);
int hmmr_ief_fwd_from(const hmmr_ief_weights_t* w, const float* strips, const float* omega_start, int m, float* omegas,
                      void* ws, size_t ws_bytes, void* stream);

typedef struct {
    float* d_fc1_phi;
    float* d_fc1_theta;
    float* d_fc2;
    float* d_fc3;
    float* d_b1;
    float* d_b2;
    float* d_b3;
} hmmr_ief_reg_grads_t;

typedef struct {
    const float* strips;
    const float* omega_start;
    const unsigned char* keep;
    float keep_scale;
    int m;
    const float* d_omegas;
    float* d_strips;
    float* d_omega_start;
    hmmr_ief_reg_grads_t reg[HMMR_MAX_REGRESSORS];
} hmmr_ief_bwd_desc_t;

size_t hmmr_ief_bwd_workspace_bytes(int m, int num_regressors, int num_stages);
int hmmr_ief_fwd_train(const hmmr_ief_weights_t* w, const float* strips, const float* omega_start, const unsigned char* keep,
                       float keep_scale, int m, float* omegas, void* ws, size_t ws_bytes, void* stream);
int hmmr_ief_bwd(const hmmr_ief_weights_t* w, const hmmr_ief_bwd_desc_t* desc, void* ws, size_t ws_bytes, void* stream);

typedef struct {
    float* d_gn1_gamma; float* d_gn1_beta;
    float* d_conv1; float* d_b1;
    float* d_gn2_gamma; float* d_gn2_beta;
    float* d_conv2; float* d_b2;
} hmmr_temporal_block_grads_t;

typedef struct {
    const float* phi;
    int b, t;
    const float* d_strips;
    float* d_phi;
    hmmr_temporal_block_grads_t block[HMMR_MAX_TEMPORAL_BLOCKS];
} hmmr_temporal_bwd_desc_t;

size_t hmmr_temporal_bwd_workspace_bytes(int b, int t, int num_blocks);
int hmmr_temporal_bwd(const hmmr_temporal_weights_t* w, const hmmr_temporal_bwd_desc_t* desc, void* ws, size_t ws_bytes, void* stream);

typedef struct {
    const float* phi;
    int m;
    const float* d_out;
    float* d_phi;
    float* d_fc1; float* d_fc2; float* d_fc3;
    float* d_b1; float* d_b2; float* d_b3;
} hmmr_hallucinator_bwd_desc_t;

size_t hmmr_hallucinator_bwd_workspace_bytes(int m);
int hmmr_hallucinator_bwd(const hmmr_hallucinator_weights_t* w, const hmmr_hallucinator_bwd_desc_t* desc, void* ws, size_t ws_bytes,
                          void* stream);

typedef struct {
    int num_verts;
    int num_kps;
    int lbs_nnz;
    int vpad;
    const float* dirs;
    const float* j_template;
    const float* j_shapedirs;
    const int32_t* parents;
    const int32_t* lbs_idx;
    const float* lbs_w;
    const int32_t* kreg_ptr;
    const int32_t* kreg_idx;
    const float* kreg_val;
    const void* dirs_split;
} hmmr_smpl_consts_t;

size_t hmmr_smpl_workspace_bytes(int m);
int hmmr_smpl_fwd(const hmmr_smpl_consts_t* c, const float* theta, int ld_theta,
                  const float* beta, int ld_beta, const float* cams, int ld_cam, int m,
                  float* verts, float* joints, float* kps, float* rs,
                  void* ws, size_t ws_bytes, void* stream);
int hmmr_smpl_fwd_strided(const hmmr_smpl_consts_t* c, const float* theta, int ld_theta,
                          const float* beta, int ld_beta, const float* cams, int ld_cam, int m,
                          float* verts, float* joints, float* kps, float* rs, int64_t ld_out,
                          void* ws, size_t ws_bytes, void* stream);
int hmmr_smpl_fwd_records(const hmmr_smpl_consts_t* c, const float* omegas, int num_containers, int n,
                          float* rec, int64_t ld_rec, const int32_t* field_offsets, void* ws, size_t ws_bytes,
                          void* stream);
int hmmr_global_rigid_transformation(const float* Rs, const float* Js, const int32_t* parents, int m,
                                     float* new_j, float* A, int rotate_base, void* stream);

typedef struct {
    int num_verts;
    int num_kps;
    const int32_t* vk_ptr;
    const int32_t* vk_idx;
    const float* vk_val;
} hmmr_smpl_grad_consts_t;

size_t hmmr_smpl_bwd_workspace_bytes(const hmmr_smpl_consts_t* c, int m);
int hmmr_smpl_bwd(const hmmr_smpl_consts_t* c, const hmmr_smpl_grad_consts_t* g,
                  const float* theta, int ld_theta, const float* beta, int ld_beta,
                  const float* cams, int ld_cam, const float* joints, int m,
                  const float* d_verts, const float* d_joints, const float* d_kps, const float* d_rs,
                  float* d_theta, float* d_beta, float* d_cams,
                  void* ws, size_t ws_bytes, void* stream);

enum { HMMR_LOSS_KP = 1, HMMR_LOSS_KP_OPTCAM = 2, HMMR_LOSS_JOINTS = 4, HMMR_LOSS_SMPL = 8, HMMR_LOSS_CONST = 16,
       HMMR_LOSS_SHAPE_PRIOR = 32 };
enum { HMMR_L_KP = 0, HMMR_L_JOINTS = 1, HMMR_L_SMPL_POSE = 2, HMMR_L_SMPL_SHAPE = 3, HMMR_L_CONST = 4, HMMR_L_SHAPE = 5,
       HMMR_L_TOTAL = 6 };
enum { HMMR_W_KP = 0, HMMR_W_JOINTS = 1, HMMR_W_SMPL = 2, HMMR_W_CONST = 3, HMMR_W_SHAPE = 4 };
#define HMMR_LOSS_NO_VISIBLE 1u
#define HMMR_LOSS_NOT_FINITE 2u
typedef struct {
    int B, T, K;
    int delta_t;
    unsigned flags;
    float weights[6];
    const float* kps_pred;
    const float* joints_pred;
    const float* rs_pred;
    const float* beta_pred;
    int ld_beta;
    const float* kps_gt;
    const float* joints_gt;
    const float* rs_gt;
    const float* shapes_gt;
    const float* has_gt3d_smpl;
    const float* has_gt3d_joints;
    float* losses;
    float* d_kps;
    float* d_joints;
    float* d_rs;
    float* d_beta;
    float* best_cam;
    unsigned* status;
    void* ws;
    size_t ws_bytes;
} hmmr_seq_loss_desc_t;

size_t hmmr_seq_losses_workspace_bytes(int B, int T);
int hmmr_seq_losses(const hmmr_seq_loss_desc_t* d, void* stream);

size_t hmmr_omega_loss_grad_workspace_bytes(const hmmr_smpl_consts_t* c, int B, int T);
int hmmr_omega_loss_grad(const hmmr_smpl_consts_t* c, const hmmr_smpl_grad_consts_t* g, const hmmr_seq_loss_desc_t* gt_and_flags,
                         const float* omega, int use_optcam, float* losses, float* d_omega,
                         void* ws, size_t ws_bytes, void* stream);

int hmmr_crop_frames(const unsigned char* frames, const int32_t* geom, int n, int h, int w,
                     float* out, void* stream);

int hmmr_tube_augment(const void* images, int images_are_u8, int n, int h, int w, const int32_t* geom,
                      const unsigned char* flip, const float* rot, int S, float* out, void* stream);

#define HMMR_TRACK_MAX_KPS 64
#define HMMR_TRACK_MAX_KERNEL 31
#define HMMR_TRACK_MAX_RADIUS 64
#define HMMR_TRACK_MAX_ROWS (1 << 27)
#define HMMR_TRACK_TILE 256
enum { HMMR_TRACK_EMPTY = 1,
       HMMR_TRACK_BEFORE_ORIGIN = 2,
       HMMR_TRACK_CLIPPED = 4,
       HMMR_TRACK_NOT_FINITE = 8 };
size_t hmmr_track_workspace_bytes(int n_total, int n_tracks);
int hmmr_track_bbox(const double* kps, const unsigned char* present, const int32_t* offsets, int n_tracks, int k,
                    double vis_thresh, int kernel_size, const double* gauss_w, int gauss_radius, double* bbox_raw,
                    double* bbox_smooth, int32_t* range, void* ws, size_t ws_bytes, void* stream);
int hmmr_track_smooth(const double* params, const int32_t* offsets, int n_tracks, int kernel_size, const double* gauss_w,
                      int gauss_radius, double* out, void* ws, size_t ws_bytes, void* stream);
int hmmr_track_crop_geom(const double* bbox_smooth, const int32_t* offsets, const int32_t* range, int n_tracks, int h, int w,
                         int32_t* geom, double* info, int32_t* status, void* stream);

int hmmr_render_handoff(const float* cams, int64_t ld_cam, const float* verts, int64_t ld_verts,
                        const float* kps, int64_t ld_kps, const float* geom, int n, int nv, int nk,
                        float* new_cam, float* proj_verts, float* kp_orig, void* stream);

#define HMMR_RENDER_MAX_FRAMES 4096
#define HMMR_RENDER_MIN_SIZE 16
#define HMMR_RENDER_MAX_SIZE 1024
#define HMMR_RENDER_MAX_FACES 65536
enum { HMMR_RENDER_BG_COLOR = 0,
       HMMR_RENDER_BG_FLOAT = 1,
       HMMR_RENDER_BG_FRAME = 2 };
typedef struct {
    const float* verts; int64_t ld_verts;
    const float* cams; int64_t ld_cam;
    const float* geom;
    const int32_t* faces;
    const float* face_colors;
    int64_t ld_face_colors;
    int n, nv, nf, size;
    int rotate;
    float rot[9];
    float color[3];
    float bg_color[3];
    float light_dir[3];
    float light_int_ambient, light_int_directional;
    float light_color_ambient[3], light_color_directional[3];
    int bg_mode;
    const void* bg_image;
    float bg_add, bg_mul;
    int frame_h, frame_w;
    int out_h, out_w;
    unsigned char* rgb;
    float* alpha;
    int32_t* face_index;
    void* ws; size_t ws_bytes;
} hmmr_render_desc_t;
size_t hmmr_render_workspace_bytes(int n, int nv, int nf);
int hmmr_render_mesh(const hmmr_render_desc_t* d, void* stream);

#define HMMR_SCENE_MAX_TRACKS 16
typedef struct {
    const float* verts; int64_t ld_verts;
    const float* cams; int64_t ld_cam;
    const float* geom;
    const float* priority;
    int start, end;
    float color[3];
} hmmr_scene_track_t;
typedef struct {
    const hmmr_scene_track_t* tracks;
    int n_tracks;
    const int32_t* faces;
    int nv, nf, n_frames, size;
    int out_h, out_w;
    float bg_color[3];
    float light_dir[3];
    float light_int_ambient, light_int_directional;
    float light_color_ambient[3], light_color_directional[3];
    int bg_mode;
    const void* bg_image;
    int frame_h, frame_w;
    unsigned char* rgb;
    float* alpha;
    int32_t* face_index;
    int32_t* owner;
    void* ws; size_t ws_bytes;
} hmmr_scene_desc_t;
size_t hmmr_render_scene_workspace_bytes(int n_frames, int n_tracks, int nv, int nf);
int hmmr_render_scene(const hmmr_scene_desc_t* d, void* stream);

enum { HMMR_BBOX_EMPTY = 1, HMMR_BBOX_NOT_FINITE = 2, HMMR_BBOX_DEGENERATE = 4, HMMR_BBOX_BEYOND_START = 8 };
int hmmr_video_bbox(const float* cams, long long ld_cam, const float* kps, long long ld_kps, int k, const double* proc,
                    double proc_size, const int32_t* offsets, int n_tracks, int img_h, int img_w, double margin,
                    int32_t* bbox, float* cams_crop, int32_t* status, void* stream);

#define HMMR_SKELETON_MAX_RADIUS 1024
typedef struct {
    const float* kps; int64_t ld_kps;
    const unsigned char* vis;
    int n, nk, h, w;
    float kp_add, kp_mul;
    int draw_edges;
    int radius;
    const float* bg_float; float bg_add, bg_mul;
    const unsigned char* bg_u8;
    unsigned char* out;
} hmmr_skeleton_desc_t;
int hmmr_skeleton_radius(int h, int w);
int hmmr_draw_skeleton(const hmmr_skeleton_desc_t* d, void* stream);

#define HMMR_COLLAGE_MAX_PANEL_WIDTH 4096
typedef struct {
// ... 123 lines not shown
```

Measured before the change: 39270.

## Compute only kept temporal rows in last conv and pick XCD-aware GEMM tile order

```diff
diff --git a/human_dynamics_amd/_lib.py b/human_dynamics_amd/_lib.py
--- a/human_dynamics_amd/_lib.py
+++ b/human_dynamics_amd/_lib.py
@@ -58,7 +58,7 @@
 
 
 class Debug(C.Structure):
-    _fields_ = [("stem_route", C.c_int), ("stem_no_conv1", C.c_int), ("gemm_probe", C.c_int), ("smpl_blend_mfma", C.c_int), ("ief_no_group", C.c_int), ("reserved", C.c_int * 3),
+    _fields_ = [("stem_route", C.c_int), ("stem_no_conv1", C.c_int), ("gemm_probe", C.c_int), ("smpl_blend_mfma", C.c_int), ("ief_no_group", C.c_int), ("reserved", C.c_int * 2), ("gemm_tile_order", C.c_int),
                 ("pair_min_pixels", C.c_int), ("pair_two_tile_min", C.c_int), ("pair_form", C.c_int)]
 
 
@@ -281,6 +281,7 @@
     "hmmr_launch_counts": (None, [C.POINTER(LaunchCounts), C.c_int]),
     "hmmr_stem_launch_counts": (None, [C.POINTER(StemCounts), C.c_int]),
     "hmmr_conv_gemm": (C.c_int, [C.POINTER(ConvDesc), _vp]),
+    "hmmr_conv_gemm_tile_order": (C.c_int, [C.POINTER(ConvDesc)]),
     "hmmr_conv_tile_info": (C.c_int, [C.c_int, C.POINTER(ConvTileInfo)]),
     "hmmr_conv_tile_for": (C.c_int, [C.c_int] * 6),
     "hmmr_conv_tile_fits": (C.c_int, [C.c_int] * 8),
@@ -294,6 +295,7 @@
     "hmmr_resnet50_plan": (C.c_int, [C.POINTER(ResnetWeights), C.c_int, C.POINTER(UnitPlan)]),
     "hmmr_temporal_workspace_bytes": (C.c_size_t, [C.c_int, C.c_int, C.c_int]),
     "hmmr_temporal_fwd": (C.c_int, [C.POINTER(TemporalWeights), _fp, C.c_int, C.c_int, _fp, _vp, C.c_size_t, _vp]),
+    "hmmr_temporal_fwd_kept": (C.c_int, [C.POINTER(TemporalWeights), _fp, C.c_int, C.c_int, C.c_int, C.c_int, _fp, _vp, C.c_size_t, _vp]),
     "hmmr_hallucinator_workspace_bytes": (C.c_size_t, [C.c_int, C.c_int]),
     "hmmr_hallucinator_fwd": (C.c_int, [C.POINTER(HallucinatorWeights), _fp, C.c_int, _fp, _vp, C.c_size_t, _vp]),
     "hmmr_groupnorm_relu": (C.c_int, [_fp, _fp, _fp, C.c_int, C.c_int, C.c_int, C.c_int, _vp, C.c_int, _vp]),
diff --git a/human_dynamics_amd/csrc/gemm_conv.hip b/human_dynamics_amd/csrc/gemm_conv.hip
--- a/human_dynamics_amd/csrc/gemm_conv.hip
+++ b/human_dynamics_amd/csrc/gemm_conv.hip
@@ -16,6 +16,7 @@
     int cin_log2, KH, KW, SY, SX, PY, PX;
     int res_strided; long long res_img_stride; int res_row_stride, res_px_stride;
     int relu, tiles_n, n_tiles;
+    int tile_order, tiles_m;
     int kt_per_slice;
     long long out_slice_stride;
     int probe;
@@ -84,6 +85,14 @@
 template <typename TO> __device__ __forceinline__ void store_tail(TO* p, const float (&v)[8], int cnt) {
     if constexpr (!std::is_same<TO, bsplit_t>::value)
         for (int j = 0; j < cnt; ++j) p[j] = elem_traits<TO>::from_f32(v[j]);
+}
+
+template <int BM, int BN> __device__ __forceinline__ void tile_origin(const ConvArgs& a, int L, int& m0, int& n0) {
+    const bool m_fast = a.tile_order == 2;
+    const unsigned inner = m_fast ? a.tiles_m : a.tiles_n;
+    const unsigned slow = (unsigned)L / inner, fast = (unsigned)L - slow * inner;
+    m0 = __builtin_amdgcn_readfirstlane((int)(m_fast ? fast : slow) * BM);
+    n0 = __builtin_amdgcn_readfirstlane((int)(m_fast ? slow : fast) * BN);
 }
 
 __device__ const u32x4 g_zero_page[4] = {};
@@ -134,9 +143,8 @@
     const int tid = threadIdx.x;
     const int lane = tid & 63;
     const int wave = __builtin_amdgcn_readfirstlane(tid >> 6);
-    const int L = xcd_remap(blockIdx.x, a.n_tiles);
-    const int m0 = (L / a.tiles_n) * BM;
-    const int n0 = (L % a.tiles_n) * BN;
+    int m0, n0;
+    tile_origin<BM, BN>(a, xcd_remap(blockIdx.x, a.n_tiles), m0, n0);
 
     const int pslot = tid & 7, r0 = tid >> 3;
     const int lslot = pslot ^ ((r0 >> 1) & 7);
@@ -588,9 +596,8 @@
     const int tid = threadIdx.x;
     const int lane = tid & 63;
     const int wave = __builtin_amdgcn_readfirstlane(tid >> 6);
-    const int L = xcd_remap(blockIdx.x, a.n_tiles);
-    const int m0 = (L / a.tiles_n) * BM;
-    const int n0 = (L % a.tiles_n) * BN;
+    int m0, n0;
+    tile_origin<BM, BN>(a, xcd_remap(blockIdx.x, a.n_tiles), m0, n0);
     const int W = a.Win, C = 1 << a.cin_log2;
     const int need = BM + 2 * W + 2;
     constexpr int ZROW = NPP * RPP - 2;
@@ -733,9 +740,8 @@
     const int tid = threadIdx.x;
     const int lane = tid & 63;
     const int wave = __builtin_amdgcn_readfirstlane(tid >> 6);
-    const int L = xcd_remap(blockIdx.x, a.n_tiles);
-    const int m0 = (L / a.tiles_n) * BM;
-    const int n0 = (L % a.tiles_n) * BN;
+    int m0, n0;
+    tile_origin<BM, BN>(a, xcd_remap(blockIdx.x, a.n_tiles), m0, n0);
     const int W = a.Win, C = 1 << a.cin_log2;
     const int need = BM + 2 * W + 2;
     constexpr int ZROW = NPP * RPP - 2;
@@ -843,12 +849,36 @@
     patch_epilogue<TO, BM, BN, WGM, WGN>(a, smem, acc, m0, n0, tid, wm, wn, lr, lh);
 }
 
+static constexpr int TILE_ORDER_MAX_TILES = 256;
+static int conv_tile_order(long long M, int cout, int bm, int bn) {
+    if (const int forced = hmmr_debug_state()->gemm_tile_order; forced == 1 || forced == 2) return forced;
+    const long long tiles_m = (M + bm - 1) / bm, tiles_n = (cout + bn - 1) / bn, n_tiles = tiles_m * tiles_n;
+    if (n_tiles > TILE_ORDER_MAX_TILES) return 1;
+    const long long q = n_tiles >> 3, r = n_tiles & 7;
+    long long rows[2] = {0, 0};
+    for (long long xcd = 0, lo = 0; xcd < 8; ++xcd) {
+        const long long len = q + (xcd < r ? 1 : 0), hi = lo + len;
+        if (!len) break;
+        for (int o = 0; o < 2; ++o) {
+            const long long inner = o ? tiles_m : tiles_n;
+            const long long n_slow = (hi - 1) / inner - lo / inner + 1, n_fast = len < inner ? len : inner;
+            rows[o] += o ? n_fast * bm + n_slow * bn : n_slow * bm + n_fast * bn;
+        }
+        lo = hi;
+    }
+    return rows[1] < rows[0] ? 2 : 1;
+}
+static void plan_tiles(ConvArgs& a, int bm, int bn) {
+    a.tiles_m = (a.M + bm - 1) / bm;
+    a.tiles_n = (a.cout + bn - 1) / bn;
+    a.n_tiles = a.tiles_m * a.tiles_n;
+    a.tile_order = conv_tile_order(a.M, a.cout, bm, bn);
+}
+
 template <typename TA, typename TO, int NPP>
 static int launch_pipe(const ConvArgs& base, hipStream_t stream) {
     ConvArgs a = base;
-    const int tiles_m = (a.M + 255) / 256;
-    a.tiles_n = (a.cout + 127) / 128;
-    a.n_tiles = tiles_m * a.tiles_n;
+    plan_tiles(a, 256, 128);
     constexpr int kloop = 4 * 128 * 128 + 2 * NPP * 64 * 128, epi = 256 * 128 * 4;
     constexpr int lds = kloop > epi ? kloop : epi;
     static_assert(lds <= 160 * 1024, "LDS");
@@ -862,9 +892,7 @@
 template <typename TA, typename TO, int BM, int BN, int WGM, int WGN, int NPP>
 static int launch_patch(const ConvArgs& base, hipStream_t stream) {
     ConvArgs a = base;
-    const int tiles_m = (a.M + BM - 1) / BM;
-    a.tiles_n = (a.cout + BN - 1) / BN;
-    a.n_tiles = tiles_m * a.tiles_n;
+    plan_tiles(a, BM, BN);
     constexpr int kloop = 3 * BN * 128 + 2 * NPP * 64 * 128, epi = BM * BN * 4;
     constexpr int lds = kloop > epi ? kloop : epi;
     static_assert(lds <= 160 * 1024, "LDS");
@@ -906,9 +934,7 @@
 template <typename TA, typename TO, int BM, int BN, int WGM, int WGN, bool PRO, bool UTAP, int NSTAGE>
 static int launch_cfg(const ConvArgs& base, int slices, hipStream_t stream) {
     ConvArgs a = base;
-    const int tiles_m = (a.M + BM - 1) / BM;
-    a.tiles_n = (a.cout + BN - 1) / BN;
-    a.n_tiles = tiles_m * a.tiles_n;
+    plan_tiles(a, BM, BN);
     constexpr int kring = NSTAGE * (BM + BN) * 128, epi = BM * BN * 4;
     const int kloop = kring + ((PRO && NSTAGE >= 3) ? 8 * a.K : 0);
     const int lds = kloop > epi ? kloop : epi;
@@ -1028,6 +1054,27 @@
 
 int hmmr_conv3x3_stream(const hmmr_conv_desc_t* d, hipStream_t stream);
 int hmmr_conv1x1_stream(const hmmr_conv_desc_t* d, hipStream_t stream);
+
+static int splitk_slices(int split_k, int nk) {
+    int slices = split_k > 1 ? split_k : 1;
+    if (slices > nk) slices = nk;
+    return (nk + ((nk + slices - 1) / slices) - 1) / ((nk + slices - 1) / slices);
+}
+
+extern "C" int hmmr_conv_gemm_tile_order(const hmmr_conv_desc_t* d) {
+    HMMR_REQUIRE(d, "hmmr_conv_gemm_tile_order: null descriptor");
+    HMMR_REQUIRE(d->k_order == 0 || d->k_order == 1, "hmmr_conv_gemm_tile_order: the stream kernels (k_order 2) walk their tiles in an order of their own");
+    HMMR_REQUIRE(d->in_dtype == HMMR_F32 || d->in_dtype == HMMR_BF16 || d->in_dtype == HMMR_F16X3, "hmmr_conv_gemm_tile_order: bad dtype %d", d->in_dtype);
+    const long long esz = d->in_dtype == HMMR_BF16 ? 2 : 4;
+    const long long M = (long long)d->n_img * d->ho * d->wo;
+    const int K = d->kh * d->kw * d->cin + (d->in2 ? d->cin2 : 0);
+    HMMR_REQUIRE(M > 0 && K > 0 && d->cout > 0 && K % (int)(128 / esz) == 0, "hmmr_conv_gemm_tile_order: empty or ragged problem");
+    int tile = d->tile;
+    if (!tile) tile = d->k_order ? conv_tiles::choose_patch() : conv_tiles::choose_generic(M, d->cout, splitk_slices(d->split_k, K / (int)(128 / esz)));
+    const hmmr_conv_tile_info_t* t = conv_tiles::row(tile);
+    HMMR_REQUIRE(t && t->family == conv_tiles::family_of(d->k_order, 0), "hmmr_conv_gemm_tile_order: %s has no tile %d", conv_tiles::family_name(conv_tiles::family_of(d->k_order, 0)), tile);
+    return conv_tile_order(M, d->cout, t->pixels, t->channels);
+}
 
 extern "C" int hmmr_conv_gemm(const hmmr_conv_desc_t* d, void* stream) {
     HMMR_REQUIRE(d && d->in && d->w && (d->out || d->out2), "hmmr_conv_gemm: null operand");
@@ -1077,7 +1124,7 @@
     a.cin_log2 = cl2; a.KH = d->kh; a.KW = d->kw; a.SY = d->sy; a.SX = d->sx; a.PY = d->py; a.PX = d->px;
     a.res_strided = d->res_strided; a.res_img_stride = d->res_img_stride;
     a.res_row_stride = d->res_row_stride; a.res_px_stride = d->res_px_stride;
-    a.relu = d->relu; a.tiles_n = 0; a.n_tiles = 0;
+    a.relu = d->relu; a.tiles_n = 0; a.n_tiles = 0; a.tile_order = 1; a.tiles_m = 0;
     a.kt_per_slice = 0; a.out_slice_stride = 0; a.probe = 0;
     a.in2 = d->in2; a.cin2 = d->in2 ? d->cin2 : 0; a.kt_split = d->cin / bke;
     a.batch = d->batch > 1 ? d->batch : 1;
@@ -1112,9 +1159,7 @@
     const bool out16 = d->out_dtype == HMMR_BF16, out32 = d->out_dtype == HMMR_F32, outx3 = d->out_dtype == HMMR_F16X3;
     HMMR_REQUIRE((in16 || in32 || inx3) && (out16 || out32 || outx3), "hmmr_conv_gemm: unsupported dtypes %d -> %d", d->in_dtype, d->out_dtype);
     const int nk = K / bke;
-    int slices = d->split_k > 1 ? d->split_k : 1;
-    if (slices > nk) slices = nk;
-    slices = (nk + ((nk + slices - 1) / slices) - 1) / ((nk + slices - 1) / slices);
+    const int slices = splitk_slices(d->split_k, nk);
     if (slices > 1) {
         const int ldw = (d->cout + 127) / 128 * 128;
         const long long plane = (long long)a.M * ldw;
diff --git a/human_dynamics_amd/csrc/tail_sched.h b/human_dynamics_amd/csrc/tail_sched.h
--- a/human_dynamics_amd/csrc/tail_sched.h
+++ b/human_dynamics_amd/csrc/tail_sched.h
@@ -32,6 +32,17 @@
     return d;
 }
 
+static inline hmmr_conv_desc_t temporal_conv_kept_desc(const void* in, int in_dtype, const hmmr_layer_t& l, const float* res, float* out, int b, int t,
+                                                       int first, int keep, void* sk, size_t skbytes) {
+    constexpr int C = TAIL_C;
+    hmmr_conv_desc_t d = temporal_conv_desc(in, in_dtype, l, nullptr, out, b, t, sk, skbytes);
+    const int above = first > 0 ? 1 : 0, below = first + keep < t ? 1 : 0;
+    d.in = (const char*)in + (size_t)(first - above) * C * (in_dtype == HMMR_BF16 ? 2 : 4);
+    d.hin = keep + above + below; d.py = 1 - above; d.ho = keep;
+    if (res) { d.res = res + (size_t)first * C; d.res_strided = 1; d.res_img_stride = (int64_t)t * C; d.res_row_stride = C; d.res_px_stride = C; }
+    return d;
+}
+
 static inline hmmr_conv_desc_t fc_desc(const void* in, int in_dtype, int m, int k, const hmmr_layer_t& l, void* out, int out_dtype, int cout,
                                        int ldo, int split_k = 0, void* sk = nullptr, size_t skbytes = 0) {
     hmmr_conv_desc_t d = {};
diff --git a/human_dynamics_amd/csrc/temporal.hip b/human_dynamics_amd/csrc/temporal.hip
--- a/human_dynamics_amd/csrc/temporal.hip
+++ b/human_dynamics_amd/csrc/temporal.hip
@@ -74,13 +74,14 @@
     return b > 0 && t > 0 ? temporal_layout(b, t, dtype).total : 0;
 }
 
-extern "C" int hmmr_temporal_fwd(const hmmr_temporal_weights_t* w, const float* phi, int b, int t,
-                                 float* strips, void* ws, size_t ws_bytes, void* stream) {
-    HMMR_REQUIRE(w && phi && strips && ws, "hmmr_temporal_fwd: null argument");
-    HMMR_REQUIRE(b > 0 && t > 0, "hmmr_temporal_fwd: bad shape");
-    HMMR_REQUIRE(w->num_blocks >= 1 && w->num_blocks <= HMMR_MAX_TEMPORAL_BLOCKS, "hmmr_temporal_fwd: bad num_blocks");
+static int temporal_run(const char* who, const hmmr_temporal_weights_t* w, const float* phi, int b, int t, int first, int keep,
+                        float* strips, void* ws, size_t ws_bytes, void* stream) {
+    HMMR_REQUIRE(w && phi && strips && ws, "%s: null argument", who);
+    HMMR_REQUIRE(b > 0 && t > 0, "%s: bad shape", who);
+    HMMR_REQUIRE(keep < 0 || (first >= 0 && keep > 0 && first + keep <= t), "%s: kept rows %d .. %d outside a window of %d", who, first, first + keep, t);
+    HMMR_REQUIRE(w->num_blocks >= 1 && w->num_blocks <= HMMR_MAX_TEMPORAL_BLOCKS, "%s: bad num_blocks", who);
     const MovieBufs L = temporal_layout(b, t, w->dtype);
-    HMMR_REQUIRE(ws_bytes >= L.total, "hmmr_temporal_fwd: workspace too small");
+    HMMR_REQUIRE(ws_bytes >= L.total, "%s: workspace too small", who);
     constexpr int C = TAIL_C;
     char* base = (char*)ws;
     void* h = base + L.buf[0];
@@ -93,11 +94,23 @@
         hmmr_conv_desc_t d = temporal_conv_desc(h, w->dtype, B.conv1, nullptr, h1, b, t, base + L.sk, L.skbytes);
         if (hmmr_conv_gemm(&d, stream)) return -2;
         if (hmmr_groupnorm_relu(h1, B.gn2_gamma, B.gn2_beta, b, t, C, GN_GROUPS, h, w->dtype, stream)) return -2;
-        d = temporal_conv_desc(h, w->dtype, B.conv2, cur, dst, b, t, base + L.sk, L.skbytes);
+        d = (keep >= 0 && dst == strips) ? temporal_conv_kept_desc(h, w->dtype, B.conv2, cur, dst, b, t, first, keep, base + L.sk, L.skbytes)
+                                         : temporal_conv_desc(h, w->dtype, B.conv2, cur, dst, b, t, base + L.sk, L.skbytes);
         if (hmmr_conv_gemm(&d, stream)) return -2;
         cur = dst;
     }
     return 0;
+}
+
+extern "C" int hmmr_temporal_fwd(const hmmr_temporal_weights_t* w, const float* phi, int b, int t,
+                                 float* strips, void* ws, size_t ws_bytes, void* stream) {
+    return temporal_run("hmmr_temporal_fwd", w, phi, b, t, 0, -1, strips, ws, ws_bytes, stream);
+}
+
+extern "C" int hmmr_temporal_fwd_kept(const hmmr_temporal_weights_t* w, const float* phi, int b, int t, int first, int keep,
+                                      float* out_kept, void* ws, size_t ws_bytes, void* stream) {
+    HMMR_REQUIRE(keep >= 0, "hmmr_temporal_fwd_kept: kept rows %d .. %d outside a window of %d", first, first + keep, t);
+    return temporal_run("hmmr_temporal_fwd_kept", w, phi, b, t, first, keep, out_kept, ws, ws_bytes, stream);
 }
 
 extern "C" size_t hmmr_hallucinator_workspace_bytes(int m, int dtype) {
diff --git a/human_dynamics_amd/engine.py b/human_dynamics_amd/engine.py
--- a/human_dynamics_amd/engine.py
+++ b/human_dynamics_amd/engine.py
@@ -19,11 +19,12 @@
 TILE_TABLES = os.path.join(os.path.dirname(os.path.abspath(__file__)), "tile_tables.json")
 
 
-def set_debug(stem_route=0, stem_no_conv1=0, gemm_probe=0, smpl_blend_mfma=0, ief_no_group=0, pair_min_pixels=0, pair_two_tile_min=0, pair_form=0):
+def set_debug(stem_route=0, stem_no_conv1=0, gemm_probe=0, smpl_blend_mfma=0, ief_no_group=0, pair_min_pixels=0, pair_two_tile_min=0, pair_form=0,
+              gemm_tile_order=0):
     d = L.Debug()
     d.stem_route, d.stem_no_conv1, d.gemm_probe = int(stem_route), int(stem_no_conv1), int(gemm_probe)
     d.smpl_blend_mfma, d.ief_no_group, d.pair_min_pixels = int(smpl_blend_mfma), int(ief_no_group), int(pair_min_pixels)
-    d.pair_two_tile_min, d.pair_form = int(pair_two_tile_min), int(pair_form)
+    d.pair_two_tile_min, d.pair_form, d.gemm_tile_order = int(pair_two_tile_min), int(pair_form), int(gemm_tile_order)
     L.load().hmmr_set_debug(C.byref(d))
 
 
@@ -102,6 +103,7 @@
         self.resnet_chunk = int(devflags.get("RESNET_CHUNK") or resnet_chunk)
         self.store = packing.DeviceStore(self.device)
         self.num_conv_layers = num_conv_layers
+        self.kept_strips = True
         self.delta_keys = sorted(int(d) for d in delta_t_values)
         w = weights if weights is not None else {}
         for name, v in w.items():
@@ -350,6 +352,18 @@
         ws = self._ws["temporal"].get(nbytes)
         L.check(self.lib.hmmr_temporal_fwd(C.byref(self.tw), phi.data_ptr(), b, t, out.data_ptr(),
                                            ws.data_ptr(), nbytes, self._stream()), "hmmr_temporal_fwd")
+        return out
+
+    def temporal_kept(self, phi, first, keep, out=None):
+        self._need(self.tw, "AZ_FC_block*")
+        phi = self.to_device(phi)
+        b, t, c = phi.shape
+        assert c == 2048
+        out = self._out(out, (b, keep, c))
+        nbytes = self.lib.hmmr_temporal_workspace_bytes(b, t, self.temporal_dtype)
+        ws = self._ws["temporal"].get(nbytes)
+        L.check(self.lib.hmmr_temporal_fwd_kept(C.byref(self.tw), phi.data_ptr(), b, t, int(first), int(keep), out.data_ptr(),
+                                                ws.data_ptr(), nbytes, self._stream()), "hmmr_temporal_fwd_kept")
         return out
 
     def hallucinate(self, phi, out=None):
diff --git a/human_dynamics_amd/evaluation/tester.py b/human_dynamics_amd/evaluation/tester.py
--- a/human_dynamics_amd/evaluation/tester.py
+++ b/human_dynamics_amd/evaluation/tester.py
@@ -285,19 +285,22 @@
                                            n_zero=n_zero if last else 0))
         return torch.cat(outs, dim=0)
 
-    def predict_strips_records(self, windows, n_keep, out=None):
+    def _kept_strips(self, windows, n_keep):
         T = self.sequence_length
         margin = (self.fov - 1) // 2
-        strips = self._movie_strips(windows)
-        kept = strips[:, margin:T - margin].reshape(-1, strips.shape[-1])[:n_keep]
-        return self.predict_records(kept, out)
+        if self.pred_mode == "pred" and getattr(self.engine, "kept_strips", True) and T > 2 * margin:
+            if self.num_conv_layers != self.engine.num_conv_layers:
+                raise ValueError("engine was packed with num_conv_layers=%d" % self.engine.num_conv_layers)
+            kept = self.engine.temporal_kept(windows, margin, T - 2 * margin)
+        else:
+            kept = self._movie_strips(windows)[:, margin:T - margin]
+        return kept.reshape(-1, kept.shape[-1])[:n_keep]
+
+    def predict_strips_records(self, windows, n_keep, out=None):
+        return self.predict_records(self._kept_strips(windows, n_keep), out)
 
     def predict_strips_omegas(self, windows, n_keep):
-        T = self.sequence_length
-        margin = (self.fov - 1) // 2
-        strips = self._movie_strips(windows)
-        kept = strips[:, margin:T - margin].reshape(-1, strips.shape[-1])[:n_keep]
-        return self.engine.ief(kept)
+        return self.engine.ief(self._kept_strips(windows, n_keep))
 
     def predict_strips_device(self, windows, n_keep):
         from ..dist import unpack_outputs
diff --git a/include/hmmr_hip.h b/include/hmmr_hip.h
--- a/include/hmmr_hip.h
+++ b/include/hmmr_hip.h
@@ -25,7 +25,8 @@
     int gemm_probe;
     int smpl_blend_mfma;
     int ief_no_group;
-    int reserved[3];
+    int reserved[2];
+    int gemm_tile_order;
     int pair_min_pixels;
     int pair_two_tile_min;
     int pair_form;
@@ -114,6 +115,7 @@
 int hmmr_conv_tile_f_movie(void);
 
 int hmmr_conv_gemm(const hmmr_conv_desc_t* d, void* stream);
+int hmmr_conv_gemm_tile_order(const hmmr_conv_desc_t* d);
 size_t hmmr_conv_splitk_workspace_bytes(int m, int cout, int split_k);
 
 typedef struct {
@@ -228,6 +230,8 @@
 size_t hmmr_temporal_workspace_bytes(int b, int t, int dtype);
 int hmmr_temporal_fwd(const hmmr_temporal_weights_t* w, const float* phi, int b, int t,
                       float* strips, void* ws, size_t ws_bytes, void* stream);
+int hmmr_temporal_fwd_kept(const hmmr_temporal_weights_t* w, const float* phi, int b, int t, int first, int keep,
+                           float* out_kept, void* ws, size_t ws_bytes, void* stream);
 
 typedef struct {
     int dtype;
```

Measured after the change: 39650 (median of 6 runs). About the same (+1.0%).
